# salesforce/LayoutDETR

Measured on AMD Instinct MI355X. Metric: images/sec G+D fwd-bwd, 256x256 bg x9 elems, higher is better.
Workload: dtype f32

## Files before the change

### include/ldetr_hip.h

```cpp
#ifndef LDETR_HIP_H
#define LDETR_HIP_H

#include <stdint.h>

#ifdef __cplusplus
extern "C" {
#endif

const char* ldetr_last_error(void);
int ldetr_abi_version(void);

int ldetr_debug_trace_tiles(int64_t* buffer);

int ldetr_set_split_bf16(int tiles);

int ldetr_engine_launch_counts(int64_t* f32_pipe, int64_t* bf16_split_pipe);

int ldetr_set_workspace(void* ptr, int64_t bytes);

typedef struct ldetr_tensor4 {
    int N, C, H, W;
    int64_t sn, sc, sh, sw;
} ldetr_tensor4;

typedef struct ldetr_epilogue {
    float alpha;
    const float* col_scale;
    const float* col_bias;
    const float* samp_scale;
    int64_t samp_ld;
    const float* residual;
    int64_t ldr;
    int act;
    float act_alpha;
    float act_gain;
    const float* mask_src;
    int64_t ldm;
    int mask_mode;
    float out_scale;
    float p_drop;
    uint64_t seed;
    const uint64_t* seed_ptr;
    int accumulate;
    float* a_rowsum;
} ldetr_epilogue;

int ldetr_bias_act_f32(const float* x, const float* b, const float* xref, const float* yref, const float* dy, float* y,
                       int64_t sizeX, int sizeB, int64_t stepB, int grad, int act, float alpha, float gain, float clamp,
                       void* stream);

int ldetr_upfirdn2d_f32(const float* x, const float* f, float* y, int N, int C, int inH, int inW,
                        const int64_t* x_strides_nchw, int fh, int fw, int64_t f_stride_h, int64_t f_stride_w,
                        int upx, int upy, int downx, int downy, int padx0, int padx1, int pady0, int pady1, int flip,
                        float gain, int outH, int outW, const int64_t* y_strides_nchw,
                        const float* act_bias, int has_act, float act_alpha, float act_gain, void* stream);

int ldetr_gemm_f32(const float* A, int64_t lda, int ta, const float* B, int64_t ldb, int tb, float* C, int64_t ldc,
                   int M, int N, int K, int splitk, const ldetr_epilogue* ep, int pix_per_sample, void* stream);

typedef struct ldetr_gemm_desc {
    const float* A; int64_t lda; int ta;
    const float* B; int64_t ldb; int tb;
    float* C; int64_t ldc;
    int M, N, K, splitk;
    const ldetr_epilogue* ep;
    int pix_per_sample;
} ldetr_gemm_desc;
int ldetr_gemm_pair_f32(const ldetr_gemm_desc* g0, const ldetr_gemm_desc* g1, void* stream);
int ldetr_gemm_pair_is_single_launch(const ldetr_gemm_desc* g0, const ldetr_gemm_desc* g1);

#define LDETR_GEMM_GROUP_MAX 32
int ldetr_gemm_small_group_f32(const ldetr_gemm_desc* g, const float* post_scale, int n, void* stream);

int ldetr_conv2d_fwd_f32(const float* x, const ldetr_tensor4* xt, const float* w, int Cout, int KH, int KW, int stride,
                         int pad, float* y, int64_t ldy, int OH, int OW, const float* in_scale, int64_t in_scale_ld,
                         const ldetr_epilogue* ep, void* stream);
int ldetr_conv2d_bwd_data_f32(const float* dy, const ldetr_tensor4* dyt, const float* w, int Cin, int KH, int KW,
                              int stride, int pad, float* dx, int64_t lddx, int IH, int IW, const float* dy_scale,
                              int64_t dy_scale_ld, const ldetr_epilogue* ep, void* stream);
int ldetr_conv2d_bwd_weight_f32(const float* x, const ldetr_tensor4* xt, const float* dy, const ldetr_tensor4* dyt,
                                float* dw, int KH, int KW, int stride, int pad, int splitk, const float* x_scale,
                                int64_t x_scale_ld, const float* dy_scale, int64_t dy_scale_ld, int accumulate, void* stream);

int ldetr_conv_transpose2d_fwd_f32(const float* x, const ldetr_tensor4* xt, const float* w, int Cout, int KH, int KW,
                                   int stride, int pad, float* y, int64_t ldy, int OH, int OW, const float* in_scale,
                                   int64_t in_scale_ld, const ldetr_epilogue* ep, void* stream);
int ldetr_conv_transpose2d_bwd_data_f32(const float* dy, const ldetr_tensor4* dyt, const float* w, int Cin, int KH,
                                        int KW, int stride, int pad, float* dx, int64_t lddx, int IH, int IW,
                                        const float* dy_scale, int64_t dy_scale_ld, const ldetr_epilogue* ep,
                                        void* stream);
int ldetr_conv_transpose2d_bwd_weight_f32(const float* x, const ldetr_tensor4* xt, const float* dy,
                                          const ldetr_tensor4* dyt, float* dw, int KH, int KW, int stride, int pad,
                                          int splitk, const float* x_scale, int64_t x_scale_ld, const float* dy_scale,
                                          int64_t dy_scale_ld, int accumulate, void* stream);

int ldetr_attention_fwd_f32(const float* q, int64_t ldq, const float* k, int64_t ldk, const float* v, int64_t ldv,
                            const unsigned char* key_padding_mask, float* out, int64_t ldo, float* lse, int B, int H,
                            int Lq, int Lk, int head_dim, float scale, float p_drop, uint64_t seed, const uint64_t* seed_ptr,
                            int causal, void* stream);
int ldetr_attention_bwd_f32(const float* q, int64_t ldq, const float* k, int64_t ldk, const float* v, int64_t ldv,
                            const unsigned char* key_padding_mask, const float* out, int64_t ldo, const float* lse,
                            const float* dout, int64_t lddo, float* dq, int64_t lddq, float* dk, int64_t lddk,
                            float* dv, int64_t lddv, int B, int H, int Lq, int Lk, int head_dim, float scale,
                            float p_drop, uint64_t seed, const uint64_t* seed_ptr, int causal, void* stream);

int ldetr_torgb_bwd_finish_f32(const float* dws, const float* s, const float* w, int B, int C, float* dw, float* ds, void* stream);

int ldetr_loss_combine_fwd_f32(const float* const* x, const float* w, const int* n, const int* fn, const int* red, int K, int ld,
                               float* vals, float* sums, float* total, void* stream);
int ldetr_loss_combine_bwd_f32(const float* const* x, const float* w, const int* n, const int* fn, const int* red, int K, int ld,
                               const float* g, float* grads, void* stream);
int ldetr_masked_mse_fwd_f32(const float* a, const float* b, const uint8_t* valid, int64_t rows, int D, int bdiv, float* out2, void* stream);
int ldetr_masked_mse_bwd_f32(const float* a, const float* b, const uint8_t* valid, int64_t rows, int D, int bdiv, const float* out2,
                             const float* g, float* da, void* stream);

typedef struct ldetr_ln_args {
    const float* x; const float* r; const float* gamma; const float* beta;
    float* y; float* z; float* mean; float* rstd;
    const float* dy; float* dx; float* dr; float* dgamma; float* dbeta;
    int64_t rows; int D; float eps, p_drop; uint64_t seed; const uint64_t* seed_ptr;
    const float* pos; int64_t pos_rows; float* ypos; const float* dy2;
    int r_parts; int64_t r_part_stride; const float* r_bias;
    const float* dy_parts; int dy_nparts; int64_t dy_part_stride;
} ldetr_ln_args;
int ldetr_layernorm_fwd_group_f32(const ldetr_ln_args* a, int n, void* stream);
int ldetr_layernorm_bwd_group_f32(const ldetr_ln_args* a, int n, void* stream);
int ldetr_sum_parts_f32(const float* base, const float* parts, int n_parts, int64_t part_stride, float* out, int64_t n, void* stream);

typedef struct ldetr_ffn_args {
    const float* x; int64_t ldx;
    const float* w1; const float* b1;
    const float* w2;
    float* h;
    float* ypart;
    int M, F;
    float p_drop; uint64_t seed; const uint64_t* seed_ptr;
    const float* dy;
    float* dxpart;
    float* dh;
} ldetr_ffn_args;
int ldetr_ffn_fwd_group_f32(const ldetr_ffn_args* a, int n, void* stream);
int ldetr_ffn_bwd_group_f32(const ldetr_ffn_args* a, int n, void* stream);

typedef struct ldetr_mha_small_args {
    const float* x; int64_t ldx;
    const float* w_in; const float* b_in; const float* w_out;
    const unsigned char* kpm;
    float* qkv; float* o; float* lse; float* ypart;
    int B, L;
    float scale, p_drop; uint64_t seed; const uint64_t* seed_ptr;
    const float* dr;
    float* dqkv; float* dxpart;
} ldetr_mha_small_args;
int ldetr_mha_small_fwd_group_f32(const ldetr_mha_small_args* a, int n, void* stream);
int ldetr_mha_small_bwd_group_f32(const ldetr_mha_small_args* a, int n, void* stream);

typedef struct ldetr_mha_cross_args {
// ... 296 lines not shown
```

### layoutdetr_amd/_lib.py

```python
import ctypes
import os
from ctypes import (POINTER, Structure, c_char_p, c_double, c_float, c_int, c_int64, c_ubyte, c_uint64, c_void_p)

_HERE = os.path.dirname(os.path.abspath(__file__))
ABI_VERSION = 25
LIB_PATH = os.environ.get('LDETR_LIB') or os.path.join(_HERE, 'lib', 'libldetr_hip.so')


class Tensor4(Structure):
    _fields_ = [('N', c_int), ('C', c_int), ('H', c_int), ('W', c_int),
                ('sn', c_int64), ('sc', c_int64), ('sh', c_int64), ('sw', c_int64)]


class GemmDesc(Structure):
    _fields_ = [('A', c_void_p), ('lda', c_int64), ('ta', c_int), ('B', c_void_p), ('ldb', c_int64), ('tb', c_int),
                ('C', c_void_p), ('ldc', c_int64), ('M', c_int), ('N', c_int), ('K', c_int), ('splitk', c_int),
                ('ep', c_void_p), ('pix_per_sample', c_int)]


class P3Epilogue(Structure):
    _fields_ = [('alpha', c_float), ('col_scale', c_void_p), ('col_bias', c_void_p), ('residual_p3', c_void_p),
                ('residual_f32', c_void_p), ('relu_mask_p3', c_void_p), ('relu', c_int)]


class Epilogue(Structure):
    _fields_ = [('alpha', c_float), ('col_scale', c_void_p), ('col_bias', c_void_p), ('samp_scale', c_void_p),
                ('samp_ld', c_int64), ('residual', c_void_p), ('ldr', c_int64), ('act', c_int),
                ('act_alpha', c_float), ('act_gain', c_float), ('mask_src', c_void_p), ('ldm', c_int64),
                ('mask_mode', c_int), ('out_scale', c_float), ('p_drop', c_float), ('seed', c_uint64),
                ('seed_ptr', c_void_p), ('accumulate', c_int), ('a_rowsum', c_void_p)]


class LnArgs(Structure):
    _fields_ = [('x', c_void_p), ('r', c_void_p), ('gamma', c_void_p), ('beta', c_void_p),
                ('y', c_void_p), ('z', c_void_p), ('mean', c_void_p), ('rstd', c_void_p),
                ('dy', c_void_p), ('dx', c_void_p), ('dr', c_void_p), ('dgamma', c_void_p), ('dbeta', c_void_p),
                ('rows', c_int64), ('D', c_int), ('eps', c_float), ('p_drop', c_float), ('seed', c_uint64), ('seed_ptr', c_void_p),
                ('pos', c_void_p), ('pos_rows', c_int64), ('ypos', c_void_p), ('dy2', c_void_p),
                ('r_parts', c_int), ('r_part_stride', c_int64), ('r_bias', c_void_p),
                ('dy_parts', c_void_p), ('dy_nparts', c_int), ('dy_part_stride', c_int64)]


class FfnArgs(Structure):
    _fields_ = [('x', c_void_p), ('ldx', c_int64), ('w1', c_void_p), ('b1', c_void_p), ('w2', c_void_p), ('h', c_void_p), ('ypart', c_void_p),
                ('M', c_int), ('F', c_int), ('p_drop', c_float), ('seed', c_uint64), ('seed_ptr', c_void_p),
                ('dy', c_void_p), ('dxpart', c_void_p), ('dh', c_void_p)]


class MhaSmallArgs(Structure):
    _fields_ = [('x', c_void_p), ('ldx', c_int64), ('w_in', c_void_p), ('b_in', c_void_p), ('w_out', c_void_p), ('kpm', c_void_p),
                ('qkv', c_void_p), ('o', c_void_p), ('lse', c_void_p), ('ypart', c_void_p), ('B', c_int), ('L', c_int),
                ('scale', c_float), ('p_drop', c_float), ('seed', c_uint64), ('seed_ptr', c_void_p),
                ('dr', c_void_p), ('dqkv', c_void_p), ('dxpart', c_void_p)]


class MhaCrossArgs(Structure):
    _fields_ = [('x', c_void_p), ('ldx', c_int64), ('w_q', c_void_p), ('b_q', c_void_p), ('k', c_void_p), ('ldk', c_int64), ('v', c_void_p), ('ldv', c_int64),
                ('w_out', c_void_p), ('kpm', c_void_p), ('q', c_void_p), ('o', c_void_p), ('lse', c_void_p), ('ypart', c_void_p),
                ('B', c_int), ('Lq', c_int), ('Lk', c_int), ('scale', c_float), ('p_drop', c_float), ('seed', c_uint64), ('seed_ptr', c_void_p),
                ('dr', c_void_p), ('dq', c_void_p), ('dk', c_void_p), ('lddk', c_int64), ('dv', c_void_p), ('lddv', c_int64), ('dxpart', c_void_p)]


class WgradDesc(Structure):
    _fields_ = [('A', c_void_p), ('lda', c_int64), ('B', c_void_p), ('ldb', c_int64), ('dW', c_void_p), ('ldw', c_int64), ('db', c_void_p),
                ('M', c_int), ('rows', c_int), ('cols', c_int)]


class DemodDesc(Structure):
    _fields_ = [('weight', c_void_p), ('so', c_int64), ('si', c_int64), ('sh', c_int64), ('sw', c_int64),
                ('styles', c_void_p), ('dcoefs', c_void_p), ('w2', c_void_p), ('grad_dcoefs', c_void_p), ('dweight', c_void_p), ('dstyles', c_void_p),
                ('O', c_int), ('I', c_int), ('KH', c_int), ('KW', c_int)]


class AffineDesc(Structure):
    _fields_ = [('ds', c_void_p), ('A', c_void_p), ('dA', c_void_p), ('db', c_void_p), ('C', c_int), ('scale', c_float), ('post', c_float)]


class LayoutRasterArgs(Structure):
    _fields_ = [('struct_bytes', c_int), ('B', c_int), ('N', c_int), ('S', c_int), ('nrow', c_int), ('n_colors', c_int), ('n_pages', c_int),
                ('bbox', c_void_p), ('valid', c_void_p), ('labels', c_void_p), ('palette', c_void_p), ('page_wh', c_void_p),
                ('pages', c_void_p), ('pages_bytes', c_int64), ('page_table', c_void_p), ('page_index', c_void_p),
                ('coeffs', c_void_p), ('coeffs_len', c_int64), ('cell_coeffs', c_void_p), ('cells_dev', c_void_p), ('out', c_void_p)]


class PatchResizeArgs(Structure):
    _fields_ = [('struct_bytes', c_int), ('n_jobs', c_int), ('src0', c_void_p), ('src0_bytes', c_int64), ('src1', c_void_p), ('src1_bytes', c_int64),
                ('dst', c_void_p), ('dst_bytes', c_int64), ('jobs', c_void_p), ('tables', c_void_p), ('tables_host', c_void_p), ('tables_len', c_int64),
                ('jobs_dev', c_void_p)]


class ImageRasterArgs(Structure):
    _fields_ = [('struct_bytes', c_int), ('B', c_int), ('N', c_int), ('S', c_int), ('nrow', c_int),
                ('bbox', c_void_p), ('valid', c_void_p), ('rects', c_void_p), ('patch_off', c_void_p), ('page_off', c_void_p), ('page_wh', c_void_p),
# ... 37 lines not shown
                            _I, _F, _I, _I, POINTER(c_int64), _P, _I, _F, _F, _P],
    'ldetr_gemm_f32': [_P, _L, _I, _P, _L, _I, _P, _L, _I, _I, _I, _I, _EP, _I, _P],
    'ldetr_conv2d_fwd_f32': [_P, _T4, _P, _I, _I, _I, _I, _I, _P, _L, _I, _I, _P, _L, _EP, _P],
    'ldetr_conv2d_bwd_data_f32': [_P, _T4, _P, _I, _I, _I, _I, _I, _P, _L, _I, _I, _P, _L, _EP, _P],
    'ldetr_conv2d_bwd_weight_f32': [_P, _T4, _P, _T4, _P, _I, _I, _I, _I, _I, _P, _L, _P, _L, _I, _P],
    'ldetr_conv_transpose2d_fwd_f32': [_P, _T4, _P, _I, _I, _I, _I, _I, _P, _L, _I, _I, _P, _L, _EP, _P],
    'ldetr_conv_transpose2d_bwd_data_f32': [_P, _T4, _P, _I, _I, _I, _I, _I, _P, _L, _I, _I, _P, _L, _EP, _P],
    'ldetr_conv_transpose2d_bwd_weight_f32': [_P, _T4, _P, _T4, _P, _I, _I, _I, _I, _I, _P, _L, _P, _L, _I, _P],
    'ldetr_attention_fwd_f32': [_P, _L, _P, _L, _P, _L, _P, _P, _L, _P, _I, _I, _I, _I, _I, _F, _F, c_uint64, _P, _I, _P],
    'ldetr_attention_bwd_f32': [_P, _L, _P, _L, _P, _L, _P, _P, _L, _P, _P, _L, _P, _L, _P, _L, _P, _L,
                                _I, _I, _I, _I, _I, _F, _F, c_uint64, _P, _I, _P],
    'ldetr_colsum_f32': [_P, _P, _I, _L, _I, _P],
    'ldetr_act_bwd_reduce_f32': [_P, _P, _P, _P, _P, _P, _P, _I, _L, _I, _I, _F, _F, _P],
    'ldetr_mul_reduce_f32': [_P, _P, _P, _P, _P, _I, _L, _I, _P],
    'ldetr_torgb_fwd_f32': [_P, _P, _P, _P, _P, _I, _L, _I, _P],
    'ldetr_torgb_bwd_f32': [_P, _P, _P, _P, _P, _P, _P, _I, _L, _I, _P],
    'ldetr_maxpool3x3s2_fwd_f32': [_P, _P, _P, _I, _I, _I, _I, _P],
    'ldetr_maxpool3x3s2_bwd_f32': [_P, _P, _P, _I, _I, _I, _I, _P],
    'ldetr_grad_sanitize_f32': [_P, _L, _F, _F, _F, _F, _P],
    'ldetr_adam_step_f32': [_P, _P, _P, _P, _L, _L, _F, _F, _F, _F, _I, _F, _F, _F, _F, _P],
    'ldetr_adam_ema_step_f32': [_P, _P, _P, _P, _L, _L, _F, _F, _F, _F, _I, _F, _F, _F, _F, _P, _F, _P],
    'ldetr_ema_lerp_f32': [_P, _P, _L, _F, _P],
    'ldetr_lsap_f64': [_P, _I, _I, _I, _P, _P, _P],
    'ldetr_layoutnet_features_f32': [_P, _P, _P, POINTER(c_int), _I, _P, _L, _I, _I, _I, _P, _P],
    'ldetr_layoutnet_forward_f32': [_P, _P, _P, _P, _L, _P, _L, _I, _I, _I, _P, _P, _P, _P, _P],
    'ldetr_feature_stats_f64': [_P, _L, _I, _P, _P, _P],
    'ldetr_box_giou_pairwise_f32': [_P, _P, _I, _I, _I, _I, _P, _P, _P, _P, c_double, _P],
    'ldetr_bmm_strided_f32': [_P, _P, _P, _P, _P, _P, _I, _I, _I, _I, _I, _F, _P],
    'ldetr_softmax_xent_fwd_f32': [_P, _L, _P, _P, _P, _P, _L, _I, _L, _F, _P],
    'ldetr_softmax_xent_bwd_f32': [_P, _L, _P, _P, _P, _P, _P, _L, _L, _I, _L, _F, _P],
    'ldetr_embedding_fwd_f32': [_P, _P, _P, _P, _L, _I, _I, _I, _P],
    'ldetr_embedding_bwd_f32': [_P, _P, _P, _L, _I, _I, _L, _P],
    'ldetr_debug_trace_tiles': [_P],
    'ldetr_set_split_bf16': [c_int],
    'ldetr_engine_launch_counts': [POINTER(c_int64), POINTER(c_int64)],
    'ldetr_layernorm_fwd_group_f32': [_P, _I, _P],
    'ldetr_layernorm_bwd_group_f32': [_P, _I, _P],
    'ldetr_sum_parts_f32': [_P, _P, _I, _L, _P, _L, _P],
    'ldetr_ffn_fwd_group_f32': [_P, _I, _P],
    'ldetr_ffn_bwd_group_f32': [_P, _I, _P],
    'ldetr_mha_small_fwd_group_f32': [_P, _I, _P],
    'ldetr_mha_small_bwd_group_f32': [_P, _I, _P],
    'ldetr_mha_cross_fwd_f32': [_P, _P],
    'ldetr_mha_cross_bwd_f32': [_P, _P],
    'ldetr_wgrad_multi_f32': [_P, _I, _P],
    'ldetr_loss_combine_fwd_f32': [_P, _P, _P, _P, _P, _I, _I, _P, _P, _P, _P],
    'ldetr_loss_combine_bwd_f32': [_P, _P, _P, _P, _P, _I, _I, _P, _P, _P],
    'ldetr_masked_mse_fwd_f32': [_P, _P, _P, _L, _I, _I, _P, _P],
    'ldetr_masked_mse_bwd_f32': [_P, _P, _P, _L, _I, _I, _P, _P, _P, _P],
    'ldetr_torgb_bwd_finish_f32': [_P, _P, _P, _I, _I, _P, _P, _P],
    'ldetr_sg2_handoff_f32': [_P, _P, _P, _P, _P, _P, _P, _P, _P, _P, _P, _P, _P, _P, _I, _L, _I, _F, _F, _P],
    'ldetr_gemm_pair_f32': [_P, _P, _P],
    'ldetr_gemm_pair_is_single_launch': [_P, _P],
    'ldetr_demod_fwd_f32': [_P, _L, _L, _L, _L, _P, _P, _P, _I, _I, _I, _I, _I, _F, _P],
    'ldetr_demod_bwd_f32': [_P, _L, _L, _L, _L, _P, _P, _P, _P, _P, _I, _P, _I, _I, _I, _I, _I, _P],
    'ldetr_demod_group_fwd_f32': [_P, _I, _I, _F, _P],
    'ldetr_demod_group_bwd_f32': [_P, _I, _I, _I, _I, _P],
    'ldetr_sg2_affine_bwd_f32': [_P, _I, _P, _P, _I, _P, _L, _I, _I, _P],
    'ldetr_gemm_small_group_f32': [_P, _P, _I, _P],
    'ldetr_torgb_fwd_add_f32': [_P, _P, _P, _P, _P, _P, _I, _L, _I, _P],
    'ldetr_layout_losses_f32': [_P, _P, _P, _I, _I, _P, _P, _P],
    'ldetr_layout_losses_bwd_f32': [_P, _P, _I, _I, _P, _P],
    'ldetr_layout_finish_f32': [_P, _P, _P, _P, _P, _P, _P, _P, _P, _I, _I, _I, _P],
    'ldetr_resample_coeffs': [_I, _I, _P, _P, _L, _P],
    'ldetr_resample_coeffs_filter': [_I, _I, _I, _P, _P, _L, _P],
    'ldetr_layout_raster_cell_size': [_I, _I, _I, _P, _P],
    'ldetr_layout_raster_u8': [_P, _P],
    'ldetr_patch_resize_u8': [_P, _P],
    'ldetr_image_raster_u8': [_P, _P],
    'ldetr_p3_split_f32': [_P, _L, _P, _L, _I, _P],
    'ldetr_p3_merge_f32': [_P, _P, _L, _L, _I, _P],
    'ldetr_p3_weight_bwd': [_P, _P, _P, _I, _I, _I, _I, _P],
    'ldetr_p3_conv2d_bwd_data': [_P, _I, _I, _I, _I, _P, _I, _I, _I, _I, _I, _I, _I, _P, _P, _P, _P],
    'ldetr_p3_conv2d_fwd': [_P, _I, _I, _I, _I, _P, _I, _I, _I, _I, _I, _P, _P, _P, _P],
    'ldetr_p3_conv2d_bwd_weight': [_P, _I, _I, _I, _I, _P, _I, _I, _I, _I, _I, _P, _P, _P],
    'ldetr_p3_weight_prep': [_P, _I, _I, _P],
    'ldetr_p3_conv2d_fwd_dual': [_P, _P, _I, _I, _I, _I, _P, _P, _I, _I, _I, _I, _I, _P, _P, _P, _P, _P, _P, _P],
    'ldetr_p3_conv2d_bwd_pair': [_P, _I, _I, _I, _I, _P, _P, _I, _I, _I, _I, _I, _I, _I, _P, _P, _P, _P, _P, _P, _P],
    'ldetr_p3_last_launch': [_P],
    'ldetr_engine_last_launch': [_P],
    'ldetr_struct_sizes': [_P],
    'ldetr_resize_normalize_u8': [_P, _L, _I, _I, _I, _I, _P, _P, _I, _P, _P, _I, _P, _P, _P, _F, _F, _F, _F, _F, _F, _P],
    'ldetr_page_filter_u8': [_P, _P, _L, _I, _I, _I, _F, _P],
    'ldetr_png_scan': [_P, _L, _P, _P, _P, _P, _L, _P, _P, _L, _P],
    'ldetr_png_decode_u8': [_P, _P],
    'ldetr_png_encode_bound': [_I, _I, _P, _P],
    'ldetr_png_encode_u8': [_P, _P],
    'ldetr_png_index_bytes': [_I, _I, _P],
    'ldetr_png_scan_packed': [_P, _L, _P, _P, _P, _L, _P, _P, _P, _L, _P],
    'ldetr_png_inflate_u8': [_P, _P],
}

_lib = None


def load():
    global _lib
    if _lib is not None:
        return _lib
    if not os.path.exists(LIB_PATH):
        raise RuntimeError(
            f'{LIB_PATH} not found: build the gfx950 kernels first (python -m layoutdetr_amd.build or '
            f'__graft_entry__.build()).  layoutdetr_amd has no CPU/PyTorch fallback path.')
    import torch
    lib = ctypes.CDLL(LIB_PATH)
    lib.ldetr_last_error.restype = c_char_p
# ... 23 lines not shown
```

### layoutdetr_amd/csrc/attention.hip

```cpp
#include "ldetr_common.hpp"
#include "../../include/ldetr_hip.h"

namespace ldetr {

struct AttnParams {
    const float* q; const float* k; const float* v;
    long ldq, ldk, ldv;
    const unsigned char* kpm;
    float* o; long ldo;
    float* lse;
    const float* dout; long lddo;
    float* dq; long lddq;
    float* dk; long lddk;
    float* dv; long lddv;
    int B, H, Lq, Lk;
    float scale, p_drop;
    unsigned long long seed;
    const unsigned long long* seed_ptr;
    int causal;
};

#define MFMA16(a, b, c) __builtin_amdgcn_mfma_f32_16x16x4f32((a), (b), (c), 0, 0, 0)

__device__ __forceinline__ float ldz(const float* p, bool ok, const float* safe) {
    const float v = *(ok ? p : safe);
    return ok ? v : 0.f;
}

__device__ __forceinline__ float attn_drop(const AttnParams& p, int bh, int q, int key, float inv_keep) {
    return drop_scale(p.seed + (p.seed_ptr ? *p.seed_ptr : 0ull), ((uint64_t)bh * p.Lq + q) * p.Lk + key, p.p_drop, inv_keep);
}

template <int NKT, int DHC>
__global__ __launch_bounds__(64) void attn_fwd_kernel(AttnParams p) {
    constexpr int DH = 32 * DHC;
    const int nqt = (p.Lq + 15) >> 4;
    const int qt = blockIdx.x % nqt;
    const int bh = blockIdx.x / nqt;
    const int b = bh / p.H, h = bh - b * p.H;
    const int lane = threadIdx.x, li = lane & 15, g = lane >> 4;
    const int q0 = qt << 4;
    const int qrow = q0 + li;
    const bool qok = qrow < p.Lq;
    const float* qp = p.q + ((long)b * p.Lq + qrow) * p.ldq + h * DH;
    const float* kb = p.k + (long)b * p.Lk * p.ldk + h * DH;
    const float* vb = p.v + (long)b * p.Lk * p.ldv + h * DH;
    const unsigned char* kpm = p.kpm ? p.kpm + (long)b * p.Lk : nullptr;

    float qf[8 * DHC];
#pragma unroll
    for (int kk = 0; kk < 8 * DHC; kk++) qf[kk] = ldz(qp + 4 * kk + g, qok, p.q) * p.scale;

    f32x4 s[NKT];
    float mx = -INFINITY;
#pragma unroll
    for (int j = 0; j < NKT; j++) {
        f32x4 acc = {0.f, 0.f, 0.f, 0.f};
        const int krow = 16 * j + li;
        const bool kok = krow < p.Lk;
        const float* kp = kb + (long)krow * p.ldk;
#pragma unroll
        for (int kk = 0; kk < 8 * DHC; kk++) acc = MFMA16(ldz(kp + 4 * kk + g, kok, p.q), qf[kk], acc);
#pragma unroll
        for (int r = 0; r < 4; r++) {
            int key = 16 * j + 4 * g + r;
            bool masked = (key >= p.Lk) || (kpm && kpm[key]) || (p.causal && key > qrow);
            acc[r] = masked ? -INFINITY : acc[r];
            mx = fmaxf(mx, acc[r]);
        }
        s[j] = acc;
    }
    mx = fmaxf(mx, __shfl_xor(mx, 16, 64));
    mx = fmaxf(mx, __shfl_xor(mx, 32, 64));
    float sum = 0.f;
#pragma unroll
    for (int j = 0; j < NKT; j++)
#pragma unroll
        for (int r = 0; r < 4; r++) { float e = expf(s[j][r] - mx); s[j][r] = e; sum += e; }
    sum += __shfl_xor(sum, 16, 64);
    sum += __shfl_xor(sum, 32, 64);
    const float inv = 1.f / sum;
    if (p.lse && g == 0 && qok) p.lse[(long)bh * p.Lq + qrow] = mx + logf(sum);
    const float inv_keep = p.p_drop > 0.f ? 1.f / (1.f - p.p_drop) : 1.f;

    f32x4 o[2 * DHC];
#pragma unroll
    for (int c = 0; c < 2 * DHC; c++) o[c] = f32x4{0.f, 0.f, 0.f, 0.f};
#pragma unroll
    for (int j = 0; j < NKT; j++) {
#pragma unroll
        for (int t = 0; t < 4; t++) {
            const int key = 16 * j + 4 * g + t;
            const bool kok = key < p.Lk;
            float pv = s[j][t] * inv;
            if (p.p_drop > 0.f) pv *= attn_drop(p, bh, qrow, key, inv_keep);
            const float* vp = vb + (long)key * p.ldv;
#pragma unroll
            for (int c = 0; c < 2 * DHC; c++) o[c] = MFMA16(ldz(vp + 16 * c + li, kok, p.q), pv, o[c]);
        }
    }
    if (qok) {
        float* op = p.o + ((long)b * p.Lq + qrow) * p.ldo + h * DH + 4 * g;
#pragma unroll
        for (int c = 0; c < 2 * DHC; c++) *reinterpret_cast<float4*>(op + 16 * c) = make_float4(o[c][0], o[c][1], o[c][2], o[c][3]);
    }
}

template <int DHC>
__global__ __launch_bounds__(64) void attn_fwd_long_kernel(AttnParams p) {
    constexpr int DH = 32 * DHC, NKT = 16;
    const int nqt = (p.Lq + 15) >> 4;
    const int qt = blockIdx.x % nqt;
    const int bh = blockIdx.x / nqt;
    const int b = bh / p.H, h = bh - b * p.H;
    const int lane = threadIdx.x, li = lane & 15, g = lane >> 4;
    const int qrow = (qt << 4) + li;
    const bool qok = qrow < p.Lq;
    const float* qp = p.q + ((long)b * p.Lq + qrow) * p.ldq + h * DH;
    const float* kb = p.k + (long)b * p.Lk * p.ldk + h * DH;
    const float* vb = p.v + (long)b * p.Lk * p.ldv + h * DH;
    const unsigned char* kpm = p.kpm ? p.kpm + (long)b * p.Lk : nullptr;
    const float inv_keep = p.p_drop > 0.f ? 1.f / (1.f - p.p_drop) : 1.f;

    float qf[8 * DHC];
#pragma unroll
    for (int kk = 0; kk < 8 * DHC; kk++) qf[kk] = ldz(qp + 4 * kk + g, qok, p.q) * p.scale;

    f32x4 o[2 * DHC];
#pragma unroll
    for (int c = 0; c < 2 * DHC; c++) o[c] = f32x4{0.f, 0.f, 0.f, 0.f};
    float run_max = -INFINITY, run_sum = 0.f;
    const int nkt = (p.Lk + 15) >> 4;
    for (int j0 = 0; j0 < nkt; j0 += NKT) {
        f32x4 s[NKT];
        float mx = run_max;
#pragma unroll
        for (int j = 0; j < NKT; j++) {
            f32x4 acc = {0.f, 0.f, 0.f, 0.f};
            const int krow = 16 * (j0 + j) + li;
            const bool kok = krow < p.Lk;
            const float* kp = kb + (long)krow * p.ldk;
#pragma unroll
            for (int kk = 0; kk < 8 * DHC; kk++) acc = MFMA16(ldz(kp + 4 * kk + g, kok, p.q), qf[kk], acc);
#pragma unroll
            for (int r = 0; r < 4; r++) {
                const int key = 16 * (j0 + j) + 4 * g + r;
                const bool masked = (key >= p.Lk) || (kpm && kpm[key]) || (p.causal && key > qrow);
                acc[r] = masked ? -INFINITY : acc[r];
                mx = fmaxf(mx, acc[r]);
            }
            s[j] = acc;
        }
        mx = fmaxf(mx, __shfl_xor(mx, 16, 64));
        mx = fmaxf(mx, __shfl_xor(mx, 32, 64));
        const float ref = (mx == -INFINITY) ? 0.f : mx;
        const float alpha = expf(run_max - ref);
        float sum = 0.f;
#pragma unroll
        for (int j = 0; j < NKT; j++)
#pragma unroll
            for (int r = 0; r < 4; r++) { const float e = expf(s[j][r] - ref); s[j][r] = e; sum += e; }
        sum += __shfl_xor(sum, 16, 64);
        sum += __shfl_xor(sum, 32, 64);
        run_sum = run_sum * alpha + sum;
        run_max = mx;
#pragma unroll
        for (int c = 0; c < 2 * DHC; c++) { o[c][0] *= alpha; o[c][1] *= alpha; o[c][2] *= alpha; o[c][3] *= alpha; }
#pragma unroll
        for (int j = 0; j < NKT; j++) {
#pragma unroll
            for (int t = 0; t < 4; t++) {
                const int key = 16 * (j0 + j) + 4 * g + t;
                const bool kok = key < p.Lk;
                float pv = s[j][t];
                if (p.p_drop > 0.f) pv *= attn_drop(p, bh, qrow, key, inv_keep);
                const float* vp = vb + (long)key * p.ldv;
#pragma unroll
                for (int c = 0; c < 2 * DHC; c++) o[c] = MFMA16(ldz(vp + 16 * c + li, kok, p.q), pv, o[c]);
            }
        }
    }
    const float inv = 1.f / run_sum;
    if (p.lse && g == 0 && qok) p.lse[(long)bh * p.Lq + qrow] = run_max + logf(run_sum);
    if (qok) {
        float* op = p.o + ((long)b * p.Lq + qrow) * p.ldo + h * DH + 4 * g;
#pragma unroll
        for (int c = 0; c < 2 * DHC; c++)
            *reinterpret_cast<float4*>(op + 16 * c) = make_float4(o[c][0] * inv, o[c][1] * inv, o[c][2] * inv, o[c][3] * inv);
    }
}

template <int NCH, int DHC>
__global__ __launch_bounds__(256) void attn_fwd_wide_kernel(AttnParams p) {
    constexpr int DH = 32 * DHC, DHP = DH + 4, NKT = 4 * NCH;
    extern __shared__ __attribute__((aligned(16))) float kv_tile[];
    const int nq64 = (p.Lq + 63) >> 6;
    const int qb = blockIdx.x % nq64;
    const int bh = blockIdx.x / nq64;
    const int b = bh / p.H, h = bh - b * p.H;
    const int wave = threadIdx.x >> 6, lane = threadIdx.x & 63, li = lane & 15, g = lane >> 4;
    const int qrow = (qb << 6) + (wave << 4) + li;
    const bool qok = qrow < p.Lq;
    const float* qp = p.q + ((long)b * p.Lq + qrow) * p.ldq + h * DH;
    const float* kb = p.k + (long)b * p.Lk * p.ldk + h * DH;
    const float* vb = p.v + (long)b * p.Lk * p.ldv + h * DH;
    const unsigned char* kpm = p.kpm ? p.kpm + (long)b * p.Lk : nullptr;

    auto stage = [&](const float* base, long ld, int key0) {
        constexpr int F4 = DH / 4;
        for (int i = threadIdx.x; i < 64 * F4; i += 256) {
            const int row = i / F4, c4 = i - row * F4;
            float4 v = make_float4(0.f, 0.f, 0.f, 0.f);
            if (key0 + row < p.Lk) v = *reinterpret_cast<const float4*>(base + (long)(key0 + row) * ld + 4 * c4);
            *reinterpret_cast<float4*>(kv_tile + row * DHP + 4 * c4) = v;
        }
    };

    float qf[8 * DHC];
#pragma unroll
    for (int kk = 0; kk < 8 * DHC; kk++) qf[kk] = ldz(qp + 4 * kk + g, qok, p.q) * p.scale;

    f32x4 s[NKT];
    float mx = -INFINITY;
#pragma unroll
    for (int c = 0; c < NCH; c++) {
        if (c > 0) __syncthreads();
        stage(kb, p.ldk, 64 * c);
        __syncthreads();
#pragma unroll
        for (int jj = 0; jj < 4; jj++) {
            const int j = 4 * c + jj;
            f32x4 acc = {0.f, 0.f, 0.f, 0.f};
            const float* kp = kv_tile + (16 * jj + li) * DHP + g;
#pragma unroll
            for (int kk = 0; kk < 8 * DHC; kk++) acc = MFMA16(kp[4 * kk], qf[kk], acc);
#pragma unroll
            for (int r = 0; r < 4; r++) {
                const int key = 16 * j + 4 * g + r;
                const bool masked = (key >= p.Lk) || (kpm && kpm[key]) || (p.causal && key > qrow);
                acc[r] = masked ? -INFINITY : acc[r];
                mx = fmaxf(mx, acc[r]);
            }
            s[j] = acc;
        }
    }
    mx = fmaxf(mx, __shfl_xor(mx, 16, 64));
    mx = fmaxf(mx, __shfl_xor(mx, 32, 64));
    float sum = 0.f;
#pragma unroll
    for (int j = 0; j < NKT; j++)
#pragma unroll
        for (int r = 0; r < 4; r++) { float e = expf(s[j][r] - mx); s[j][r] = e; sum += e; }
    sum += __shfl_xor(sum, 16, 64);
    sum += __shfl_xor(sum, 32, 64);
    const float inv = 1.f / sum;
    if (p.lse && g == 0 && qok) p.lse[(long)bh * p.Lq + qrow] = mx + logf(sum);
    const float inv_keep = p.p_drop > 0.f ? 1.f / (1.f - p.p_drop) : 1.f;

    f32x4 o[2 * DHC];
#pragma unroll
    for (int cc = 0; cc < 2 * DHC; cc++) o[cc] = f32x4{0.f, 0.f, 0.f, 0.f};
#pragma unroll
    for (int c = 0; c < NCH; c++) {
        __syncthreads();
        stage(vb, p.ldv, 64 * c);
        __syncthreads();
#pragma unroll
        for (int jj = 0; jj < 4; jj++) {
            const int j = 4 * c + jj;
#pragma unroll
            for (int t = 0; t < 4; t++) {
                const int key = 16 * j + 4 * g + t;
                float pv = s[j][t] * inv;
                if (p.p_drop > 0.f) pv *= attn_drop(p, bh, qrow, key, inv_keep);
                const float* vp = kv_tile + (16 * jj + 4 * g + t) * DHP + li;
#pragma unroll
                for (int cc = 0; cc < 2 * DHC; cc++) o[cc] = MFMA16(vp[16 * cc], pv, o[cc]);
            }
        }
    }
    if (qok) {
        float* op = p.o + ((long)b * p.Lq + qrow) * p.ldo + h * DH + 4 * g;
#pragma unroll
        for (int cc = 0; cc < 2 * DHC; cc++) *reinterpret_cast<float4*>(op + 16 * cc) = make_float4(o[cc][0], o[cc][1], o[cc][2], o[cc][3]);
    }
}

template <int NKT, int DHC>
__device__ __forceinline__ void attn_bwd_dq(const AttnParams& p, int bh, int qt) {
    constexpr int DH = 32 * DHC;
    const int b = bh / p.H, h = bh - b * p.H;
    const int lane = threadIdx.x, li = lane & 15, g = lane >> 4;
    const int qrow = (qt << 4) + li;
    const bool qok = qrow < p.Lq;
    const float* qp = p.q + ((long)b * p.Lq + qrow) * p.ldq + h * DH;
    const float* dop = p.dout + ((long)b * p.Lq + qrow) * p.lddo + h * DH;
    const float* op = p.o + ((long)b * p.Lq + qrow) * p.ldo + h * DH;
    const float* kb = p.k + (long)b * p.Lk * p.ldk + h * DH;
    const float* vb = p.v + (long)b * p.Lk * p.ldv + h * DH;
    const unsigned char* kpm = p.kpm ? p.kpm + (long)b * p.Lk : nullptr;
    const float inv_keep = p.p_drop > 0.f ? 1.f / (1.f - p.p_drop) : 1.f;

    float qf[8 * DHC], dof[8 * DHC];
    float delta = 0.f;
#pragma unroll
    for (int kk = 0; kk < 8 * DHC; kk++) {
        qf[kk] = ldz(qp + 4 * kk + g, qok, p.q) * p.scale;
        dof[kk] = ldz(dop + 4 * kk + g, qok, p.q);
        delta += dof[kk] * ldz(op + 4 * kk + g, qok, p.q);
    }
    delta += __shfl_xor(delta, 16, 64);
    delta += __shfl_xor(delta, 32, 64);
    const float lse = qok ? p.lse[(long)bh * p.Lq + qrow] : 0.f;

    f32x4 dq[2 * DHC];
#pragma unroll
    for (int c = 0; c < 2 * DHC; c++) dq[c] = f32x4{0.f, 0.f, 0.f, 0.f};
    const int nkt_all = (p.Lk + 15) >> 4;
    for (int j0 = 0; j0 < nkt_all; j0 += NKT)
#pragma unroll
    for (int jj = 0; jj < NKT; jj++) {
        const int j = j0 + jj;
        f32x4 sacc = {0.f, 0.f, 0.f, 0.f}, dpacc = {0.f, 0.f, 0.f, 0.f};
        const int krow = 16 * j + li;
        const bool kok = krow < p.Lk;
        const float* kp = kb + (long)krow * p.ldk;
        const float* vp = vb + (long)krow * p.ldv;
#pragma unroll
        for (int kk = 0; kk < 8 * DHC; kk++) {
            sacc = MFMA16(ldz(kp + 4 * kk + g, kok, p.q), qf[kk], sacc);
            dpacc = MFMA16(ldz(vp + 4 * kk + g, kok, p.q), dof[kk], dpacc);
        }
        f32x4 ds;
#pragma unroll
        for (int r = 0; r < 4; r++) {
            int key = 16 * j + 4 * g + r;
            bool masked = (key >= p.Lk) || (kpm && kpm[key]) || (p.causal && key > qrow);
            float pr = masked ? 0.f : expf(sacc[r] - lse);
// ... 188 lines not shown
            const float* qp = Qs + (16 * jq + li) * DHP + g;
            const float* dop = Ds + (16 * jq + li) * DHP + g;
#pragma unroll
            for (int kk = 0; kk < 8; kk++) {
                sacc = MFMA16(qp[4 * kk] * p.scale, kf[kk], sacc);
                dpacc = MFMA16(dop[4 * kk], vf[kk], dpacc);
            }
            float pd[4], ds[4];
#pragma unroll
            for (int r = 0; r < 4; r++) {
                const int qr = 16 * jq + 4 * g + r;
                const bool qok = qr < p.Lq;
                const float pr = (kmasked || !qok || (p.causal && krow > qr)) ? 0.f : expf(sacc[r] - lse_s[qr]);
                float dm = 1.f;
                if (p.p_drop > 0.f) dm = attn_drop(p, bh, qr, krow, inv_keep);
                pd[r] = pr * dm;
                ds[r] = pr * (dpacc[r] * dm - delta_s[qr]) * p.scale;
            }
#pragma unroll
            for (int t = 0; t < 4; t++) {
                const int qr = 16 * jq + 4 * g + t;
#pragma unroll
                for (int c = 0; c < 2; c++) {
                    dv[c] = MFMA16(Ds[qr * DHP + 16 * c + li], pd[t], dv[c]);
                    dk[c] = MFMA16(Qs[qr * DHP + 16 * c + li], ds[t], dk[c]);
                }
            }
        }
        if (kok) {
            float* dkp = p.dk + ((long)b * p.Lk + krow) * p.lddk + h * DH + 4 * g;
            float* dvp = p.dv + ((long)b * p.Lk + krow) * p.lddv + h * DH + 4 * g;
#pragma unroll
            for (int c = 0; c < 2; c++) {
                *reinterpret_cast<float4*>(dkp + 16 * c) = make_float4(dk[c][0], dk[c][1], dk[c][2], dk[c][3]);
                *reinterpret_cast<float4*>(dvp + 16 * c) = make_float4(dv[c][0], dv[c][1], dv[c][2], dv[c][3]);
            }
        }
    }
}

static int check_attn(const AttnParams& p, const char* what) {
    LDETR_CHECK(p.q && p.k && p.v && p.o, "%s: null pointer", what);
    LDETR_CHECK(p.B > 0 && p.H > 0 && p.Lq > 0 && p.Lk > 0, "%s: empty problem", what);
    LDETR_CHECK(p.Lk <= 16384, "%s: Lk > 16384 is unsupported", what);
    LDETR_CHECK(p.p_drop >= 0.f && p.p_drop < 1.f, "%s: dropout must be in [0,1)", what);
    LDETR_CHECK((p.ldo % 4) == 0 && ((uintptr_t)p.o & 15) == 0, "%s: output must be 16-byte aligned", what);
    return LDETR_OK;
}

}

using namespace ldetr;

extern "C" int ldetr_attention_fwd_f32(const float* q, int64_t ldq, const float* k, int64_t ldk, const float* v, int64_t ldv,
                                       const unsigned char* key_padding_mask, float* out, int64_t ldo, float* lse,
                                       int B, int H, int Lq, int Lk, int head_dim, float scale,
                                       float p_drop, uint64_t seed, const uint64_t* seed_ptr, int causal, void* stream) {
    LDETR_CHECK(head_dim >= 32 && head_dim <= 192 && head_dim % 32 == 0, "attention_fwd: head_dim must be a multiple of 32 up to 192 (got %d)", head_dim);
    AttnParams p; memset(&p, 0, sizeof(p));
    p.q = q; p.k = k; p.v = v; p.ldq = ldq; p.ldk = ldk; p.ldv = ldv; p.kpm = key_padding_mask;
    p.o = out; p.ldo = ldo; p.lse = lse; p.B = B; p.H = H; p.Lq = Lq; p.Lk = Lk;
    p.scale = scale; p.p_drop = p_drop; p.seed = seed; p.seed_ptr = (const unsigned long long*)seed_ptr; p.causal = causal;
    LDETR_CHECK(!causal || Lq == Lk, "attention_fwd: the causal mask is defined for self-attention (Lq == Lk)");
    int rc = check_attn(p, "attention_fwd");
    if (rc) return rc;
    const int nqt = (Lq + 15) / 16, nkt = (Lk + 15) / 16;
    const int grid = B * H * nqt;
    hipStream_t st = (hipStream_t)stream;
#define LDETR_ATTN_FWD(DHC)                                                                     \
    do {                                                                                         \
        if (nkt <= 1) hipLaunchKernelGGL((attn_fwd_kernel<1, DHC>), grid, 64, 0, st, p);         \
        else if (nkt <= 2) hipLaunchKernelGGL((attn_fwd_kernel<2, DHC>), grid, 64, 0, st, p);    \
        else if (nkt <= 4) hipLaunchKernelGGL((attn_fwd_kernel<4, DHC>), grid, 64, 0, st, p);    \
        else if (nkt <= 8) hipLaunchKernelGGL((attn_fwd_kernel<8, DHC>), grid, 64, 0, st, p);    \
        else hipLaunchKernelGGL((attn_fwd_kernel<16, DHC>), grid, 64, 0, st, p);                 \
    } while (0)
    if (nkt > 16) {
        switch (head_dim / 32) {
            case 1: hipLaunchKernelGGL((attn_fwd_long_kernel<1>), grid, 64, 0, st, p); break;
            case 2: hipLaunchKernelGGL((attn_fwd_long_kernel<2>), grid, 64, 0, st, p); break;
            case 3: hipLaunchKernelGGL((attn_fwd_long_kernel<3>), grid, 64, 0, st, p); break;
            case 4: hipLaunchKernelGGL((attn_fwd_long_kernel<4>), grid, 64, 0, st, p); break;
            case 5: hipLaunchKernelGGL((attn_fwd_long_kernel<5>), grid, 64, 0, st, p); break;
            default: hipLaunchKernelGGL((attn_fwd_long_kernel<6>), grid, 64, 0, st, p); break;
        }
        return check_launch("attention_fwd_long");
    }
    if ((head_dim >= 64 || Lq >= 48) && (ldk % 4) == 0 && (ldv % 4) == 0 && ((((uintptr_t)k) | ((uintptr_t)v)) & 15) == 0) {
        const int nch = (Lk + 63) / 64, wgrid = B * H * ((Lq + 63) / 64);
#define LDETR_ATTN_WIDE(NCH, DHC)                                                                                         \
    do {                                                                                                                   \
        constexpr size_t lds = (size_t)64 * (32 * DHC + 4) * sizeof(float);                                                \
        hipLaunchKernelGGL((attn_fwd_wide_kernel<NCH, DHC>), wgrid, 256, lds, st, p);                                      \
    } while (0)
#define LDETR_ATTN_WIDE_D(DHC)                                                                                            \
    do {                                                                                                                   \
        if (nch <= 1) LDETR_ATTN_WIDE(1, DHC); else if (nch <= 2) LDETR_ATTN_WIDE(2, DHC);                                 \
        else if (nch <= 3) LDETR_ATTN_WIDE(3, DHC); else LDETR_ATTN_WIDE(4, DHC);                                          \
    } while (0)
        switch (head_dim / 32) {
            case 1: LDETR_ATTN_WIDE_D(1); break;
            case 2: LDETR_ATTN_WIDE_D(2); break;
            case 3: LDETR_ATTN_WIDE_D(3); break;
            case 4: LDETR_ATTN_WIDE_D(4); break;
            case 5: LDETR_ATTN_WIDE_D(5); break;
            default: LDETR_ATTN_WIDE_D(6); break;
        }
#undef LDETR_ATTN_WIDE_D
#undef LDETR_ATTN_WIDE
        return check_launch("attention_fwd_wide");
    }
    switch (head_dim / 32) {
        case 1: LDETR_ATTN_FWD(1); break;
        case 2: LDETR_ATTN_FWD(2); break;
        case 3: LDETR_ATTN_FWD(3); break;
        case 4: LDETR_ATTN_FWD(4); break;
        case 5: LDETR_ATTN_FWD(5); break;
        default: LDETR_ATTN_FWD(6); break;
    }
#undef LDETR_ATTN_FWD
    return check_launch("attention_fwd");
}

extern "C" int ldetr_attention_bwd_f32(const float* q, int64_t ldq, const float* k, int64_t ldk, const float* v, int64_t ldv,
                                       const unsigned char* key_padding_mask, const float* out, int64_t ldo, const float* lse,
                                       const float* dout, int64_t lddo,
                                       float* dq, int64_t lddq, float* dk, int64_t lddk, float* dv, int64_t lddv,
                                       int B, int H, int Lq, int Lk, int head_dim, float scale,
                                       float p_drop, uint64_t seed, const uint64_t* seed_ptr, int causal, void* stream) {
    LDETR_CHECK(head_dim >= 32 && head_dim <= 192 && head_dim % 32 == 0, "attention_bwd: head_dim must be a multiple of 32 up to 192 (got %d)", head_dim);
    LDETR_CHECK(lse && dout && dq && dk && dv, "attention_bwd: null pointer");
    LDETR_CHECK(!causal || Lq == Lk, "attention_bwd: the causal mask is defined for self-attention (Lq == Lk)");
    AttnParams p; memset(&p, 0, sizeof(p));
    p.q = q; p.k = k; p.v = v; p.ldq = ldq; p.ldk = ldk; p.ldv = ldv; p.kpm = key_padding_mask;
    p.o = const_cast<float*>(out); p.ldo = ldo; p.lse = const_cast<float*>(lse);
    p.dout = dout; p.lddo = lddo; p.dq = dq; p.lddq = lddq; p.dk = dk; p.lddk = lddk; p.dv = dv; p.lddv = lddv;
    p.B = B; p.H = H; p.Lq = Lq; p.Lk = Lk; p.scale = scale; p.p_drop = p_drop; p.seed = seed; p.seed_ptr = (const unsigned long long*)seed_ptr;
    p.causal = causal;
    int rc = check_attn(p, "attention_bwd");
    if (rc) return rc;
    LDETR_CHECK((lddq % 4) == 0 && (lddk % 4) == 0 && (lddv % 4) == 0 &&
                (((uintptr_t)dq | (uintptr_t)dk | (uintptr_t)dv) & 15) == 0, "attention_bwd: gradients must be 16-byte aligned");
    const int nqt = (Lq + 15) / 16, nkt = (Lk + 15) / 16;
    const int grid = B * H * (nqt + nkt);
    hipStream_t st = (hipStream_t)stream;
    if (head_dim == 32 && Lq <= 64 && Lk <= 64 && nkt >= 2 && (ldq % 4) == 0 && (ldk % 4) == 0 && (ldv % 4) == 0 && (lddo % 4) == 0 && (ldo % 4) == 0 &&
        ((((uintptr_t)q) | ((uintptr_t)k) | ((uintptr_t)v) | ((uintptr_t)dout) | ((uintptr_t)out)) & 15) == 0) {
        hipLaunchKernelGGL(attn_bwd_lds_kernel, B * H, 512, 0, st, p);
        return check_launch("attention_bwd_lds");
    }
#define LDETR_ATTN_BWD(DHC)                                                                     \
    do {                                                                                         \
        if (nkt <= 1) hipLaunchKernelGGL((attn_bwd_kernel<1, DHC>), grid, 64, 0, st, p);         \
        else if (nkt <= 2) hipLaunchKernelGGL((attn_bwd_kernel<2, DHC>), grid, 64, 0, st, p);    \
        else if (nkt <= 4) hipLaunchKernelGGL((attn_bwd_kernel<4, DHC>), grid, 64, 0, st, p);    \
        else if (nkt <= 8) hipLaunchKernelGGL((attn_bwd_kernel<8, DHC>), grid, 64, 0, st, p);    \
        else hipLaunchKernelGGL((attn_bwd_kernel<16, DHC>), grid, 64, 0, st, p);                 \
    } while (0)
    switch (head_dim / 32) {
        case 1: LDETR_ATTN_BWD(1); break;
        case 2: LDETR_ATTN_BWD(2); break;
        case 3: LDETR_ATTN_BWD(3); break;
        case 4: LDETR_ATTN_BWD(4); break;
        case 5: LDETR_ATTN_BWD(5); break;
        default: LDETR_ATTN_BWD(6); break;
    }
#undef LDETR_ATTN_BWD
    return check_launch("attention_bwd");
}
```

### layoutdetr_amd/csrc/gemm_conv.hip

```cpp
#include <cstdlib>
#include <type_traits>
#include <atomic>
#include "ldetr_common.hpp"
#include "../../include/ldetr_hip.h"

namespace ldetr {
static thread_local int64_t t_launches_f32 = 0, t_launches_split = 0;
void count_engine_launch(bool bf16_split_pipe) { (bf16_split_pipe ? t_launches_split : t_launches_f32)++; }

enum {
    OP_KC_DENSE = 0,
    OP_KC_CONV = 1,
    OP_KC_CONVT = 2,
    OP_KC_WTAP = 3,
    OP_RC_DENSE = 4,
    OP_RC_PIX = 5,
    OP_RC_WT = 6,
    OP_RC_CONVK = 7,
};

struct Operand {
    const float* p;
    long ld;
    int vec;
// ... 1220 lines not shown
    float alpha, post;
};
struct SmallGroup { SmallGroupProblem q[LDETR_GEMM_GROUP_MAX]; int start[LDETR_GEMM_GROUP_MAX + 1]; int n; GemmEpilogue ep0; };

template <int NW, bool FAST>
__global__ __launch_bounds__(NW * 64) void gemm_small_group_kernel(SmallGroup g) {
    const int blk = (int)blockIdx.x;
    int pi = 0;
    for (int i = 1; i < g.n; i++) pi += (blk >= g.start[i]) ? 1 : 0;
    const SmallGroupProblem& q = g.q[pi];
    GemmParams p = {};
    p.A.KW = p.A.KH = p.A.stride = p.A.C = p.A.Cr = 1; p.B.KW = p.B.KH = p.B.stride = p.B.C = p.B.Cr = 1;
    p.A.p = q.A; p.A.ld = q.lda; p.A.vec = q.avec; p.B.p = q.B; p.B.ld = q.ldb; p.B.vec = q.bvec;
    p.M = q.M; p.N = q.N; p.K = q.K; p.C = q.C; p.ldc = q.ldc;
    p.splitk = 1; p.pstep = 1; p.nsamp = 1;
    p.ep = g.ep0; p.ep.alpha = q.alpha; p.ep.col_bias = q.col_bias;
    const int t = blk - g.start[pi], gx = (q.N + 31) >> 5;
    gemm_small_body<0, 0, NW, FAST, true>(p, t % gx, t / gx, 0, 1, gx, q.post);
}

static inline bool al16(const void* p) { return (((uintptr_t)p) & 15) == 0; }


constexpr long WS_COUNTERS = 262144;
struct Workspace { void* ptr; size_t bytes; size_t counter_cursor; size_t partial_cursor; };
static Workspace g_workspace[64];
static Workspace& workspace_for_current_device() {
    static Workspace none = {nullptr, 0, 0, 0};
    int dev = 0;
    if (hipGetDevice(&dev) != hipSuccess || dev < 0 || dev >= 64) return none;
    return g_workspace[dev];
}

static bool ring_alloc(long tiles, size_t bytes, int** counters, float** partials) {
    Workspace& w = workspace_for_current_device();
    const size_t need = (bytes + 255) & ~(size_t)255;
    const size_t pbytes = w.bytes > WS_COUNTERS * sizeof(int) ? w.bytes - WS_COUNTERS * sizeof(int) : 0;
    if (!w.ptr || need > pbytes || tiles > WS_COUNTERS) return false;
    if (w.counter_cursor + tiles > (size_t)WS_COUNTERS) w.counter_cursor = 0;
    if (w.partial_cursor + need > pbytes) w.partial_cursor = 0;
    *counters = reinterpret_cast<int*>(w.ptr) + w.counter_cursor;
    *partials = reinterpret_cast<float*>(reinterpret_cast<char*>(w.ptr) + WS_COUNTERS * sizeof(int) + w.partial_cursor);
    w.counter_cursor += tiles; w.partial_cursor += need;
    return true;
}

bool splitk_ws_alloc(long tiles, size_t partial_bytes, float** ws, int** counters) { return ring_alloc(tiles, partial_bytes, counters, ws); }

float* scratch_alloc(size_t bytes) {
    int* counters; float* r;
    return ring_alloc(0, bytes, &counters, &r) ? r : nullptr;
}

static int plan_small_split(GemmParams& p, long blocks) {
    int sk = 1;
    if (blocks <= 128 && p.K >= 1024) {
        sk = p.K / 256; if (sk > 8) sk = 8;
        while (sk > 1 && blocks * sk > 640) sk--;
        if (sk > 1 && !ring_alloc(blocks, (size_t)blocks * sk * 1024 * sizeof(float), &p.ws_count, &p.ws)) sk = 1;
    }
    return sk;
}

static bool small_fast_ok(const GemmParams& p, int ta, int tb) {
    static const int on = (int)knob("SMALL_FAST", 1);
    const long a_bytes = (ta ? (long)p.K * p.A.ld : (long)p.M * p.A.ld) * 4, b_bytes = (tb ? (long)p.K * p.B.ld : (long)p.N * p.B.ld) * 4;
    return on && (p.K % 32) == 0 && a_bytes < 0x7fffffffL && b_bytes < 0x7fffffffL && (ta || (p.A.ld % 4) == 0) && (tb || (p.B.ld % 4) == 0) &&
           ((((uintptr_t)p.A.p) | ((uintptr_t)p.B.p)) & 15) == 0;
}

static bool small_wants8(long blocks, int sk, int K) { return blocks * sk <= 256 && (K + sk - 1) / sk >= 512; }

template <int NW, bool FAST, int TA, int TB>
static auto small_kernel() { return gemm_small_kernel<TA, TB, NW, FAST>; }
template <int NW, bool FAST, int TA0, int TB0, int TA1, int TB1>
static auto small_kernel() { return gemm_small_pair_kernel<TA0, TB0, TA1, TB1, NW, FAST>; }

template <int... MODES, typename... Args>
static void launch_small_kernel(bool fast, bool w8, dim3 grid, hipStream_t st, const Args&... args) {
    if (fast) {
        if (w8) hipLaunchKernelGGL((small_kernel<8, true, MODES...>()), grid, 512, 0, st, args...);
        else hipLaunchKernelGGL((small_kernel<4, true, MODES...>()), grid, 256, 0, st, args...);
    } else {
        if (w8) hipLaunchKernelGGL((small_kernel<8, false, MODES...>()), grid, 512, 0, st, args...);
        else hipLaunchKernelGGL((small_kernel<4, false, MODES...>()), grid, 256, 0, st, args...);
    }
    t_launches_f32++;
}

template <int TA, int TB>
static int launch_small(GemmParams& p, hipStream_t st) {
    dim3 grid(cdiv(p.N, 32), cdiv(p.M, 32), 1);
    const long blocks = (long)grid.x * grid.y;
    const int sk = plan_small_split(p, blocks);
    grid.z = sk;
    const bool fast = small_fast_ok(p, TA, TB);
    const bool w8 = small_wants8(blocks, sk, p.K);
    launch_small_kernel<TA, TB>(fast, w8, grid, st, p);
    note_engine_launch(2, 32, 32, 0, w8 ? 8 : 4, fast ? 1 : 0, 0, sk, blocks * sk, TA * 2 + TB);
    return check_launch("gemm_small");
}

template <int TA0>
static int launch_small_pair(GemmParams& p0, GemmParams& p1, hipStream_t st) {
    const int gx0 = cdiv(p0.N, 32), nt0 = gx0 * cdiv(p0.M, 32), gx1 = cdiv(p1.N, 32), nt1 = gx1 * cdiv(p1.M, 32);
    const int sk0 = plan_small_split(p0, nt0), sk1 = plan_small_split(p1, nt1);
    const bool w8 = small_wants8(nt0, sk0, p0.K) && small_wants8(nt1, sk1, p1.K);
    const bool fast = small_fast_ok(p0, TA0, 1) && small_fast_ok(p1, 1, 1);
    const dim3 grid((unsigned)(nt0 * sk0 + nt1 * sk1));
    launch_small_kernel<TA0, 1, 1, 1>(fast, w8, grid, st, p0, p1, gx0, nt0, sk0, gx1, nt1, sk1);
    note_engine_launch(3, 32, 32, 0, w8 ? 8 : 4, fast ? 1 : 0, 0, sk0 * 256 + sk1, (long)grid.x, (TA0 * 2 + 1) * 4 + 3);
    return check_launch("gemm_small_pair");
}
// ... 373 lines not shown
    const bool auto_split = (g.splitk == 0);
    const bool small = auto_split && small_class(M, N, K);
    if (p.ep.a_rowsum) {
        LDETR_CHECK(ta == 1 && g.lda == M, "gemm: a_rowsum needs ta == 1 and a packed A (lda == M)");
        if (!(small && tb)) {
            int rc = ldetr_colsum_f32(g.A, p.ep.a_rowsum, 1, K, M, stream);
            if (rc) return rc;
            p.ep.a_rowsum = nullptr;
        }
    }
    if (small) {
        if (!ta && !tb) return launch_small<0, 0>(p, st);
        if (!ta && tb) return launch_small<0, 1>(p, st);
        if (ta && tb) return launch_small<1, 1>(p, st);
    }
    if (!ta && !tb) return launch_gemm<OP_KC_DENSE, OP_KC_DENSE>(p, M, M, 1, auto_split, false, st);
    if (!ta && tb) return launch_gemm<OP_KC_DENSE, OP_RC_DENSE>(p, M, M, 1, auto_split, false, st);
    if (ta && tb) return launch_gemm<OP_RC_DENSE, OP_RC_DENSE>(p, M, M, 1, auto_split, false, st);
    set_error("gemm: (ta=1, tb=0) is not instantiated");
    return LDETR_ERR_UNSUPPORTED;
}

extern "C" int ldetr_gemm_f32(const float* A, int64_t lda, int ta, const float* B, int64_t ldb, int tb,
                              float* C, int64_t ldc, int M, int N, int K, int splitk,
                              const ldetr_epilogue* ep, int pix_per_sample, void* stream) {
    const ldetr_gemm_desc g = {A, lda, ta, B, ldb, tb, C, ldc, M, N, K, splitk, ep, pix_per_sample};
    return gemm_dense(g, stream);
}

static bool small_class(const ldetr_gemm_desc& g) {
    return g.splitk == 0 && g.M > 0 && g.N > 0 && g.K > 0 && small_class(g.M, g.N, g.K);
}

static bool pair_single_launch(const ldetr_gemm_desc* g0, const ldetr_gemm_desc* g1) {
    static const int pair_on = (int)knob("GEMM_PAIR", 1);
    const bool nn_tn = g0->ta == 0 && g0->tb == 1 && g1->ta == 1 && g1->tb == 1, tn_tn = g0->ta == 1 && g0->tb == 1 && g1->ta == 1 && g1->tb == 1;
    return pair_on && (nn_tn || tn_tn) && g0->A && g0->B && g0->C && g1->A && g1->B && g1->C && small_class(*g0) && small_class(*g1) &&
           (!g1->ep || !g1->ep->a_rowsum || g1->lda == g1->M) && (!(g0->ep && g0->ep->a_rowsum) || (tn_tn && g0->lda == g0->M));
}

extern "C" int ldetr_gemm_pair_is_single_launch(const ldetr_gemm_desc* g0, const ldetr_gemm_desc* g1) {
    return (g0 && g1 && pair_single_launch(g0, g1)) ? 1 : 0;
}

extern "C" int ldetr_gemm_pair_f32(const ldetr_gemm_desc* g0, const ldetr_gemm_desc* g1, void* stream) {
    LDETR_CHECK(g0 && g1, "gemm_pair: null descriptor");
    if (pair_single_launch(g0, g1)) {
        GemmParams p0 = fill_dense(*g0), p1 = fill_dense(*g1);
        return g0->ta == 1 ? launch_small_pair<1>(p0, p1, (hipStream_t)stream) : launch_small_pair<0>(p0, p1, (hipStream_t)stream);
    }
    int rc = gemm_dense(*g0, stream);
    if (rc) return rc;
    return gemm_dense(*g1, stream);
}

static int launch_small_group(const ldetr_gemm_desc* d, const float* post_scale, int n, hipStream_t st) {
    SmallGroup g; memset(&g, 0, sizeof(g));
    g.n = n;
    fill_epilogue(g.ep0, nullptr);
    long total = 0;
    bool fast = false, w8 = false;
    for (int i = 0; i < n; i++) {
        const ldetr_gemm_desc& q = d[i];
        LDETR_CHECK(q.A && q.B && q.C, "gemm_small_group: null pointer (problem %d)", i);
        LDETR_CHECK(q.M > 0 && q.N > 0 && q.K > 0, "gemm_small_group: empty problem %d", i);
        const ldetr_epilogue* e = q.ep;
        const bool plain_ep = !e || (!e->col_scale && !e->samp_scale && !e->residual && e->act == 0 && e->mask_mode == 0 && e->out_scale == 1.f &&
                                     e->p_drop == 0.f && !e->accumulate && !e->a_rowsum);
        if (q.ta || q.tb || q.splitk != 0 || !plain_ep || !small_class(q.M, q.N, q.K)) {
            set_error("gemm_small_group: problem %d is not a plain NN small-tile problem", i);
            return LDETR_ERR_UNSUPPORTED;
        }
        const long blocks = (long)cdiv(q.N, 32) * cdiv(q.M, 32);
        if (blocks <= 128 && q.K >= 1024) {
            set_error("gemm_small_group: problem %d splits its reduction", i);
            return LDETR_ERR_UNSUPPORTED;
        }
        ldetr_gemm_desc one = q; one.pix_per_sample = 0;
        const GemmParams p = fill_dense(one);
        const bool f = small_fast_ok(p, 0, 0), w = small_wants8(blocks, 1, p.K);
        if (i == 0) { fast = f; w8 = w; }
        else if (f != fast || w != w8) {
            set_error("gemm_small_group: problem %d resolves to another instantiation than problem 0", i);
            return LDETR_ERR_UNSUPPORTED;
        }
        SmallGroupProblem& o = g.q[i];
        LDETR_CHECK(q.lda < 0x7fffffffL && q.ldb < 0x7fffffffL && q.ldc < 0x7fffffffL, "gemm_small_group: leading dimension above 2^31 (problem %d)", i);
        o.A = q.A; o.B = q.B; o.C = q.C; o.col_bias = p.ep.col_bias;
        o.lda = (int)q.lda; o.ldb = (int)q.ldb; o.ldc = (int)q.ldc; o.avec = p.A.vec; o.bvec = p.B.vec; o.M = q.M; o.N = q.N; o.K = q.K;
        o.alpha = p.ep.alpha; o.post = post_scale ? post_scale[i] : 1.f;
        g.start[i] = (int)total;
        total += blocks;
    }
    g.start[n] = (int)total;
    const dim3 grid((unsigned)total);
    if (fast) {
        if (w8) hipLaunchKernelGGL((gemm_small_group_kernel<8, true>), grid, 512, 0, st, g);
        else hipLaunchKernelGGL((gemm_small_group_kernel<4, true>), grid, 256, 0, st, g);
    } else {
        if (w8) hipLaunchKernelGGL((gemm_small_group_kernel<8, false>), grid, 512, 0, st, g);
        else hipLaunchKernelGGL((gemm_small_group_kernel<4, false>), grid, 256, 0, st, g);
    }
    t_launches_f32++;
    note_engine_launch(7, 32, 32, 0, w8 ? 8 : 4, fast ? 1 : 0, 0, 1, total, 0);
    return check_launch("gemm_small_group");
}
// ... 204 lines not shown
```

### layoutdetr_amd/hip/attention.py

```python
import math

import torch

from . import core
from .linear import linear


class _AttnFn(torch.autograd.Function):

    @staticmethod
    def forward(ctx, q, k, v, kpm, B, H, Lq, Lk, p_drop, kv_grad_dst=None):
        core.require_gpu(q, k, v, kpm)
        ctx.kv_grad_dst = kv_grad_dst
        dh = q.shape[1] // H
        assert q.stride(1) == 1 and k.stride(1) == 1 and v.stride(1) == 1
        d = H * dh
        out = torch.empty((B * Lq, d), device=q.device, dtype=torch.float32)
        lse = torch.empty((B * H * Lq,), device=q.device, dtype=torch.float32)
        seed = core.next_seed() if p_drop > 0 else 0
        scale = 1.0 / math.sqrt(dh)
        core.check(core.lib().ldetr_attention_fwd_f32(
            core.ptr(q), q.stride(0), core.ptr(k), k.stride(0), core.ptr(v), v.stride(0), core.ptr(kpm),
            core.ptr(out), d, core.ptr(lse), B, H, Lq, Lk, dh, scale, p_drop, seed, core.seed_ptr() if p_drop > 0 else None,
            0, core.stream()), 'attention_fwd')
        ctx.save_for_backward(q, k, v, kpm, out, lse)
        ctx.cfg = (B, H, Lq, Lk, dh, scale, p_drop, seed)
        return out

    @staticmethod
    def backward(ctx, dout):
        q, k, v, kpm, out, lse = ctx.saved_tensors
        B, H, Lq, Lk, dh, scale, p_drop, seed = ctx.cfg
        d = H * dh
        dout = core.f32c(dout)
        dq = torch.empty((B * Lq, d), device=q.device, dtype=torch.float32)
        if ctx.kv_grad_dst is not None:
            dk, dv = ctx.kv_grad_dst()
        else:
            dk = torch.empty((B * Lk, d), device=q.device, dtype=torch.float32)
            dv = torch.empty((B * Lk, d), device=q.device, dtype=torch.float32)
        core.check(core.lib().ldetr_attention_bwd_f32(
            core.ptr(q), q.stride(0), core.ptr(k), k.stride(0), core.ptr(v), v.stride(0), core.ptr(kpm),
            core.ptr(out), d, core.ptr(lse), core.ptr(dout), d, core.ptr(dq), d, core.ptr(dk), dk.stride(0), core.ptr(dv), dv.stride(0),
            B, H, Lq, Lk, dh, scale, p_drop, seed, core.seed_ptr() if p_drop > 0 else None, 0, core.stream()), 'attention_bwd')
        return dq, dk, dv, None, None, None, None, None, None, None


class _AttnPackedFn(torch.autograd.Function):

    @staticmethod
    def forward(ctx, qkv, v_sep, kpm, B, H, L, p_drop, causal=False):
        core.require_gpu(qkv, v_sep, kpm)
        assert qkv.stride(1) == 1
        d = qkv.shape[1] // (3 if v_sep is None else 2)
        dh = d // H
        q, k = qkv[:, :d], qkv[:, d:2 * d]
        v = qkv[:, 2 * d:] if v_sep is None else v_sep
        assert v.stride(1) == 1
        out = torch.empty((B * L, d), device=qkv.device, dtype=torch.float32)
        lse = torch.empty((B * H * L,), device=qkv.device, dtype=torch.float32)
        seed = core.next_seed() if p_drop > 0 else 0
        scale = 1.0 / math.sqrt(dh)
        core.check(core.lib().ldetr_attention_fwd_f32(
            core.ptr(q), q.stride(0), core.ptr(k), k.stride(0), core.ptr(v), v.stride(0), core.ptr(kpm),
            core.ptr(out), d, core.ptr(lse), B, H, L, L, dh, scale, p_drop, seed, core.seed_ptr() if p_drop > 0 else None,
            1 if causal else 0, core.stream()), 'attention_fwd')
        ctx.save_for_backward(qkv, v_sep, kpm, out, lse)
        ctx.cfg = (B, H, L, dh, scale, p_drop, seed, 1 if causal else 0)
        return out

    @staticmethod
    def backward(ctx, dout):
        qkv, v_sep, kpm, out, lse = ctx.saved_tensors
        B, H, L, dh, scale, p_drop, seed, causal = ctx.cfg
        d = H * dh
        q, k = qkv[:, :d], qkv[:, d:2 * d]
        v = qkv[:, 2 * d:] if v_sep is None else v_sep
        dout = core.f32c(dout)
        dqkv = torch.empty_like(qkv)
        dq, dk = dqkv[:, :d], dqkv[:, d:2 * d]
        dv = dqkv[:, 2 * d:] if v_sep is None else torch.empty((B * L, d), device=qkv.device, dtype=torch.float32)
        core.check(core.lib().ldetr_attention_bwd_f32(
            core.ptr(q), q.stride(0), core.ptr(k), k.stride(0), core.ptr(v), v.stride(0), core.ptr(kpm),
            core.ptr(out), d, core.ptr(lse), core.ptr(dout), d, core.ptr(dq), dq.stride(0), core.ptr(dk), dk.stride(0),
            core.ptr(dv), dv.stride(0), B, H, L, L, dh, scale, p_drop, seed, core.seed_ptr() if p_drop > 0 else None,
            causal, core.stream()), 'attention_bwd')
        return dqkv, (None if v_sep is None else dv), None, None, None, None, None, None


def kpm_u8(key_padding_mask):
    m = key_padding_mask
    if m is None:
        return None
    if m.dtype == torch.bool:
        return (m if m.is_contiguous() else m.contiguous()).view(torch.uint8)
    return m.to(torch.uint8).contiguous()


def attention(q, k, v, key_padding_mask, B, H, Lq, Lk, p_drop=0.0, kv_grad_dst=None):
    return _AttnFn.apply(q, k, v, kpm_u8(key_padding_mask), B, H, Lq, Lk, p_drop, kv_grad_dst)


class _GroupedKVFn(torch.autograd.Function):

    @staticmethod
    def forward(ctx, mem_pos, mem, holder, *params):
        core.require_gpu(mem_pos, mem)
        ctx.set_materialize_grads(False)
        Ws, bs = params[0::2], params[1::2]
        n, d = len(Ws), mem.shape[1]
        M = mem.shape[0]
        mp, mm = core.f32c(mem_pos), core.f32c(mem)
        with torch.no_grad():
            Wk = torch.cat([w.detach()[d:2 * d] for w in Ws] + [w.detach()[2 * d:] for w in Ws])
            bk = torch.cat([b.detach()[d:2 * d] for b in bs] + [b.detach()[2 * d:] for b in bs])
        nd = n * d
        KV = torch.empty((M, 2 * nd), device=mem.device, dtype=torch.float32)
        core.gemm(mp, Wk[:nd], 0, 0, M, nd, d, out=KV[:, :nd], ep=core.epilogue(col_bias=bk[:nd]))
        core.gemm(mm, Wk[nd:], 0, 0, M, nd, d, out=KV[:, nd:], ep=core.epilogue(col_bias=bk[nd:]))
# ... 122 lines not shown
```

### layoutdetr_amd/hip/blocks.py

```python
import math

from .. import _lib
from . import core

D_MODEL, N_HEAD = 256, 8
SCALE = 1.0 / math.sqrt(D_MODEL // N_HEAD)

_ENTRIES = {'layernorm_fwd': ('ldetr_layernorm_fwd_group_f32', True), 'layernorm_bwd': ('ldetr_layernorm_bwd_group_f32', True),
            'ffn_fwd': ('ldetr_ffn_fwd_group_f32', True), 'ffn_bwd': ('ldetr_ffn_bwd_group_f32', True),
            'mha_small_fwd': ('ldetr_mha_small_fwd_group_f32', True), 'mha_small_bwd': ('ldetr_mha_small_bwd_group_f32', True),
            'mha_cross_fwd': ('ldetr_mha_cross_fwd_f32', False), 'mha_cross_bwd': ('ldetr_mha_cross_bwd_f32', False)}


def launch(what, args, flops=0.0, nbytes=0.0):
    entry, grouped = _ENTRIES[what]
    fn = getattr(core.lib(), entry)
    n = len(args)
    arr = (type(args[0]) * n)(*args)
    if grouped:
        call = lambda: core.check(fn(arr, n, core.stream()), what)
    else:
        assert n == 1
        call = lambda: core.check(fn(arr, core.stream()), what)
    if flops > 0:
        core.engine_call('ldetr_token_stack', flops, call, nbytes=nbytes)
    else:
        call()


def draw_seed(p_drop):
    return core.next_seed() if p_drop > 0 else 0


def _set_dropout(a, p_drop, seed):
    a.p_drop, a.seed, a.seed_ptr = p_drop, seed, (core.iter_seed().data_ptr() if p_drop > 0 else None)


def _p(t):
    return t.data_ptr() if t is not None else None


def ln_fwd(x, r, gamma, beta, eps, p_drop, seed, y, z, mean, rstd, r_parts=0, r_bias=None, pos=None, ypos=None):
    a = _lib.LnArgs()
    M, D = x.shape
    a.x, a.r, a.gamma, a.beta, a.y, a.z, a.mean, a.rstd = x.data_ptr(), _p(r), gamma.data_ptr(), beta.data_ptr(), y.data_ptr(), _p(z), mean.data_ptr(), rstd.data_ptr()
    a.rows, a.D, a.eps = M, D, eps
    if r is not None:
        _set_dropout(a, p_drop, seed)
    a.r_parts, a.r_part_stride = r_parts, M * D
    a.r_bias = _p(r_bias) if r_parts > 0 else None
    if pos is not None:
        a.pos, a.pos_rows, a.ypos = pos.data_ptr(), pos.shape[0], ypos.data_ptr()
    return a


def ln_bwd(dy, z, mean, rstd, gamma, dx, dr, dgamma, dbeta, p_drop, seed, dy2=None, parts=None, n_parts=0):
    a = _lib.LnArgs()
    M, D = z.shape
    a.dy, a.z, a.mean, a.rstd, a.gamma, a.dx = dy.data_ptr(), z.data_ptr(), mean.data_ptr(), rstd.data_ptr(), gamma.data_ptr(), dx.data_ptr()
    a.dy2, a.dr, a.dgamma, a.dbeta = _p(dy2), _p(dr), _p(dgamma), _p(dbeta)
    a.dy_parts = parts.data_ptr() if n_parts else None
    a.dy_nparts, a.dy_part_stride = n_parts, M * D
    a.rows, a.D = M, D
    _set_dropout(a, p_drop, seed)
    return a


def ffn_fwd(x, w1, b1, w2, h, ypart, p_drop, seed):
    a = _lib.FfnArgs()
    a.x, a.ldx, a.w1, a.b1, a.w2, a.h, a.ypart = x.data_ptr(), x.stride(0), w1.data_ptr(), b1.data_ptr(), w2.data_ptr(), h.data_ptr(), ypart.data_ptr()
    a.M, a.F = h.shape
    _set_dropout(a, p_drop, seed)
    return a


def ffn_bwd(dy, x, h, w1, w2, dxpart, dh, p_drop):
    a = _lib.FfnArgs()
    a.dy, a.x, a.ldx, a.h, a.w1, a.w2, a.dxpart, a.dh = dy.data_ptr(), x.data_ptr(), x.stride(0), h.data_ptr(), w1.data_ptr(), w2.data_ptr(), dxpart.data_ptr(), _p(dh)
    a.M, a.F = h.shape
    a.p_drop = p_drop
    return a


def mha_small_fwd(x, w_in, b_in, w_out, kpm, qkv, o, lse, ypart, B, L, p_drop, seed):
    a = _lib.MhaSmallArgs()
    a.x, a.ldx, a.w_in, a.b_in, a.w_out, a.kpm = x.data_ptr(), x.stride(0), w_in.data_ptr(), b_in.data_ptr(), w_out.data_ptr(), _p(kpm)
    a.qkv, a.o, a.lse, a.ypart, a.B, a.L, a.scale = qkv.data_ptr(), o.data_ptr(), lse.data_ptr(), ypart.data_ptr(), B, L, SCALE
    _set_dropout(a, p_drop, seed)
    return a


def mha_small_bwd(dr, w_in, w_out, kpm, qkv, o, lse, dqkv, dxpart, B, L, p_drop, seed):
    a = _lib.MhaSmallArgs()
    a.w_in, a.w_out, a.kpm, a.qkv, a.o, a.lse = w_in.data_ptr(), w_out.data_ptr(), _p(kpm), qkv.data_ptr(), o.data_ptr(), lse.data_ptr()
    a.dr, a.dqkv, a.dxpart, a.B, a.L, a.scale = dr.data_ptr(), _p(dqkv), dxpart.data_ptr(), B, L, SCALE
    _set_dropout(a, p_drop, seed)
    return a


def mha_cross_fwd(x, w_q, b_q, k, v, w_out, kpm, q, o, lse, ypart, B, Lq, Lk, p_drop, seed):
    a = _lib.MhaCrossArgs()
    a.x, a.ldx, a.w_q, a.b_q, a.w_out, a.kpm = x.data_ptr(), x.stride(0), w_q.data_ptr(), b_q.data_ptr(), w_out.data_ptr(), _p(kpm)
    a.k, a.ldk, a.v, a.ldv = k.data_ptr(), k.stride(0), v.data_ptr(), v.stride(0)
    a.q, a.o, a.lse, a.ypart, a.B, a.Lq, a.Lk, a.scale = q.data_ptr(), o.data_ptr(), lse.data_ptr(), ypart.data_ptr(), B, Lq, Lk, SCALE
    _set_dropout(a, p_drop, seed)
    return a


def mha_cross_bwd(dr, w_q, k, v, w_out, kpm, q, o, lse, dq, dk, dv, dxpart, B, Lq, Lk, p_drop, seed):
    a = _lib.MhaCrossArgs()
    a.w_q, a.w_out, a.kpm, a.q, a.o, a.lse = w_q.data_ptr(), w_out.data_ptr(), _p(kpm), q.data_ptr(), o.data_ptr(), lse.data_ptr()
    a.k, a.ldk, a.v, a.ldv = k.data_ptr(), k.stride(0), v.data_ptr(), v.stride(0)
    a.dr, a.dq, a.dk, a.lddk, a.dv, a.lddv, a.dxpart = dr.data_ptr(), dq.data_ptr(), dk.data_ptr(), dk.stride(0), dv.data_ptr(), dv.stride(0), dxpart.data_ptr()
    a.B, a.Lq, a.Lk, a.scale = B, Lq, Lk, SCALE
    _set_dropout(a, p_drop, seed)
    return a
```

### layoutdetr_amd/hip/core.py

```python
import ctypes
import os

import torch

from .. import _lib
from .._lib import Epilogue, Tensor4

ACT_NONE, ACT_RELU, ACT_LRELU = 0, 1, 2

_seed_counter = [0x5EED]

WEIGHT_GRADIENTS_DISABLED = [False]


class _EngineProfile(object):

    def __init__(self):
        self.enabled = False
        self.records = []

    def reset(self):
        self.records = []

    def summary(self):
# ... 33 lines not shown
    return default


def engine_call(tag, flops, thunk, operands=(), nbytes=None):
    if not PROF.enabled:
        return thunk()
    s = torch.cuda.Event(enable_timing=True)
    e = torch.cuda.Event(enable_timing=True)
    c0 = engine_launch_counts()
    s.record()
    r = thunk()
    e.record()
    c1 = engine_launch_counts()
    if nbytes is None:
        nbytes = 4.0 * sum(t.numel() for t in operands if t is not None)
    PROF.records.append((tag, float(flops), s, e, nbytes, (c1[0] - c0[0], c1[1] - c0[1]), launched_kernel(tag)))
    return r


_P3_KINDS = {1: 'p3_nt_kernel', 2: 'p3_c3_kernel', 3: 'p3_tn_kernel', 4: 'p3_bwd_pair_nt_kernel', 5: 'p3_bwd_pair_c3_kernel'}
_ENGINE_KINDS = {1: 'gemm_f32_kernel', 2: 'gemm_small_kernel', 3: 'gemm_small_pair_kernel', 4: 'conv3x3_c32_kernel', 5: 'wgrad_c32_3x3_kernel', 6: 'stem_conv7x7_kernel', 7: 'gemm_small_group_kernel'}


def launched_kernel(tag):
    info = (ctypes.c_int32 * 10)()
    if tag.startswith('ldetr_p3'):
        check(lib().ldetr_p3_last_launch(info), 'p3_last_launch')
        kind, bm, bn, nw, sk = info[0], info[1], info[2], info[3], info[4]
        name = _P3_KINDS.get(kind, 'p3_?')
        if kind in (2, 5):
            return name
        return f'{name}<{bm},{bn},{nw}w>' + (f' splitK={sk}' if sk > 1 else '')
    if tag == 'ldetr_token_stack':
        return 'token-stack kernels (mha_small / mha_cross / ffn / wgrad_multi)'
    check(lib().ldetr_engine_last_launch(info), 'engine_last_launch')
    kind, bm, bn, bk, nw, fast, split, sk = [info[i] for i in range(8)]
    name = _ENGINE_KINDS.get(kind, 'engine_?')
    if kind == 1:
        return f'{name}<{bm},{bn},{bk},{nw}w' + (',FAST' if fast else '') + (',SPLIT' if split else '') + '>' + (f' splitK={sk}' if sk > 1 else '')
    if kind in (2, 3, 7):
        return f'{name}<{nw}w' + (',FAST' if fast else '') + '>'
    if kind == 4:
        return 'conv3x3_c32_split_kernel' if split else name
    return name


def engine_launch_counts():
    a, b = ctypes.c_int64(0), ctypes.c_int64(0)
    lib().ldetr_engine_launch_counts(ctypes.byref(a), ctypes.byref(b))
    return a.value, b.value



_workspace = {}
WORKSPACE_BYTES = int(os.environ.get('LDETR_WORKSPACE_MIB', '256')) << 20


def disable_splitk_workspace():
    l = _lib.load()
    dev = torch.cuda.current_device()
    _workspace[dev] = None
    check(l.ldetr_set_workspace(None, 0), 'set_workspace')


def enable_splitk_workspace():
    _workspace.pop(torch.cuda.current_device(), None)
    lib()


def lib():
    l = _lib.load()
    if torch.cuda.is_available():
        dev = torch.cuda.current_device()
        if dev not in _workspace:
            ws = torch.zeros(WORKSPACE_BYTES // 4, dtype=torch.float32, device=torch.device('cuda', dev))
            _workspace[dev] = ws
            check_rc = l.ldetr_set_workspace(ctypes.c_void_p(ws.data_ptr()), ws.numel() * 4)
            if check_rc != 0:
                raise RuntimeError('ldetr_set_workspace failed: ' + l.ldetr_last_error().decode())
    return l


def check(rc, what=''):
    _lib.check(rc, what)


def require_gpu(*tensors):
    for t in tensors:
        if t is not None and t.device.type != 'cuda':
            raise RuntimeError('layoutdetr_amd ops require tensors in GPU memory (no CPU fallback); got device '
                               f'{t.device}')


def stream():
    return ctypes.c_void_p(torch.cuda.current_stream().cuda_stream)


def ptr(t):
    if t is None:
        return None
    return ctypes.c_void_p(t.data_ptr())


def f32c(t):
    if t is None:
        return None
    if t.dtype != torch.float32:
        t = t.float()
    return t.contiguous()


def next_seed():
    _seed_counter[0] += 1
    base = int(torch.initial_seed()) & 0xFFFFFFFF
    return ((base << 32) ^ (_seed_counter[0] * 0x9E3779B1)) & 0xFFFFFFFFFFFFFFFF


_iter_seed = {}


def iter_seed(device=None):
    device = torch.device('cuda', torch.cuda.current_device()) if device is None else torch.device(device)
    key = (device.type, device.index)
    if key not in _iter_seed:
        _iter_seed[key] = torch.zeros(1, dtype=torch.int64, device=device)
    return _iter_seed[key]


def reseed(device=None):
    iter_seed(device).random_()


def seed_ptr():
    return ctypes.c_void_p(iter_seed().data_ptr())


def tensor4_nhwc(x):
    N, H, W, C = x.shape
    sn, sh, sw, sc = x.stride()
    return Tensor4(N, C, H, W, sn, sc, sh, sw)


def tensor4_nchw(x):
    N, C, H, W = x.shape
    sn, sc, sh, sw = x.stride()
    return Tensor4(N, C, H, W, sn, sc, sh, sw)


def epilogue(alpha=1.0, col_scale=None, col_bias=None, samp_scale=None, residual=None, act=ACT_NONE, act_alpha=0.0,
             act_gain=1.0, mask_src=None, mask_mode=0, out_scale=1.0, p_drop=0.0, seed=0, accumulate=False, a_rowsum=None):
    ep = Epilogue()
    ep.alpha = alpha
    ep.col_scale = col_scale.data_ptr() if col_scale is not None else None
    ep.col_bias = col_bias.data_ptr() if col_bias is not None else None
    if samp_scale is not None:
        ep.samp_scale = samp_scale.data_ptr()
        ep.samp_ld = samp_scale.stride(0)
    if residual is not None:
        ep.residual = residual.data_ptr()
        ep.ldr = residual.shape[-1]
    ep.act = act
    ep.act_alpha = act_alpha
    ep.act_gain = act_gain
    if mask_src is not None:
        ep.mask_src = mask_src.data_ptr()
        ep.ldm = mask_src.shape[-1]
    ep.mask_mode = mask_mode
    ep.out_scale = out_scale
    ep.p_drop = p_drop
    ep.seed = seed
    ep.seed_ptr = iter_seed().data_ptr() if p_drop > 0 else None
    ep.accumulate = 1 if accumulate else 0
    ep.a_rowsum = a_rowsum.data_ptr() if a_rowsum is not None else None
    return ep


def gemm(A, B, ta, tb, M, N, K, out=None, ep=None, splitk=0, pix_per_sample=0, lda=None, ldb=None):
    require_gpu(A, B)
    if out is None:
        out = torch.empty((M, N), device=A.device, dtype=torch.float32)
    lda = A.stride(0) if lda is None else lda
    ldb = B.stride(0) if ldb is None else ldb
    engine_call('gemm', 2.0 * M * N * K, lambda: check(lib().ldetr_gemm_f32(
        ptr(A), lda, int(ta), ptr(B), ldb, int(tb), ptr(out), out.stride(0), M, N, K, splitk,
        ctypes.byref(ep) if ep is not None else None, pix_per_sample, stream()), 'gemm'), nbytes=4.0 * (M * K + N * K + M * N))
    return out


def _pair_descs(g0, g1):
    descs = []
    flops = 0.0
    for g in (g0, g1):
        require_gpu(g['A'], g['B'], g['out'])
        d = _lib.GemmDesc()
        d.A = g['A'].data_ptr(); d.lda = g['A'].stride(0); d.ta = int(g['ta'])
        d.B = g['B'].data_ptr(); d.ldb = g['B'].stride(0); d.tb = int(g['tb'])
        d.C = g['out'].data_ptr(); d.ldc = g['out'].stride(0)
        d.M, d.N, d.K, d.splitk = int(g['M']), int(g['N']), int(g['K']), 0
        d.ep = ctypes.addressof(g['ep']) if g.get('ep') is not None else None
        d.pix_per_sample = 0
        descs.append(d)
        flops += 2.0 * d.M * d.N * d.K
    return descs, flops


def gemm_pair_is_single_launch(g0, g1):
    descs, _ = _pair_descs(g0, g1)
    return lib().ldetr_gemm_pair_is_single_launch(ctypes.byref(descs[0]), ctypes.byref(descs[1])) == 1


def gemm_pair(g0, g1):
    descs, flops = _pair_descs(g0, g1)
    engine_call('gemm', flops, lambda: check(lib().ldetr_gemm_pair_f32(ctypes.byref(descs[0]), ctypes.byref(descs[1]), stream()), 'gemm_pair'),
                nbytes=4.0 * sum(d.M * d.K + d.N * d.K + d.M * d.N for d in descs))


GEMM_GROUP_MAX = 32


def gemm_group(problems, post=None):
    n = len(problems)
    if n < 1 or n > GEMM_GROUP_MAX:
        return False
    descs = (_lib.GemmDesc * n)()
    flops = nbytes = 0.0
    for d, g in zip(descs, problems):
        require_gpu(g['A'], g['B'], g['out'])
        d.A = g['A'].data_ptr(); d.lda = g['A'].stride(0); d.ta = 0
        d.B = g['B'].data_ptr(); d.ldb = g['B'].stride(0); d.tb = 0
        d.C = g['out'].data_ptr(); d.ldc = g['out'].stride(0)
        d.M, d.N, d.K, d.splitk = int(g['M']), int(g['N']), int(g['K']), 0
        d.ep = ctypes.addressof(g['ep']) if g.get('ep') is not None else None
        d.pix_per_sample = 0
        flops += 2.0 * d.M * d.N * d.K
        nbytes += 4.0 * (d.M * d.K + d.N * d.K + d.M * d.N)
# ... 95 lines not shown
```

### layoutdetr_amd/hip/linear.py

```python
import ctypes
import os

import torch

from . import core
from .core import ACT_LRELU, ACT_NONE, ACT_RELU


def act_backward(dy2, y2, act, act_alpha, act_gain, want_dbias, bias=None, demod=None, want_ddemod=False, B=1, dbias_out=None):
    R, C = dy2.shape
    if C % 4 != 0:
        if act == ACT_NONE:
            dv = dy2 * act_gain if act_gain != 1.0 else dy2
        else:
            neg = 0.0 if act == ACT_RELU else act_alpha
            dv = dy2 * torch.where(y2 > 0, act_gain, act_gain * neg)
        if want_dbias and dbias_out is not None:
            dbias_out += dv.sum(0)
            return dv, None, None
        return dv, (dv.sum(0) if want_dbias else None), None
    dv = torch.empty_like(dy2)
    if want_dbias and dbias_out is not None:
        dbias = dbias_out
    else:
        dbias = torch.zeros(C, device=dy2.device, dtype=torch.float32) if want_dbias else None
    ddemod = core.zeros((B, C), dy2.device) if want_ddemod else None
    core.check(core.lib().ldetr_act_bwd_reduce_f32(
        core.ptr(dy2), core.ptr(y2), core.ptr(dv), core.ptr(bias), core.ptr(demod), core.ptr(dbias), core.ptr(ddemod),
        B, R // B, C, act, act_alpha, act_gain, core.stream()), 'act_bwd_reduce')
    return dv, (None if dbias_out is not None else dbias), ddemod


class _LinearFn(torch.autograd.Function):
    @staticmethod
    def forward(ctx, x, weight, bias, act, act_alpha, act_gain, p_drop, wscale, rows, add_input, passthru):
        core.require_gpu(x, weight, bias)
        ctx.set_materialize_grads(False)
        r0, r1 = rows if rows is not None else (0, weight.shape[0])
        N, K = r1 - r0, weight.shape[1]
        x2 = x.reshape(-1, K)
        if not (x2.dtype == torch.float32 and x2.stride(1) == 1 and x2.stride(0) >= K and x2.stride(0) % 4 == 0 and x2.data_ptr() % 16 == 0):
            x2 = core.f32c(x2)
        if add_input is not None:
            if add_input.requires_grad:
                raise RuntimeError('linear: add_input is a constant (the sine position embedding); a learned embedding must be added by the caller')
            x2 = x2 + add_input.reshape(-1, K)
        w = core.f32c(weight.detach()[r0:r1])
        b = core.f32c(bias.detach()[r0:r1]) if bias is not None else None
        M = x2.shape[0]
        seed = core.next_seed() if p_drop > 0 else 0
        ep = core.epilogue(alpha=wscale, col_bias=b, act=act, act_alpha=act_alpha, act_gain=act_gain, p_drop=p_drop,
                           seed=seed)
        y = core.gemm(x2, w, 0, 0, M, N, K, ep=ep)
        ctx.save_for_backward(x2, w, y if act != ACT_NONE else None)
        ctx.cfg = (act, act_alpha, act_gain, p_drop, wscale, bias is not None, x.shape)
        ctx.params = (weight, bias, r0, r1)
        if p_drop > 0 and act != ACT_RELU:
            raise RuntimeError('linear: fused dropout is only defined after relu (FFN hidden layer)')
        if passthru:
            return y.reshape(*x.shape[:-1], N), x
        return y.reshape(*x.shape[:-1], N)

    @staticmethod
    def backward(ctx, dy, dx_pass=None):
        x2, w, y = ctx.saved_tensors
        act, act_alpha, act_gain, p_drop, wscale, has_bias, xshape = ctx.cfg
        N, K = w.shape
        M = x2.shape[0]
        if dy is None:
            return (dx_pass,) + (None,) * 10
        dy2 = core.f32c(dy.reshape(-1, N))
        need_x, need_w, need_b = ctx.needs_input_grad[0], ctx.needs_input_grad[1], has_bias and ctx.needs_input_grad[2]
        wparam, bparam, r0, r1 = ctx.params
        gw = core.flat_grad(wparam) if need_w else None
        gb = core.flat_grad(bparam) if need_b else None
        if gw is not None:
            gw = gw[r0:r1]
        if gb is not None:
            gb = gb[r0:r1] if (N % 4 == 0 and r0 % 4 == 0) else None
        pairable = need_x and need_w and gw is not None and gw.is_contiguous()
        dx = dw = db = None
        if act != ACT_NONE:
            gain = act_gain / (1.0 - p_drop) if p_drop > 0 else act_gain
            dpre, db, _ = act_backward(dy2, y, act, act_alpha, gain, need_b, dbias_out=gb)
        else:
            dpre = dy2
            db = None
            fold_db = need_b and gb is not None and need_w and gw is not None and gw.is_contiguous() and dpre.is_contiguous()
            if need_b and not fold_db:
                if gb is not None:
                    core.check(core.lib().ldetr_colsum_f32(core.ptr(dpre), core.ptr(gb), 1, M, N, core.stream()), 'colsum')
                else:
                    db = core.colsum(dpre).reshape(-1)
        if need_x and need_w and pairable:
            res = core.f32c(dx_pass.reshape(-1, K)) if dx_pass is not None else None
            dx2 = torch.empty((M, K), device=dpre.device, dtype=torch.float32)
            rsum = gb if (act == ACT_NONE and fold_db) else None
            core.gemm_pair(dict(A=dpre, B=w, ta=0, tb=1, M=M, N=K, K=N, out=dx2, ep=core.epilogue(alpha=wscale, residual=res)),
# ... 24 lines not shown
```

### layoutdetr_amd/training/detr_transformer.py

```python
import copy
from typing import Optional

import torch
from torch import Tensor, nn

from ..hip import composite, core
from ..hip.attention import kpm_u8 as _mask_u8
from ..hip.attention import grouped_kv, mha_cross_kv, mha_forward
from ..hip import ffn as hffn
from ..hip import stacks as hstacks
from ..hip.layernorm import add_layernorm
from ..hip.linear import linear


class _MHAParams(nn.MultiheadAttention):

    def forward(self, *a, **k):
        raise RuntimeError('use layoutdetr_amd.hip.attention.mha_forward')


def _mha(m: nn.MultiheadAttention, q2, k2, v2, B, Lq, Lk, kpm, training, same_qk=False, same_qkv=False, qk_pos=None, qk_in=None, kv_alias=False):
    p = m.dropout if training else 0.0
    return mha_forward(q2, k2, v2, m.in_proj_weight, m.in_proj_bias, m.out_proj.weight, m.out_proj.bias, m.num_heads,
                       B, Lq, Lk, key_padding_mask=kpm, p_drop=p, same_qk=same_qk, same_qkv=same_qkv, qk_pos=qk_pos, passthru=True,
                       qk_in=qk_in, kv_alias=kv_alias)


_GROUP_KV = True


def _ffn(layer, x2):
    p = layer.dropout.p if layer.training else 0.0
    if hffn.large_usable(x2, layer.linear1, layer.linear2):
        return hffn.ffn_large(x2, layer.linear1, layer.linear2, p)
    h, x2 = linear(x2, layer.linear1.weight, layer.linear1.bias, act=core.ACT_RELU, p_drop=p, passthru=True)
    return linear(h, layer.linear2.weight, layer.linear2.bias), x2


def _add_ln(norm: nn.LayerNorm, x2, r2, drop: nn.Dropout, training, pos=None):
    return add_layernorm(x2, r2, norm.weight, norm.bias, norm.eps, drop.p if training else 0.0, pos=pos)


def _add_ln_ffn_add_ln(layer, norm_a: nn.LayerNorm, x2, r2, drop_a: nn.Dropout, norm_b: nn.LayerNorm, drop_b: nn.Dropout, pos=None):
    t = layer.training
    if hffn.usable(x2, layer.linear1, layer.linear2):
        return hffn.add_ln_ffn_add_ln(x2, r2, norm_a, drop_a.p if t else 0.0, layer.linear1, layer.linear2, norm_b, layer.dropout.p if t else 0.0,
                                      drop_b.p if t else 0.0, pos=pos)
    x2 = _add_ln(norm_a, x2, r2, drop_a, t)
    f, x2 = _ffn(layer, x2)
    return _add_ln(norm_b, x2, f, drop_b, t, pos=pos)


class TransformerEncoderLayer(nn.Module):
    def __init__(self, d_model, nhead, dim_feedforward=2048, dropout=0.1, activation='relu', normalize_before=False):
        super().__init__()
        if activation != 'relu' or normalize_before:
            raise NotImplementedError('only the post-norm relu configuration used by LayoutDETR is implemented')
        self.self_attn = _MHAParams(d_model, nhead, dropout=dropout)
        self.linear1 = nn.Linear(d_model, dim_feedforward)
# ... 10 lines not shown
            a, x2 = _mha(self.self_attn, x2, x2, x2, B, L, L, kpm, self.training, same_qkv=True)
            return _add_ln_ffn_add_ln(self, self.norm1, x2, a, self.dropout1, self.norm2, self.dropout2)
        a, x2 = _mha(self.self_attn, x2, x2, x2, B, L, L, kpm, self.training, same_qk=True, qk_pos=pos2, qk_in=xpos2)
        return _add_ln_ffn_add_ln(self, self.norm1, x2, a, self.dropout1, self.norm2, self.dropout2, pos=pos2 if emit_pos else None)


class TransformerDecoderLayer(nn.Module):
    def __init__(self, d_model, nhead, dim_feedforward=2048, dropout=0.1, activation='relu', normalize_before=False):
        super().__init__()
        if activation != 'relu' or normalize_before:
            raise NotImplementedError('only the post-norm relu configuration used by LayoutDETR is implemented')
        self.self_attn = _MHAParams(d_model, nhead, dropout=dropout)
        self.multihead_attn = _MHAParams(d_model, nhead, dropout=dropout)
        self.linear1 = nn.Linear(d_model, dim_feedforward)
        self.dropout = nn.Dropout(dropout)
        self.linear2 = nn.Linear(dim_feedforward, d_model)
        self.norm1 = nn.LayerNorm(d_model)
        self.norm2 = nn.LayerNorm(d_model)
        self.norm3 = nn.LayerNorm(d_model)
        self.dropout1 = nn.Dropout(dropout)
        self.dropout2 = nn.Dropout(dropout)
        self.dropout3 = nn.Dropout(dropout)
        self.normalize_before = normalize_before

    def forward2d(self, t2, mem2, mem_pos2, B, Lq, S, tgt_kpm, mem_kpm, kv=None):
        a, t2 = _mha(self.self_attn, t2, t2, t2, B, Lq, Lq, tgt_kpm, self.training, same_qkv=True)
        t2 = _add_ln(self.norm1, t2, a, self.dropout1, self.training)
        if kv is not None:
            m = self.multihead_attn
            a, t2 = mha_cross_kv(t2, kv[0], kv[1], kv[2], m.in_proj_weight, m.in_proj_bias, m.out_proj.weight, m.out_proj.bias, m.num_heads, B, Lq, S,
                                 key_padding_mask=mem_kpm, p_drop=m.dropout if self.training else 0.0)
        else:
            a, t2, mem_pos2, mem2 = _mha(self.multihead_attn, t2, mem_pos2, mem2, B, Lq, S, mem_kpm, self.training, kv_alias=True)
        return _add_ln_ffn_add_ln(self, self.norm2, t2, a, self.dropout2, self.norm3, self.dropout3), mem2, mem_pos2


def _get_clones(module, N):
    return nn.ModuleList([copy.deepcopy(module) for _ in range(N)])


class TransformerEncoder(nn.Module):
    def __init__(self, encoder_layer, num_layers, norm=None):
        super().__init__()
        self.layers = _get_clones(encoder_layer, num_layers)
        self.num_layers = num_layers
        self.norm = norm

    def as_prog(self, x2, B, L, kpm):
        if self.norm is not None or not hstacks.ENABLED:
            return None
        prog = hstacks.Prog('enc', self.layers, x2, B, L, _mask_u8(kpm), self.training)
        return prog if hstacks.usable(prog) else None

    def forward2d(self, x2, B, L, kpm, pos2, want_pos=False):
        kpm = _mask_u8(kpm)
        if pos2 is None and not want_pos:
            prog = self.as_prog(x2, B, L, kpm)
            if prog is not None:
                return hstacks.run([prog])[0]
        xpos2 = None
        n = len(self.layers)
        for i, layer in enumerate(self.layers):
            emit = pos2 is not None and (i + 1 < n or (want_pos and self.norm is None))
            if pos2 is not None and xpos2 is None:
                xpos2 = x2 + pos2
            r = layer.forward2d(x2, B, L, kpm, pos2, xpos2=xpos2, emit_pos=emit)
            x2, xpos2 = r if emit else (r, None)
        if self.norm is not None:
            r = add_layernorm(x2, None, self.norm.weight, self.norm.bias, self.norm.eps, pos=pos2 if want_pos else None)
            x2, xpos2 = r if (want_pos and pos2 is not None) else (r, None)
        if want_pos:
            return x2, (xpos2 if xpos2 is not None else x2 + pos2)
        return x2


class TransformerDecoder(nn.Module):
    def __init__(self, decoder_layer, num_layers, norm=None, return_intermediate=False):
        super().__init__()
        if return_intermediate:
            raise NotImplementedError('return_intermediate_dec=True is not used by LayoutDETR')
        self.layers = _get_clones(decoder_layer, num_layers)
        self.num_layers = num_layers
        self.norm = norm
        self.return_intermediate = return_intermediate

    def forward2d(self, t2, mem2, pos2, B, Lq, S, tgt_kpm, mem_kpm, mem_pos2=None, partner=None):
        if mem_pos2 is None:
            mem_pos2 = mem2 + pos2
        if composite.active():
            out = composite.decoder_forward2d(self, t2, mem2, mem_pos2, B, Lq, S, tgt_kpm, mem_kpm)
            return out if partner is None else (out, hstacks.run([partner])[0])
        tgt_kpm, mem_kpm = _mask_u8(tgt_kpm), _mask_u8(mem_kpm)
        kvs = grouped_kv(mem_pos2, mem2, [l.multihead_attn for l in self.layers]) if (_GROUP_KV and len(self.layers) > 1) else None
        if kvs is not None and hstacks.ENABLED:
            prog = hstacks.Prog('dec', self.layers, t2, B, Lq, tgt_kpm, self.training, final_norm=self.norm, kvs=kvs, S=S, mem_kpm=mem_kpm)
            if hstacks.usable(prog):
                outs = hstacks.run([prog] + ([partner] if partner is not None else []))
                return outs[0] if partner is None else (outs[0], outs[1])
        for i, layer in enumerate(self.layers):
            t2, mem2, mem_pos2 = layer.forward2d(t2, mem2, mem_pos2, B, Lq, S, tgt_kpm, mem_kpm, kv=None if kvs is None else kvs[i])
        if self.norm is not None:
            t2 = add_layernorm(t2, None, self.norm.weight, self.norm.bias, self.norm.eps)
        return t2 if partner is None else (t2, hstacks.run([partner])[0])


def _rows_from_nchw(x):
    B, C, h, w = x.shape
    return x.permute(0, 2, 3, 1).reshape(B * h * w, C), h * w


class Transformer(nn.Module):
    _with_token = False

    def __init__(self, d_model=512, nhead=8, num_encoder_layers=6, num_decoder_layers=6, dim_feedforward=2048,
                 dropout=0.1, activation='relu', normalize_before=False, return_intermediate_dec=False):
        super().__init__()
        if self._with_token:
            self.token = nn.Parameter(torch.randn(1, 1, d_model))
            self.register_buffer('token_mask', torch.zeros(1, 1, dtype=torch.bool))
        encoder_layer = TransformerEncoderLayer(d_model, nhead, dim_feedforward, dropout, activation, normalize_before)
        encoder_norm = nn.LayerNorm(d_model) if normalize_before else None
        self.encoder = TransformerEncoder(encoder_layer, num_encoder_layers, encoder_norm)
        decoder_layer = TransformerDecoderLayer(d_model, nhead, dim_feedforward, dropout, activation, normalize_before)
        decoder_norm = nn.LayerNorm(d_model)
        self.decoder = TransformerDecoder(decoder_layer, num_decoder_layers, decoder_norm,
                                          return_intermediate=return_intermediate_dec)
        self._reset_parameters()
        self.d_model = d_model
        self.nhead = nhead
        if d_model % nhead != 0 or (d_model // nhead) % 32 != 0 or d_model // nhead > 192:
            raise NotImplementedError('the fused attention kernels take head widths that are multiples of 32 up to 192 '
                                      f'(d_model {d_model} / {nhead} heads = {d_model / nhead:g})')

    def _reset_parameters(self):
        for p in self.parameters():
            if p.dim() > 1:
                nn.init.xavier_uniform_(p)

    def forward(self, src, mask, pos_embed, tgt, tgt_key_padding_mask, decoder_mask=None, partner=None):
        if decoder_mask is not None:
            raise NotImplementedError('decoder_mask (tgt_mask) is never passed on the LayoutDETR path')
        bs, c, h, w = src.shape
        x2, S = _rows_from_nchw(src)
        pos2, _ = _rows_from_nchw(pos_embed)
        pos2 = pos2.contiguous()
        mem_kpm = mask.flatten(1)
        mem2, mem_pos2 = self.encoder.forward2d(x2, bs, S, mem_kpm, pos2, want_pos=True)
        if self._with_token:
            tgt = torch.cat([self.token.expand(-1, bs, -1), tgt], dim=0)
            tgt_key_padding_mask = torch.cat([self.token_mask.expand(bs, -1), tgt_key_padding_mask], dim=1)
        Lq = tgt.shape[0]
        t2 = tgt.permute(1, 0, 2).reshape(bs * Lq, c)
        hs2 = self.decoder.forward2d(t2, mem2, pos2, bs, Lq, S, tgt_key_padding_mask, mem_kpm, mem_pos2=mem_pos2, partner=partner)
        if partner is not None:
            hs2, other = hs2
        hs = hs2.reshape(bs, Lq, c)
        memory = mem2.reshape(bs, h, w, c).permute(0, 3, 1, 2)
        return (hs, memory) if partner is None else (hs, memory, other)


class TransformerWithToken(Transformer):
    _with_token = True


def build_transformer(args):
    return Transformer(d_model=args.hidden_dim, dropout=args.dropout, nhead=args.nheads,
                       dim_feedforward=args.dim_feedforward, num_encoder_layers=args.enc_layers,
                       num_decoder_layers=args.dec_layers, normalize_before=args.pre_norm, return_intermediate_dec=True)
```

### layoutdetr_amd/training/loss.py

```python

import torch
import torch.nn.functional as F

from ..detr_util.misc import NestedTensor
from ..hip import composite, core

from ..hip import losses as hl
from ..metrics.metric_layoutnet import compute_alignment, compute_overlap, generalized_iou_loss, layout_losses_per_sample
from .detr_backbone import ResNet50Body, dual_trunk_forward, trunk_body


def _masked_mse(a, b, valid):
    if a.is_cuda and a.dtype == torch.float32 and not b.requires_grad:
        return hl.masked_mse(a, b, valid.contiguous().view(torch.uint8))
    vf = valid.to(a.dtype)
    return ((a - b).square().sum(-1) * vf).sum() / (vf.sum().clamp_min(1.0) * a.shape[-1])


def _masked_ce(logits, target, valid):
    from .med import softmax_cross_entropy
    return softmax_cross_entropy(logits.flatten(0, 1), target.flatten().masked_fill(~valid.flatten(), -100), raw=True)


def _masked_giou(a, b, valid):
    unit = a.new_full((4,), 0.5)
    unit[2:] = 1.0
    v3 = valid.unsqueeze(-1)
    a2 = torch.where(v3, a, unit).flatten(0, 1)
    b2 = torch.where(v3, b, unit).flatten(0, 1)
    l1, t1, r1, b1 = a2[:, 0] - a2[:, 2] / 2, a2[:, 1] - a2[:, 3] / 2, a2[:, 0] + a2[:, 2] / 2, a2[:, 1] + a2[:, 3] / 2
    l2, t2, r2, bb2 = b2[:, 0] - b2[:, 2] / 2, b2[:, 1] - b2[:, 3] / 2, b2[:, 0] + b2[:, 2] / 2, b2[:, 1] + b2[:, 3] / 2
    a_1, a_2 = (r1 - l1) * (b1 - t1), (r2 - l2) * (bb2 - t2)
    lm, rm, tm, bm = torch.maximum(l1, l2), torch.minimum(r1, r2), torch.maximum(t1, t2), torch.minimum(b1, bb2)
    ai = torch.where((lm < rm) & (tm < bm), (rm - lm) * (bm - tm), torch.zeros_like(a_1))
    au = a_1 + a_2 - ai
    ah = (torch.maximum(r1, r2) - torch.minimum(l1, l2)) * (torch.maximum(b1, bb2) - torch.minimum(t1, t2))
    per = 1.0 - (ai / au - (ah - au) / ah)
    vf = valid.to(a.dtype).flatten()
    return (per * vf).sum() / vf.sum().clamp_min(1.0)


def _detached(trunk_out):
    feats, pos = trunk_out
    return [NestedTensor(f.tensors.detach(), f.mask, getattr(f, 'uniform', False)) for f in feats], [p.detach() for p in pos]


class Loss:
    def accumulate_gradients(self, phase, bbox_real, bbox_class, bbox_text, bbox_patch, padding_mask, background, real_c, gen_z, gen_c, gain, cur_nimg,
                             trunks=None):
        raise NotImplementedError()


class StyleGAN2Loss(Loss):
    def __init__(self, device, G, D, augment_pipe=None, r1_gamma=0.0, style_mixing_prob=0, pl_weight=0.0, pl_batch_shrink=2,
                 pl_decay=0.01, pl_no_weight_grad=False, blur_init_sigma=0, blur_fade_kimg=0,
                 Dreal_bbox_cls_weight=50.0, Dreal_bbox_rec_weight=500.0, Dreal_text_rec_weight=0.1, Dreal_text_len_rec_weight=2.0,
                 Dreal_im_rec_weight=0.5, Ggen_bbox_rec_weight=100.0, Ggen_bbox_gIoU_weight=4.0, Ggen_overlapping_weight=7.0,
                 Ggen_alignment_weight=17.0, Ggen_z_rec_weight=5.0, Ggen_bbox_cls_weight=50.0, Ggen_text_rec_weight=1.0,
                 Ggen_text_len_rec_weight=1.0, report_fn=None, share_D_trunk=True):
        super().__init__()
        self.device = device
        self.G = G
        self.D = D
        self.augment_pipe = augment_pipe
        self.r1_gamma = r1_gamma
        self.style_mixing_prob = style_mixing_prob
        self.pl_weight = pl_weight
        self.pl_batch_shrink = pl_batch_shrink
        self.pl_decay = pl_decay
        self.pl_no_weight_grad = pl_no_weight_grad
        self.pl_mean = torch.zeros([], device=device)
        self.pl_noise_fn = None
        self.w = dict(Dreal_bbox_cls=Dreal_bbox_cls_weight, Dreal_bbox_rec=Dreal_bbox_rec_weight, Dreal_text_rec=Dreal_text_rec_weight,
                      Dreal_text_len_rec=Dreal_text_len_rec_weight, Dreal_im_rec=Dreal_im_rec_weight, Ggen_bbox_rec=Ggen_bbox_rec_weight,
                      Ggen_bbox_gIoU=Ggen_bbox_gIoU_weight, Ggen_overlapping=Ggen_overlapping_weight, Ggen_alignment=Ggen_alignment_weight,
                      Ggen_z_rec=Ggen_z_rec_weight, Ggen_bbox_cls=Ggen_bbox_cls_weight, Ggen_text_rec=Ggen_text_rec_weight,
                      Ggen_text_len_rec=Ggen_text_len_rec_weight)
        self.share_D_trunk = share_D_trunk
        self.pair_D_passes = bool(share_D_trunk) and hasattr(D, 'forward_pair')
        self._reporting = report_fn is not None
        self.report = report_fn if report_fn is not None else (lambda name, value: None)
        self.last = {}

    def precompute_D_trunk(self, background, stages=None):
        if self.share_D_trunk != 'iteration' or not hasattr(self.D, 'trunk'):
            return None
        body = self.D.backbone[0].body
        trunk_params = [p for m in (self.G, self.D) if hasattr(m, 'backbone') for p in m.backbone.parameters()]
        was = [p.requires_grad for p in trunk_params]
        for p in trunk_params:
            p.requires_grad_(True)
        try:
            if stages is not None:
                body.stages = stages
            with torch.enable_grad():
                g_out, d_out = self.grouped_trunks(background)
                return g_out, (d_out if d_out is not None else self.D.trunk(background))
        finally:
            if stages is not None:
                body.stages = None
            for p, w in zip(trunk_params, was):
                p.requires_grad_(w)

    def grouped_trunks(self, background):
        g_body, d_body = trunk_body(self.G), trunk_body(self.D)
        if (not isinstance(background, torch.Tensor) or not isinstance(g_body, ResNet50Body) or type(d_body) is not type(g_body)
                or g_body.stages is not None or d_body.stages is not None):
            return None, None
        outs = dual_trunk_forward(g_body, d_body, background, background)
        if outs is None:
            return None, None
        return self.G.trunk(background, body_out=outs[0]), self.D.trunk(background, body_out=outs[1])

    def run_G(self, z, bbox_class, bbox_real, bbox_text, bbox_patch, padding_mask, background, c, reconst=False, update_emas=False, trunk_out=None):
        kw = {} if trunk_out is None else dict(trunk_out=trunk_out)
        if not reconst:
            return self.G(z, bbox_class, bbox_real, bbox_text, bbox_patch, padding_mask, background, c, **kw)
        return self.G(z, bbox_class, bbox_real, bbox_text, bbox_patch, padding_mask, background, c, reconst, **kw)

    def run_D(self, bbox, bbox_class, bbox_text, bbox_patch, padding_mask, background, c, reconst=False, blur_sigma=0, update_emas=False,
              trunk_out=None):
        kw = {} if trunk_out is None else dict(trunk_out=trunk_out)
        if not reconst:
            return self.D(bbox, bbox_class, bbox_text, bbox_patch, padding_mask, background, c, **kw)
        return self.D(bbox, bbox_class, bbox_text, bbox_patch, padding_mask, background, c, reconst, **kw)

    def g_main_loss(self, bbox_real, bbox_class, bbox_text, bbox_patch, padding_mask, background, gen_z, gen_c, gain=1.0, trunks=None):
        w = self.w
        valid = ~padding_mask
        static = bool(getattr(self.G, 'static_shapes', False))
        g_trunk, d_trunk = self.grouped_trunks(background) if trunks is None else (trunks[0], _detached(trunks[1]))
        bbox_fake, loss_z, cls_logits, loss_lm, loss_text_len = self.run_G(gen_z, bbox_class, bbox_real, bbox_text, bbox_patch, padding_mask, background, gen_c,
                                                                           reconst=True, trunk_out=g_trunk)
        gen_logits, gen_logits_uncond = self.run_D(bbox_fake, bbox_class, bbox_text, bbox_patch, padding_mask, background, gen_c, trunk_out=d_trunk)
        T = hl.Term
        lay = None
        if static and bbox_fake.is_cuda and bbox_fake.shape[1] <= 64:
            lay = layout_losses_per_sample(bbox_fake, bbox_real, valid)
        elif static:
            l_rec, l_giou = _masked_mse(bbox_fake, bbox_real, valid), _masked_giou(bbox_fake, bbox_real, valid)
            l_ovl, l_aln = compute_overlap(bbox_fake, valid), compute_alignment(bbox_fake, valid)
        else:
            l_rec, l_giou = F.mse_loss(bbox_fake[valid], bbox_real[valid]), generalized_iou_loss(bbox_fake[valid], bbox_real[valid])
            l_ovl, l_aln = compute_overlap(bbox_fake, valid), compute_alignment(bbox_fake, valid)
        self.report('Loss/scores/fake', gen_logits)
        if self._reporting:
            self.report('Loss/signs/fake', gen_logits.sign())
        terms = [T('loss_Ggen', gen_logits, 1.0, hl.SOFTPLUS_NEG), T('loss_Ggen_uncond', gen_logits_uncond, 1.0, hl.SOFTPLUS_NEG)]
        if lay is not None:
            terms.append(T(['loss_Ggen_bbox_rec', 'loss_Ggen_bbox_gIoU', 'loss_Ggen_overlapping', 'loss_Ggen_alignment'], lay,
                           [w['Ggen_bbox_rec'], w['Ggen_bbox_gIoU'], w['Ggen_overlapping'], w['Ggen_alignment']], hl.IDENT, [True, True, False, False]))
        else:
            terms += [T('loss_Ggen_bbox_rec', l_rec, w['Ggen_bbox_rec']), T('loss_Ggen_bbox_gIoU', l_giou, w['Ggen_bbox_gIoU']),
                      T('loss_Ggen_overlapping', l_ovl, w['Ggen_overlapping']), T('loss_Ggen_alignment', l_aln, w['Ggen_alignment'])]
        terms.append(T('loss_Ggen_z_rec', loss_z, w['Ggen_z_rec']))
        if static:
            terms.append(T('loss_Ggen_bbox_cls', _masked_ce(cls_logits, bbox_class, valid), w['Ggen_bbox_cls'], hl.RATIO))
        else:
            terms.append(T('loss_Ggen_bbox_cls', F.cross_entropy(cls_logits, bbox_class[valid]), w['Ggen_bbox_cls']))
        terms += [T('loss_Ggen_text_rec', loss_lm, w['Ggen_text_rec']), T('loss_Ggen_text_len_rec', loss_text_len, w['Ggen_text_len_rec'])]
        total, rep = hl.combine(terms, gain)
        for k, v in rep.items():
            self.report('Loss/G/' + k, v)
        self.last = dict(bbox_fake=bbox_fake.detach(), **{k: v.detach() for k, v in rep.items()})
        return total

    def _generate_for_D(self, bbox_real, bbox_class, bbox_text, bbox_patch, padding_mask, background, gen_z, gen_c, trunk_out=None):
        g_trunk = None
        if trunk_out is None:
            g_trunk, trunk_out = self.grouped_trunks(background)
        bbox_fake = self.run_G(gen_z, bbox_class, bbox_real, bbox_text, bbox_patch, padding_mask, background, gen_c, update_emas=True, trunk_out=g_trunk)
        return bbox_fake, trunk_out

    def d_gen_terms(self, bbox_real, bbox_class, bbox_text, bbox_patch, padding_mask, background, gen_z, gen_c, trunk_out=None, gen_out=None):
        if gen_out is None:
            bbox_fake, trunk_out = self._generate_for_D(bbox_real, bbox_class, bbox_text, bbox_patch, padding_mask, background, gen_z, gen_c, trunk_out)
            gen_out = self.run_D(bbox_fake, bbox_class, bbox_text, bbox_patch, padding_mask, background, gen_c, update_emas=True, trunk_out=trunk_out)
        gen_logits, gen_logits_uncond = gen_out
        self.report('Loss/scores/fake', gen_logits)
        if self._reporting:
            self.report('Loss/signs/fake', gen_logits.sign())
        return [hl.Term('loss_Dgen', gen_logits, 1.0, hl.SOFTPLUS), hl.Term('loss_Dgen_uncond', gen_logits_uncond, 1.0, hl.SOFTPLUS)]

    def d_real_terms(self, bbox_real, bbox_class, bbox_text, bbox_patch, padding_mask, background, real_c, trunk_out=None, real_out=None):
        w = self.w
        valid = ~padding_mask
        static = bool(getattr(self.D, 'static_shapes', False))
        bbox_real_tmp = bbox_real.detach()
        if real_out is None:
            real_out = self.run_D(bbox_real_tmp, bbox_class, bbox_text, bbox_patch, padding_mask, background, real_c, reconst=True, trunk_out=trunk_out)
        (real_logits, real_logits_uncond, bbox_rec, cls_logits, loss_lm, loss_text_len, bg_rec, bbox_rec_uncond, cls_logits_uncond) = real_out
        T = hl.Term

        def ce(logits):
            if static:
                return dict(x=_masked_ce(logits, bbox_class, valid), fn=hl.RATIO)
            return dict(x=F.cross_entropy(logits, bbox_class[valid]))
        mse = (lambda a: _masked_mse(a, bbox_real_tmp, valid)) if static else (lambda a: F.mse_loss(a, bbox_real_tmp[valid]))
        self.report('Loss/scores/real', real_logits)
        if self._reporting:
            self.report('Loss/signs/real', real_logits.sign())
        return [T('loss_Dreal', real_logits, 1.0, hl.SOFTPLUS_NEG), T('loss_Dreal_uncond', real_logits_uncond, 1.0, hl.SOFTPLUS_NEG),
                T('loss_Dreal_bbox_rec', mse(bbox_rec), w['Dreal_bbox_rec']), T('loss_Dreal_bbox_cls', weight=w['Dreal_bbox_cls'], **ce(cls_logits)),
                T('loss_Dreal_text_rec', loss_lm, w['Dreal_text_rec']), T('loss_Dreal_text_len_rec', loss_text_len, w['Dreal_text_len_rec']),
                T('loss_Dreal_bg_rec', F.mse_loss(bg_rec, background), w['Dreal_im_rec']),
                T('loss_Dreal_bbox_rec_uncond', mse(bbox_rec_uncond), w['Dreal_bbox_rec']),
                T('loss_Dreal_bbox_cls_uncond', weight=w['Dreal_bbox_cls'], **ce(cls_logits_uncond))]

    def _finish(self, terms, prefix, gain=1.0):
        total, rep = hl.combine(terms, gain)
        for k, v in rep.items():
            self.report(prefix + k, v)
        return total

    def d_gen_loss(self, *args, gain=1.0, **kwargs):
        return self._finish(self.d_gen_terms(*args, **kwargs), 'Loss/D/', gain)

    def d_real_loss(self, *args, gain=1.0, **kwargs):
        return self._finish(self.d_real_terms(*args, **kwargs), 'Loss/D/', gain)

    def accumulate_gradients(self, phase, bbox_real, bbox_class, bbox_text, bbox_patch, padding_mask, background, real_c, gen_z, gen_c, gain, cur_nimg,
                             trunks=None):
        assert phase in ['Gmain', 'Greg', 'Gboth', 'Dmain', 'Dreg', 'Dboth']
        if self.pl_weight == 0:
# ... 3 lines not shown
        if isinstance(background, torch.Tensor) and background.is_cuda:
            core.zero_arena_begin(background.device)
        try:
            self._run_phase(phase, bbox_real, bbox_class, bbox_text, bbox_patch, padding_mask, background, real_c, gen_z, gen_c, gain, trunks)
        finally:
            core.zero_arena_end()

    def g_pl_loss(self, bbox_real, bbox_class, bbox_text, bbox_patch, padding_mask, background, gen_z, gen_c, gain=1.0):
        bs = gen_z.shape[0] // self.pl_batch_shrink
        z = gen_z[:bs].detach().requires_grad_(True)
        with composite.higher_order():
            bbox_fake = self.run_G(z, bbox_class[:bs], bbox_real[:bs], bbox_text[:bs], bbox_patch[:bs], padding_mask[:bs], background[:bs], gen_c[:bs])
        noise = self.pl_noise_fn(bbox_fake) if self.pl_noise_fn is not None else torch.randn_like(bbox_fake)
        pl_noise = noise / float(bbox_fake.shape[2])
        pl_grads = torch.autograd.grad(outputs=[(bbox_fake * pl_noise).sum()], inputs=[z], create_graph=True, only_inputs=True)[0]
        pl_lengths = pl_grads.square().sum([1, 2]).sqrt()
        pl_mean = self.pl_mean.lerp(pl_lengths.mean(), self.pl_decay)
        self.pl_mean.copy_(pl_mean.detach())
        pl_penalty = (pl_lengths - pl_mean).square()
        self.report('Loss/pl_penalty', pl_penalty)
        loss_Gpl = pl_penalty * self.pl_weight
        self.report('Loss/G/reg', loss_Gpl)
        self.last = dict(pl_penalty=pl_penalty.detach(), pl_lengths=pl_lengths.detach(), pl_grads=pl_grads.detach())
        return loss_Gpl.mean().mul(gain)

    def d_r1_loss(self, bbox_real, bbox_class, bbox_text, bbox_patch, padding_mask, background, real_c, gain=1.0):
        bbox_real_tmp = bbox_real.detach().requires_grad_(True)
        with composite.higher_order():
            real_logits, _ = self.run_D(bbox_real_tmp, bbox_class, bbox_text, bbox_patch, padding_mask, background, real_c)
        self.report('Loss/scores/real', real_logits)
        if self._reporting:
            self.report('Loss/signs/real', real_logits.sign())
        r1_grads = torch.autograd.grad(outputs=[real_logits.sum()], inputs=[bbox_real_tmp], create_graph=True, only_inputs=True)[0]
        r1_penalty = r1_grads.square().sum([1, 2])
        loss_Dr1 = r1_penalty * (self.r1_gamma / 2)
        self.report('Loss/r1_penalty', r1_penalty)
        self.report('Loss/D/reg', loss_Dr1)
        self.last = dict(r1_penalty=r1_penalty.detach(), r1_grads=r1_grads.detach(), real_logits=real_logits.detach())
        return loss_Dr1.mean().mul(gain)

    def _run_phase(self, phase, bbox_real, bbox_class, bbox_text, bbox_patch, padding_mask, background, real_c, gen_z, gen_c, gain, trunks):
        if phase in ('Greg', 'Gboth'):
            if phase == 'Gboth':
                self._run_phase('Gmain', bbox_real, bbox_class, bbox_text, bbox_patch, padding_mask, background, real_c, gen_z, gen_c, gain, trunks)
            self.g_pl_loss(bbox_real, bbox_class, bbox_text, bbox_patch, padding_mask, background, gen_z, gen_c, gain=gain).backward()
        if phase in ('Dreg', 'Dboth'):
            if phase == 'Dboth':
                self._run_phase('Dmain', bbox_real, bbox_class, bbox_text, bbox_patch, padding_mask, background, real_c, gen_z, gen_c, gain, trunks)
            self.d_r1_loss(bbox_real, bbox_class, bbox_text, bbox_patch, padding_mask, background, real_c, gain=gain).backward()
        if phase == 'Gmain':
            self.g_main_loss(bbox_real, bbox_class, bbox_text, bbox_patch, padding_mask, background, gen_z, gen_c, gain=gain, trunks=trunks).backward()
        if phase == 'Dmain':
            if self.share_D_trunk and hasattr(self.D, 'trunk'):
                bbox_fake, trunk = self._generate_for_D(bbox_real, bbox_class, bbox_text, bbox_patch, padding_mask, background, gen_z, gen_c,
                                                        None if trunks is None else trunks[1])
                if self.pair_D_passes:
                    gen_out, real_out = self.D.forward_pair(bbox_fake, bbox_real.detach(), bbox_class, bbox_text, bbox_patch, padding_mask, background, real_c,
                                                            trunk_out=trunk)
                else:
                    trunk = trunk if trunk is not None else self.D.trunk(background)
                    gen_out = self.run_D(bbox_fake, bbox_class, bbox_text, bbox_patch, padding_mask, background, gen_c, update_emas=True, trunk_out=trunk)
                    real_out = None
                t_gen = self.d_gen_terms(bbox_real, bbox_class, bbox_text, bbox_patch, padding_mask, background, gen_z, gen_c, gen_out=gen_out)
                t_real = self.d_real_terms(bbox_real, bbox_class, bbox_text, bbox_patch, padding_mask, background, real_c, trunk_out=trunk, real_out=real_out)
                self._finish(t_gen + t_real, 'Loss/D/', gain).backward()
            else:
                self.d_gen_loss(bbox_real, bbox_class, bbox_text, bbox_patch, padding_mask, background, gen_z, gen_c, gain=gain).backward()
                self.d_real_loss(bbox_real, bbox_class, bbox_text, bbox_patch, padding_mask, background, real_c, gain=gain).backward()
```

### layoutdetr_amd/training/networks_detr.py

```python
import numpy as np
import torch
import torch.nn as nn
import torch.nn.functional as F

from ..detr_util.misc import NestedTensor, nested_tensor_from_tensor_list
from ..hip import composite
from ..hip import conv as hconv
from ..hip import core
from ..hip.linear import linear
from .detr_backbone import Backbone, Joiner
from .detr_position_encoding import PositionEmbeddingSine
from .detr_transformer import Transformer, TransformerEncoder, TransformerEncoderLayer, TransformerWithToken
from .networks_stylegan2 import Decoder
from .util import TransformerWithToken_layoutganpp, encode_seq_first, encode_seq_first_pair


def merge_lists(lists):
    ret = []
    for l in lists:
        ret += l
    return ret


def split_list(list_a, chunk_size):
    return [list_a[i:i + chunk_size] for i in range(0, len(list_a), chunk_size)]


def normalize_2nd_moment(x, eps=1e-8):
    return x * (x.square().mean(dim=1, keepdim=True) + eps).rsqrt()


REFERENCE_DEFAULTS = False


def _resolve_text_mode(text_mode, tokenizer):
    if text_mode is not None:
        return text_mode
    if not REFERENCE_DEFAULTS:
        return 'features'
    if tokenizer is None:
        raise RuntimeError("Generator / Discriminator built through the reference's module names (layoutdetr_amd.dropin) take strings as bbox_text "
                           "and therefore need the BERT vocabulary: set LDETR_BERT_VOCAB=<path to bert-base-uncased vocab.txt> (or pass "
                           "tokenizer_vocab=...), or pass text_mode='features' and feed TextFeatures")
    return 'encoder+lm'


def build_backbone():
    backbone = Backbone(name='resnet50', train_backbone=True, return_interm_layers=None, dilation=False)
    position_embedding = PositionEmbeddingSine(num_pos_feats=128, normalize=True)
    model = Joiner(backbone, position_embedding)
    model.num_channels = backbone.num_channels
    return model


class TextFeatures(object):

    def __init__(self, text_feat, text_len, input_ids=None, attention_mask=None):
        self.text_feat = text_feat
        self.text_len = text_len
        self.input_ids = input_ids
        self.attention_mask = attention_mask

    def __len__(self):
        return self.text_feat.shape[0]

# ... 163 lines not shown

def _masked_ce_static(logits, target, valid):
    from .med import softmax_cross_entropy
    return softmax_cross_entropy(logits.flatten(0, 1), target.flatten().masked_fill(~valid.flatten(), -100))


def _zero_like_loss(ref):
    return ref.new_full((), 0.0)


class Generator(nn.Module):
    def __init__(self, z_dim, num_bbox_labels, img_channels, img_height, img_width, c_dim,
                 f_dim=256, num_heads=4, num_layers=8, hidden_dim=256,
                 med_config='configs/med_config.json', bert_f_dim=768, bert_num_encoder_layers=12, bert_num_decoder_layers=12,
                 bert_num_heads=12, background_size=1024, im_f_dim=512, max_text_length=256, text_mode=None, tokenizer_vocab=None):
        super().__init__()
        self.z_dim = z_dim
        self.tokenizer = _build_tokenizer(tokenizer_vocab)
        self.num_bbox_labels = num_bbox_labels
        self.c_dim = c_dim
        self.max_text_length = max_text_length
        self.text_mode = text_mode = _resolve_text_mode(text_mode, self.tokenizer)
        self.static_shapes = False
        _check_background_size(background_size)

        self.backbone = build_backbone()
        self.input_proj = Conv1x1(self.backbone.num_channels, hidden_dim, kernel_size=1)
        self.fc_z = Linear(z_dim * 9, bert_f_dim)
        self.emb_label = Embedding(num_bbox_labels, bert_f_dim)
        self.text_encoder = _build_text_encoder(text_mode, med_config, bert_num_encoder_layers, bert_num_heads)
        self.text_decoder = _build_text_decoder(text_mode, med_config, bert_num_decoder_layers, bert_num_heads, im_f_dim)
        self.enc_text_len = Embedding(max_text_length, bert_f_dim)
        self.fc_in = MLP(input_dim=4 * bert_f_dim, hidden_dim=bert_f_dim, output_dim=hidden_dim, num_layers=3)
        self.transformer = Transformer(d_model=hidden_dim, dropout=0.1, nhead=8, dim_feedforward=2048, num_encoder_layers=6,
                                       num_decoder_layers=6, normalize_before=False, return_intermediate_dec=False)
        self.bbox_embed = MLP(input_dim=hidden_dim, hidden_dim=hidden_dim, output_dim=4, num_layers=3)
        self.fc_z_rec = Linear(hidden_dim, z_dim * 9)
        self.fc_out_cls = Linear(hidden_dim, num_bbox_labels)
        self.fc_text_len_rec = Linear(hidden_dim, max_text_length)

    def trunk(self, background, body_out=None):
        if isinstance(background, (list, torch.Tensor)):
            background = nested_tensor_from_tensor_list(background)
        return self.backbone(background, body_out)

    def encode_condition(self, background, bbox_class, bbox_text, padding_mask):
        from . import shared_decode
        return shared_decode.encode_condition(self, background, bbox_class, bbox_text, padding_mask)

    def decode_candidates(self, cond, z):
        from . import shared_decode
        return shared_decode.decode_candidates(self, cond, z)

    def forward(self, z, bbox_class, bbox_real, bbox_text, bbox_patch, padding_mask, background, c, reconst=False, trunk_out=None):
        bg_feat, pos = self.trunk(background) if trunk_out is None else trunk_out
        bg_feat, mask = bg_feat[-1].decompose()
        assert mask is not None

        B, N = bbox_patch.shape[0], bbox_patch.shape[1]
        bbox_text = _coerce_text(self, bbox_text, bbox_class.device)
        z0 = normalize_2nd_moment(z.view(B, -1))
        zf = self.fc_z(z0).unsqueeze(1).expand(-1, N, -1)
        l = self.emb_label(bbox_class)
        text_feat, text_len = _text_inputs(self, bbox_text, B, N, bbox_class.device)
        text_len_feat = self.enc_text_len(text_len)
        x = torch.cat([zf, l, text_feat, text_len_feat], dim=-1)
        x = self.fc_in(x, final_relu=True).permute(1, 0, 2)

        x = self.transformer(src=self.input_proj(bg_feat), mask=mask, pos_embed=pos[-1], tgt=x, tgt_key_padding_mask=padding_mask)[0]
        bbox_fake = self.bbox_embed(x).sigmoid()
        if not reconst:
            return bbox_fake

        valid = ~padding_mask
        if self.static_shapes:
            z_rec = self.fc_z_rec(x)
            if z_rec.is_cuda and not z0.requires_grad:
                from ..hip.losses import masked_mse
                loss_z = masked_mse(z_rec, z0, valid.contiguous().view(torch.uint8), bdiv=N)
            else:
                vf = valid.to(torch.float32)
                cnt = vf.sum().clamp_min(1.0)
                loss_z = ((z_rec - z0.unsqueeze(1)).square().sum(-1) * vf).sum() / (cnt * z_rec.shape[-1])
            logit_cls = self.fc_out_cls(x)
            loss_text_len = _masked_ce_static(self.fc_text_len_rec(x), text_len, valid)
            loss_lm = _lm_loss(self, bbox_text, padding_mask, B, N, True)
            return bbox_fake, loss_z, logit_cls, (loss_lm if loss_lm is not None else _zero_like_loss(loss_z)), loss_text_len
        xv = x[valid]
        z_rec = self.fc_z_rec(xv)
        loss_z = F.mse_loss(z_rec, z0.unsqueeze(1).expand(-1, N, -1)[valid])
        logit_cls = self.fc_out_cls(xv)
        loss_lm = _lm_loss(self, bbox_text, padding_mask, B, N, False)
        loss_lm = loss_lm if loss_lm is not None else _zero_like_loss(loss_z)
        text_len_rec = self.fc_text_len_rec(xv)
        loss_text_len = F.cross_entropy(text_len_rec, text_len[valid])
        return bbox_fake, loss_z, logit_cls, loss_lm, loss_text_len


class Discriminator(nn.Module):
    def __init__(self, num_bbox_labels, img_channels, img_height, img_width, c_dim,
                 f_dim=256, num_heads=4, num_layers=8, max_bbox=50, hidden_dim=256,
                 med_config='configs/med_config.json', bert_f_dim=768, bert_num_encoder_layers=12, bert_num_decoder_layers=12,
                 bert_num_heads=12, background_size=1024, im_f_dim=512, max_text_length=256, text_mode=None, tokenizer_vocab=None):
        super().__init__()
        self.tokenizer = _build_tokenizer(tokenizer_vocab)
        self.num_bbox_labels = num_bbox_labels
        self.c_dim = c_dim
        self.max_text_length = max_text_length
        self.text_mode = text_mode = _resolve_text_mode(text_mode, self.tokenizer)
        self.static_shapes = False
        _check_background_size(background_size)

        self.backbone = build_backbone()
        self.input_proj = Conv1x1(self.backbone.num_channels, hidden_dim, kernel_size=1)
        self.fc_bbox = Linear(4, bert_f_dim)
        self.emb_label = Embedding(num_bbox_labels, bert_f_dim)
        self.text_encoder = _build_text_encoder(text_mode, med_config, bert_num_encoder_layers, bert_num_heads)
        self.text_decoder = _build_text_decoder(text_mode, med_config, bert_num_decoder_layers, bert_num_heads, im_f_dim)
        self.enc_text_len = Embedding(max_text_length, bert_f_dim)
        self.enc_fc_in = MLP(input_dim=4 * bert_f_dim, hidden_dim=bert_f_dim, output_dim=hidden_dim, num_layers=3)
        self.enc_transformer = TransformerWithToken(d_model=hidden_dim, dropout=0.1, nhead=8, dim_feedforward=2048,
                                                    num_encoder_layers=6, num_decoder_layers=6, normalize_before=False,
                                                    return_intermediate_dec=False)
        self.fc_out_disc = Linear(hidden_dim, 1)

        self.pos_token = nn.Parameter(torch.rand(max_bbox, 1, hidden_dim))
        self.dec_fc_in = Linear(hidden_dim + hidden_dim, hidden_dim)
        self.dec_transformer = TransformerEncoder(TransformerEncoderLayer(d_model=hidden_dim, nhead=8, dim_feedforward=2048), num_layers=6)
        self.bbox_embed = Linear(hidden_dim, 4)
        self.fc_out_cls = Linear(hidden_dim, num_bbox_labels)
        self.fc_text_len_rec = Linear(hidden_dim, max_text_length)
        self.bg_decoder = Decoder(z_dim=hidden_dim, w_dim=im_f_dim, channel_max=im_f_dim, channel_base=8192, img_channels=img_channels,
                                  img_resolution=background_size, use_noise=False, num_fp16_res=0, conv_clamp=None,
                                  fused_modconv_default=False)

        self.fc_bbox_uncond = Linear(4, bert_f_dim)
        self.emb_label_uncond = Embedding(num_bbox_labels, bert_f_dim)
        self.enc_fc_in_uncond = MLP(input_dim=2 * bert_f_dim, hidden_dim=bert_f_dim, output_dim=hidden_dim, num_layers=3)
        self.enc_transformer_uncond = TransformerWithToken_layoutganpp(d_model=hidden_dim, dim_feedforward=2048, nhead=8, num_layers=6)
        self.fc_out_disc_uncond = Linear(hidden_dim, 1)
        self.pos_token_uncond = nn.Parameter(torch.rand(max_bbox, 1, hidden_dim))
        self.dec_fc_in_uncond = Linear(hidden_dim + hidden_dim, hidden_dim)
        self.dec_transformer_uncond = TransformerEncoder(TransformerEncoderLayer(d_model=hidden_dim, nhead=8, dim_feedforward=2048), num_layers=6)
        self.bbox_embed_uncond = Linear(hidden_dim, 4)
        self.fc_out_cls_uncond = Linear(hidden_dim, num_bbox_labels)

    def trunk(self, background, body_out=None):
        if isinstance(background, (list, torch.Tensor)):
            background = nested_tensor_from_tensor_list(background)
        return self.backbone(background, body_out)

    def _logits(self, bbox, l, text_feat, text_len_feat, l_uncond, padding_mask, src, mask, pos):
        b = self.fc_bbox(bbox)
        x = torch.cat([b, l, text_feat, text_len_feat], dim=-1)
        x = self.enc_fc_in(x, final_relu=True).permute(1, 0, 2)
        x_uncond = torch.cat([self.fc_bbox_uncond(bbox), l_uncond], dim=-1)
        x_uncond = self.enc_fc_in_uncond(x_uncond, final_relu=True).permute(1, 0, 2)
        partner = None if composite.active() else self.enc_transformer_uncond.as_prog(x_uncond, padding_mask)
        if partner is not None:
            x, _, y_uncond = self.enc_transformer(src=src, mask=mask, pos_embed=pos, tgt=x, tgt_key_padding_mask=padding_mask, partner=partner[0])
            x_uncond = partner[1](y_uncond)
        else:
            x = self.enc_transformer(src=src, mask=mask, pos_embed=pos, tgt=x, tgt_key_padding_mask=padding_mask)[0]
            x_uncond = self.enc_transformer_uncond(x_uncond, src_key_padding_mask=padding_mask)
        x0 = x.transpose(0, 1)[0]
        logit_disc = self.fc_out_disc(x0).squeeze(-1)
        x0_uncond = x_uncond[0]
        return x0, logit_disc, x0_uncond, self.fc_out_disc_uncond(x0_uncond).squeeze(-1)

    def _reconstruct(self, x0, x0_uncond, bbox_text, text_len, padding_mask, B, N):
        valid = ~padding_mask
        x = x0.unsqueeze(0).expand(N, -1, -1)
        t = self.pos_token[:N].expand(-1, B, -1)
        x = self.dec_fc_in(torch.cat([x, t], dim=-1), relu=True)
        x_uncond = x0_uncond.unsqueeze(0).expand(N, -1, -1)
        t_uncond = self.pos_token_uncond[:N].expand(-1, B, -1)
        x_uncond = self.dec_fc_in_uncond(torch.cat([x_uncond, t_uncond], dim=-1), relu=True)
        x, x_uncond = encode_seq_first_pair(self.dec_transformer, x, self.dec_transformer_uncond, x_uncond, padding_mask)
        static = self.static_shapes
        x = x.permute(1, 0, 2) if static else x.permute(1, 0, 2)[valid]
        bbox_pred = self.bbox_embed(x).sigmoid()
        logit_cls = self.fc_out_cls(x)
        text_len_rec = self.fc_text_len_rec(x)
        if static:
            loss_text_len = _masked_ce_static(text_len_rec, text_len, valid)
        else:
            loss_text_len = F.cross_entropy(text_len_rec, text_len[valid])
        loss_lm = _lm_loss(self, bbox_text, padding_mask, B, N, static)
        loss_lm = loss_lm if loss_lm is not None else _zero_like_loss(loss_text_len)
        bg_rec = self.bg_decoder(x0)

        x_uncond = x_uncond.permute(1, 0, 2) if static else x_uncond.permute(1, 0, 2)[valid]
        bbox_pred_uncond = self.bbox_embed_uncond(x_uncond).sigmoid()
        logit_cls_uncond = self.fc_out_cls_uncond(x_uncond)
        return bbox_pred, logit_cls, loss_lm, loss_text_len, bg_rec, bbox_pred_uncond, logit_cls_uncond

    def forward(self, bbox, bbox_class, bbox_text, bbox_patch, padding_mask, background, c, reconst=False, trunk_out=None):
        bg_feat, pos = self.trunk(background) if trunk_out is None else trunk_out
        bg_feat, mask = bg_feat[-1].decompose()
        assert mask is not None

        B, N = bbox_patch.shape[0], bbox_patch.shape[1]
        bbox_text = _coerce_text(self, bbox_text, bbox_class.device)
        l = self.emb_label(bbox_class)
        text_feat, text_len = _text_inputs(self, bbox_text, B, N, bbox_class.device)
        text_len_feat = self.enc_text_len(text_len)
        x0, logit_disc, x0_uncond, logit_disc_uncond = self._logits(bbox, l, text_feat, text_len_feat, self.emb_label_uncond(bbox_class), padding_mask,
                                                                    self.input_proj(bg_feat), mask, pos[-1])
        if not reconst:
            return logit_disc, logit_disc_uncond
        return (logit_disc, logit_disc_uncond) + self._reconstruct(x0, x0_uncond, bbox_text, text_len, padding_mask, B, N)

    def forward_pair(self, bbox_fake, bbox_real, bbox_class, bbox_text, bbox_patch, padding_mask, background, c, trunk_out=None):
        bg_feat, pos = self.trunk(background) if trunk_out is None else trunk_out
        bg_feat, mask = bg_feat[-1].decompose()
        B, N = bbox_patch.shape[0], bbox_patch.shape[1]
        bbox_text = _coerce_text(self, bbox_text, bbox_class.device)
        l = self.emb_label(bbox_class)
        text_feat, text_len = _text_inputs(self, bbox_text, B, N, bbox_class.device)
        text_len_feat = self.enc_text_len(text_len)
        l_uncond = self.emb_label_uncond(bbox_class)
        two = lambda t: torch.cat([t, t], dim=0)
        x0, logit, x0_uncond, logit_uncond = self._logits(torch.cat([bbox_fake, bbox_real], dim=0), two(l), two(text_feat), two(text_len_feat), two(l_uncond),
                                                            two(padding_mask), two(self.input_proj(bg_feat)), two(mask), two(pos[-1]))
        rec = self._reconstruct(x0[B:], x0_uncond[B:], bbox_text, text_len, padding_mask, B, N)
        return (logit[:B], logit_uncond[:B]), (logit[B:], logit_uncond[B:]) + rec
```

### layoutdetr_amd/training/training_loop.py

```python
import copy

import numpy as np
import torch

from ..hip import core
from .detr_backbone import BackwardStages, trunk_body
from .networks_detr import split_list


def _phys_view(flat_slice, like):
    if like.is_contiguous():
        return flat_slice.view(like.shape)
    if like.ndim == 4 and like.is_contiguous(memory_format=torch.channels_last):
        O, I, KH, KW = like.shape
        return flat_slice.view(O, KH, KW, I).permute(0, 3, 1, 2)
    raise RuntimeError('FlatModule: parameter is neither contiguous nor channels_last')


def _trunk_bodies(module):
    from .detr_backbone import ResNet50Body
    return [m for m in module.modules() if isinstance(m, ResNet50Body)]


def refresh_weight_planes(module):
# ... 430 lines not shown
        try:
            return torch.load(resume_pkl, map_location='cpu')
        except Exception:
            raise RuntimeError(f'resume_pkl={resume_pkl!r}: neither a snapshot of this package (save_snapshot) nor a torch file of state dicts; '
                               f'pickles of the reference\'s own classes need the reference tree + its legacy loader ({e})')


def load_resume(resume_pkl, G, D, G_ema):
    data = read_snapshot(resume_pkl)
    for name, module in (('G', G), ('D', D), ('G_ema', G_ema)):
        if name in data and data[name] is not None:
            copy_params_and_buffers(data[name], module, require_all=False)


MIN_STAGE_MS = 1.5


def backward_stage_count(per_gpu_batch, stage_ms=None):
    import os
    forced = os.environ.get('LDETR_BACKWARD_STAGES')
    if forced in ('2', '3'):
        return int(forced)
    if stage_ms is not None and len(stage_ms) == 3:
        return 3 if min(stage_ms) >= MIN_STAGE_MS else 2
    return 2 if per_gpu_batch <= 4 else 3


def measure_backward_stages(loss, phase, dp, accumulate):
    segs = phase.fm.stage_segments(3)
    body = trunk_body(phase.module)
    if segs is None or body is None or not hasattr(body, 'stages') or not torch.cuda.is_available():
        return None
    ev = [torch.cuda.Event(enable_timing=True) for _ in range(4)]
    ev[0].record()
    staged_backward(loss, phase, dp, accumulate, between=lambda i: ev[i].record(), exchange=lambda ranges: None, n_stages=3)
    torch.cuda.synchronize()
    return [ev[i].elapsed_time(ev[i + 1]) for i in range(3)]


def staged_backward(loss, phase, dp, run_stage1, between=None, exchange=None, stages=None, n_stages=3):
    if stages is not None:
        n_stages = stages.n_stages
    segs = phase.fm.stage_segments(n_stages)
    body = trunk_body(phase.module)
    if segs is None or body is None or not hasattr(body, 'stages'):
        run_stage1()
        return False
    st = stages if stages is not None else BackwardStages(n_stages)
    if stages is None:
        body.stages = st
    if exchange is None:
        exchange = lambda ranges: [dp.exchange_async(phase.fm.gflat, lo, hi) for lo, hi in ranges]
    try:
        run_stage1()
        if between is not None:
            between(1)
        exchange(segs[0])
        for i in range(2, n_stages + 1):
            st.run(i)
            if between is not None:
                between(i)
            exchange(segs[i - 1])
    finally:
        body.stages = None
    return True


def _shares_iteration(loss, phases):
    return getattr(loss, 'share_D_trunk', None) == 'iteration' and any(p.name == 'Dmain' for p in phases)


def trunk_pre_pass(loss, phases, batch, batch_gpu, overlap, n_stages):
    if not _shares_iteration(loss, phases):
        return None, None
    b = batch['bbox_real'].shape[0]
    d_stages = None
    d_phase = next(p for p in phases if p.name == 'Dmain')
    if overlap and b <= batch_gpu and d_phase.fm.stage_segments() is not None and hasattr(trunk_body(d_phase.module), 'stages'):
        d_stages = BackwardStages(n_stages)
    pre = [loss.precompute_D_trunk(batch['background'][s:s + batch_gpu], stages=d_stages) for s in range(0, b, batch_gpu)]
    return [None if t is None else list(t) for t in pre], d_stages


def accumulate_micro_batches(loss, phase, batch, batch_gpu, gen_z, gen_c, gain, cur_nimg, pre=None):
    for i, s in enumerate(range(0, batch['bbox_real'].shape[0], batch_gpu)):
        sl = slice(s, s + batch_gpu)
        trunks = None if pre is None or pre[i] is None else tuple(pre[i])
        if trunks is not None and phase.name in ('Gmain', 'Gboth'):
            pre[i][0] = None
        if trunks is not None and phase.name == 'Dmain':
            pre[i] = None
        loss.accumulate_gradients(phase=phase.name, bbox_real=batch['bbox_real'][sl], bbox_class=batch['bbox_class'][sl],
                                  bbox_text=batch['bbox_text'][sl], bbox_patch=batch['bbox_patch'][sl],
                                  padding_mask=batch['padding_mask'][sl], background=batch['background'][sl],
                                  real_c=batch['real_c'][sl], gen_z=gen_z[sl], gen_c=gen_c[sl], gain=gain, cur_nimg=cur_nimg, trunks=trunks)


def training_iteration(loss, phases, dp, batch, batch_gpu, gen_z_per_phase, ema=None, batch_size=None, ema_kimg=None, cur_nimg=0, overlap=None,
                       gen_c_per_phase=None, ema_rampup=0.05, batch_idx=0):
    b = batch['bbox_real'].shape[0]
    core.reseed(batch['bbox_real'].device)
    if overlap is None:
        overlap = dp.world > 1
    pre, d_stages = trunk_pre_pass(loss, phases, batch, batch_gpu, overlap, backward_stage_count(b))
    lerp_done = False
    due = [batch_idx % getattr(p, 'interval', 1) == 0 for p in phases]
    last_of_fm = {id(p.fm): pi for pi, p in enumerate(phases) if due[pi]}
    for pi, (phase, gen_z) in enumerate(zip(phases, gen_z_per_phase)):
        if not due[pi]:
            continue
        regulariser = getattr(phase, 'main', phase) is not phase
        phase.fm.zero_grad()
        phase.module.requires_grad_(True)
        phase.module.text_encoder.requires_grad_(False)
        gen_c = batch['gen_c'] if gen_c_per_phase is None else gen_c_per_phase[pi]

# ... 297 lines not shown
```

Measured before the change: 522.2.

## Co-launch G and D encoder work as paired attention and GEMM kernels

Adds paired forward kernels for attention and small NT GEMMs. Each takes two independent problems and runs them in one grid, with the block index choosing which problem a block handles. The G generator and D discriminator transformer encoders over the same background are wired through an EncoderPartner/rider path so their layers can be issued together. The aim is to cut launch count and fill the GPU better on small per-layer problems. In exchange it adds a lot of plumbing through the training loop and a backward_staged flag, and it only supports 32-wide heads and problems that resolve to the same kernel instantiation.

New measurement: 528.6, median of 6. +1.2%, better.

```diff
diff --git a/include/ldetr_hip.h b/include/ldetr_hip.h
--- a/include/ldetr_hip.h
+++ b/include/ldetr_hip.h
@@ -69,6 +69,8 @@
 int ldetr_gemm_pair_f32(const ldetr_gemm_desc* g0, const ldetr_gemm_desc* g1, void* stream);
 int ldetr_gemm_pair_is_single_launch(const ldetr_gemm_desc* g0, const ldetr_gemm_desc* g1);
 
+int ldetr_gemm_pair_fwd_f32(const ldetr_gemm_desc* g0, const ldetr_gemm_desc* g1, void* stream);
+
 #define LDETR_GEMM_GROUP_MAX 32
 int ldetr_gemm_small_group_f32(const ldetr_gemm_desc* g, const float* post_scale, int n, void* stream);
 
@@ -103,6 +105,17 @@
                             const float* dout, int64_t lddo, float* dq, int64_t lddq, float* dk, int64_t lddk,
                             float* dv, int64_t lddv, int B, int H, int Lq, int Lk, int head_dim, float scale,
                             float p_drop, uint64_t seed, const uint64_t* seed_ptr, int causal, void* stream);
+
+typedef struct ldetr_attn_args {
+    const float* q; int64_t ldq; const float* k; int64_t ldk; const float* v; int64_t ldv;
+    const unsigned char* key_padding_mask;
+    float* out; int64_t ldo; float* lse;
+    int B, H, Lq, Lk, head_dim;
+    float scale, p_drop;
+    uint64_t seed; const uint64_t* seed_ptr;
+    int causal;
+} ldetr_attn_args;
+int ldetr_attention_fwd_group_f32(const ldetr_attn_args* a, int n, void* stream);
 
 int ldetr_torgb_bwd_finish_f32(const float* dws, const float* s, const float* w, int B, int C, float* dw, float* ds, void* stream);
 
diff --git a/layoutdetr_amd/_lib.py b/layoutdetr_amd/_lib.py
--- a/layoutdetr_amd/_lib.py
+++ b/layoutdetr_amd/_lib.py
@@ -39,6 +39,12 @@
                 ('pos', c_void_p), ('pos_rows', c_int64), ('ypos', c_void_p), ('dy2', c_void_p),
                 ('r_parts', c_int), ('r_part_stride', c_int64), ('r_bias', c_void_p),
                 ('dy_parts', c_void_p), ('dy_nparts', c_int), ('dy_part_stride', c_int64)]
+
+
+class AttnArgs(Structure):
+    _fields_ = [('q', c_void_p), ('ldq', c_int64), ('k', c_void_p), ('ldk', c_int64), ('v', c_void_p), ('ldv', c_int64), ('key_padding_mask', c_void_p),
+                ('out', c_void_p), ('ldo', c_int64), ('lse', c_void_p), ('B', c_int), ('H', c_int), ('Lq', c_int), ('Lk', c_int), ('head_dim', c_int),
+                ('scale', c_float), ('p_drop', c_float), ('seed', c_uint64), ('seed_ptr', c_void_p), ('causal', c_int)]
 
 
 class FfnArgs(Structure):
@@ -182,6 +188,8 @@
     'ldetr_sg2_handoff_f32': [_P, _P, _P, _P, _P, _P, _P, _P, _P, _P, _P, _P, _P, _P, _I, _L, _I, _F, _F, _P],
     'ldetr_gemm_pair_f32': [_P, _P, _P],
     'ldetr_gemm_pair_is_single_launch': [_P, _P],
+    'ldetr_gemm_pair_fwd_f32': [_P, _P, _P],
+    'ldetr_attention_fwd_group_f32': [_P, _I, _P],
     'ldetr_demod_fwd_f32': [_P, _L, _L, _L, _L, _P, _P, _P, _I, _I, _I, _I, _I, _F, _P],
     'ldetr_demod_bwd_f32': [_P, _L, _L, _L, _L, _P, _P, _P, _P, _P, _I, _P, _I, _I, _I, _I, _I, _P],
     'ldetr_demod_group_fwd_f32': [_P, _I, _I, _F, _P],
diff --git a/layoutdetr_amd/csrc/attention.hip b/layoutdetr_amd/csrc/attention.hip
--- a/layoutdetr_amd/csrc/attention.hip
+++ b/layoutdetr_amd/csrc/attention.hip
@@ -32,11 +32,11 @@
 }
 
 template <int NKT, int DHC>
-__global__ __launch_bounds__(64) void attn_fwd_kernel(AttnParams p) {
+__device__ __forceinline__ void attn_fwd_body(const AttnParams& p, const int blk) {
     constexpr int DH = 32 * DHC;
     const int nqt = (p.Lq + 15) >> 4;
-    const int qt = blockIdx.x % nqt;
-    const int bh = blockIdx.x / nqt;
+    const int qt = blk % nqt;
+    const int bh = blk / nqt;
     const int b = bh / p.H, h = bh - b * p.H;
     const int lane = threadIdx.x, li = lane & 15, g = lane >> 4;
     const int q0 = qt << 4;
@@ -104,6 +104,18 @@
 #pragma unroll
         for (int c = 0; c < 2 * DHC; c++) *reinterpret_cast<float4*>(op + 16 * c) = make_float4(o[c][0], o[c][1], o[c][2], o[c][3]);
     }
+}
+
+template <int NKT, int DHC>
+__global__ __launch_bounds__(64) void attn_fwd_kernel(AttnParams p) {
+    attn_fwd_body<NKT, DHC>(p, (int)blockIdx.x);
+}
+
+template <int NKT, int DHC>
+__global__ __launch_bounds__(64) void attn_fwd_pair_kernel(AttnParams pa, AttnParams pb, int nb0) {
+    const int blk = (int)blockIdx.x;
+    if (blk < nb0) attn_fwd_body<NKT, DHC>(pa, blk);
+    else attn_fwd_body<NKT, DHC>(pb, blk - nb0);
 }
 
 template <int DHC>
@@ -191,12 +203,12 @@
 }
 
 template <int NCH, int DHC>
-__global__ __launch_bounds__(256) void attn_fwd_wide_kernel(AttnParams p) {
+__device__ __forceinline__ void attn_fwd_wide_body(const AttnParams& p, const int blk) {
     constexpr int DH = 32 * DHC, DHP = DH + 4, NKT = 4 * NCH;
     extern __shared__ __attribute__((aligned(16))) float kv_tile[];
     const int nq64 = (p.Lq + 63) >> 6;
-    const int qb = blockIdx.x % nq64;
-    const int bh = blockIdx.x / nq64;
+    const int qb = blk % nq64;
+    const int bh = blk / nq64;
     const int b = bh / p.H, h = bh - b * p.H;
     const int wave = threadIdx.x >> 6, lane = threadIdx.x & 63, li = lane & 15, g = lane >> 4;
     const int qrow = (qb << 6) + (wave << 4) + li;
@@ -284,6 +296,18 @@
 #pragma unroll
         for (int cc = 0; cc < 2 * DHC; cc++) *reinterpret_cast<float4*>(op + 16 * cc) = make_float4(o[cc][0], o[cc][1], o[cc][2], o[cc][3]);
     }
+}
+
+template <int NCH, int DHC>
+__global__ __launch_bounds__(256) void attn_fwd_wide_kernel(AttnParams p) {
+    attn_fwd_wide_body<NCH, DHC>(p, (int)blockIdx.x);
+}
+
+template <int NCH, int DHC>
+__global__ __launch_bounds__(256) void attn_fwd_wide_pair_kernel(AttnParams pa, AttnParams pb, int nb0) {
+    const int blk = (int)blockIdx.x;
+    if (blk < nb0) attn_fwd_wide_body<NCH, DHC>(pa, blk);
+    else attn_fwd_wide_body<NCH, DHC>(pb, blk - nb0);
 }
 
 template <int NKT, int DHC>
@@ -578,6 +602,19 @@
 
 using namespace ldetr;
 
+static int attn_fwd_route(const AttnParams& p, int head_dim, int* tmpl) {
+    const int nkt = (p.Lk + 15) / 16;
+    *tmpl = 0;
+    if (nkt > 16) return 0;
+    if ((head_dim >= 64 || p.Lq >= 48) && (p.ldk % 4) == 0 && (p.ldv % 4) == 0 && ((((uintptr_t)p.k) | ((uintptr_t)p.v)) & 15) == 0) {
+        const int nch = (p.Lk + 63) / 64;
+        *tmpl = nch <= 1 ? 1 : nch <= 2 ? 2 : nch <= 3 ? 3 : 4;
+        return 2;
+    }
+    *tmpl = nkt <= 1 ? 1 : nkt <= 2 ? 2 : nkt <= 4 ? 4 : nkt <= 8 ? 8 : 16;
+    return 1;
+}
+
 extern "C" int ldetr_attention_fwd_f32(const float* q, int64_t ldq, const float* k, int64_t ldk, const float* v, int64_t ldv,
                                        const unsigned char* key_padding_mask, float* out, int64_t ldo, float* lse,
                                        int B, int H, int Lq, int Lk, int head_dim, float scale,
@@ -590,18 +627,20 @@
     LDETR_CHECK(!causal || Lq == Lk, "attention_fwd: the causal mask is defined for self-attention (Lq == Lk)");
     int rc = check_attn(p, "attention_fwd");
     if (rc) return rc;
-    const int nqt = (Lq + 15) / 16, nkt = (Lk + 15) / 16;
+    const int nqt = (Lq + 15) / 16;
     const int grid = B * H * nqt;
     hipStream_t st = (hipStream_t)stream;
+    int tmpl = 0;
+    const int route = attn_fwd_route(p, head_dim, &tmpl);
 #define LDETR_ATTN_FWD(DHC)                                                                     \
     do {                                                                                         \
-        if (nkt <= 1) hipLaunchKernelGGL((attn_fwd_kernel<1, DHC>), grid, 64, 0, st, p);         \
-        else if (nkt <= 2) hipLaunchKernelGGL((attn_fwd_kernel<2, DHC>), grid, 64, 0, st, p);    \
-        else if (nkt <= 4) hipLaunchKernelGGL((attn_fwd_kernel<4, DHC>), grid, 64, 0, st, p);    \
-        else if (nkt <= 8) hipLaunchKernelGGL((attn_fwd_kernel<8, DHC>), grid, 64, 0, st, p);    \
+        if (tmpl == 1) hipLaunchKernelGGL((attn_fwd_kernel<1, DHC>), grid, 64, 0, st, p);        \
+        else if (tmpl == 2) hipLaunchKernelGGL((attn_fwd_kernel<2, DHC>), grid, 64, 0, st, p);   \
+        else if (tmpl == 4) hipLaunchKernelGGL((attn_fwd_kernel<4, DHC>), grid, 64, 0, st, p);   \
+        else if (tmpl == 8) hipLaunchKernelGGL((attn_fwd_kernel<8, DHC>), grid, 64, 0, st, p);   \
         else hipLaunchKernelGGL((attn_fwd_kernel<16, DHC>), grid, 64, 0, st, p);                 \
     } while (0)
-    if (nkt > 16) {
+    if (route == 0) {
         switch (head_dim / 32) {
             case 1: hipLaunchKernelGGL((attn_fwd_long_kernel<1>), grid, 64, 0, st, p); break;
             case 2: hipLaunchKernelGGL((attn_fwd_long_kernel<2>), grid, 64, 0, st, p); break;
@@ -612,8 +651,8 @@
         }
         return check_launch("attention_fwd_long");
     }
-    if ((head_dim >= 64 || Lq >= 48) && (ldk % 4) == 0 && (ldv % 4) == 0 && ((((uintptr_t)k) | ((uintptr_t)v)) & 15) == 0) {
-        const int nch = (Lk + 63) / 64, wgrid = B * H * ((Lq + 63) / 64);
+    if (route == 2) {
+        const int nch = tmpl, wgrid = B * H * ((Lq + 63) / 64);
 #define LDETR_ATTN_WIDE(NCH, DHC)                                                                                         \
     do {                                                                                                                   \
         constexpr size_t lds = (size_t)64 * (32 * DHC + 4) * sizeof(float);                                                \
@@ -646,6 +685,55 @@
     }
 #undef LDETR_ATTN_FWD
     return check_launch("attention_fwd");
+}
+
+extern "C" int ldetr_attention_fwd_group_f32(const ldetr_attn_args* a, int n, void* stream) {
+    LDETR_CHECK(a && (n == 1 || n == 2), "attention_fwd_group: 1 or 2 problems");
+    if (n == 1)
+        return ldetr_attention_fwd_f32(a->q, a->ldq, a->k, a->ldk, a->v, a->ldv, a->key_padding_mask, a->out, a->ldo, a->lse, a->B, a->H, a->Lq, a->Lk,
+                                       a->head_dim, a->scale, a->p_drop, a->seed, a->seed_ptr, a->causal, stream);
+    AttnParams p[2];
+    int route[2], tmpl[2] = {0, 0};
+    for (int i = 0; i < 2; i++) {
+        const ldetr_attn_args& s = a[i];
+        if (s.head_dim != 32) {
+            set_error("attention_fwd_group: 32-wide heads only (problem %d has %d)", i, s.head_dim);
+            return LDETR_ERR_UNSUPPORTED;
+        }
+        AttnParams& q = p[i]; memset(&q, 0, sizeof(q));
+        q.q = s.q; q.k = s.k; q.v = s.v; q.ldq = s.ldq; q.ldk = s.ldk; q.ldv = s.ldv; q.kpm = s.key_padding_mask;
+        q.o = s.out; q.ldo = s.ldo; q.lse = s.lse; q.B = s.B; q.H = s.H; q.Lq = s.Lq; q.Lk = s.Lk;
+        q.scale = s.scale; q.p_drop = s.p_drop; q.seed = s.seed; q.seed_ptr = (const unsigned long long*)s.seed_ptr; q.causal = s.causal;
+        LDETR_CHECK(!s.causal || s.Lq == s.Lk, "attention_fwd_group: the causal mask is defined for self-attention (Lq == Lk)");
+        int rc = check_attn(q, "attention_fwd_group");
+        if (rc) return rc;
+        route[i] = attn_fwd_route(q, s.head_dim, &tmpl[i]);
+    }
+    if (route[0] == 0 || route[0] != route[1] || tmpl[0] != tmpl[1]) {
+        set_error("attention_fwd_group: the problems resolve to different kernels");
+        return LDETR_ERR_UNSUPPORTED;
+    }
+    hipStream_t st = (hipStream_t)stream;
+    if (route[0] == 2) {
+        const int nb0 = p[0].B * p[0].H * ((p[0].Lq + 63) / 64), nb1 = p[1].B * p[1].H * ((p[1].Lq + 63) / 64);
+        constexpr size_t lds = (size_t)64 * (32 + 4) * sizeof(float);
+        switch (tmpl[0]) {
+            case 1: hipLaunchKernelGGL((attn_fwd_wide_pair_kernel<1, 1>), nb0 + nb1, 256, lds, st, p[0], p[1], nb0); break;
+            case 2: hipLaunchKernelGGL((attn_fwd_wide_pair_kernel<2, 1>), nb0 + nb1, 256, lds, st, p[0], p[1], nb0); break;
+            case 3: hipLaunchKernelGGL((attn_fwd_wide_pair_kernel<3, 1>), nb0 + nb1, 256, lds, st, p[0], p[1], nb0); break;
+            default: hipLaunchKernelGGL((attn_fwd_wide_pair_kernel<4, 1>), nb0 + nb1, 256, lds, st, p[0], p[1], nb0); break;
+        }
+        return check_launch("attention_fwd_wide_pair");
+    }
+    const int nb0 = p[0].B * p[0].H * ((p[0].Lq + 15) / 16), nb1 = p[1].B * p[1].H * ((p[1].Lq + 15) / 16);
+    switch (tmpl[0]) {
+        case 1: hipLaunchKernelGGL((attn_fwd_pair_kernel<1, 1>), nb0 + nb1, 64, 0, st, p[0], p[1], nb0); break;
+        case 2: hipLaunchKernelGGL((attn_fwd_pair_kernel<2, 1>), nb0 + nb1, 64, 0, st, p[0], p[1], nb0); break;
+        case 4: hipLaunchKernelGGL((attn_fwd_pair_kernel<4, 1>), nb0 + nb1, 64, 0, st, p[0], p[1], nb0); break;
+        case 8: hipLaunchKernelGGL((attn_fwd_pair_kernel<8, 1>), nb0 + nb1, 64, 0, st, p[0], p[1], nb0); break;
+        default: hipLaunchKernelGGL((attn_fwd_pair_kernel<16, 1>), nb0 + nb1, 64, 0, st, p[0], p[1], nb0); break;
+    }
+    return check_launch("attention_fwd_pair");
 }
 
 extern "C" int ldetr_attention_bwd_f32(const float* q, int64_t ldq, const float* k, int64_t ldk, const float* v, int64_t ldv,
diff --git a/layoutdetr_amd/csrc/gemm_conv.hip b/layoutdetr_amd/csrc/gemm_conv.hip
--- a/layoutdetr_amd/csrc/gemm_conv.hip
+++ b/layoutdetr_amd/csrc/gemm_conv.hip
@@ -1296,13 +1296,18 @@
     return ring_alloc(0, bytes, &counters, &r) ? r : nullptr;
 }
 
+static int small_split_factor(int K, long blocks) {
+    int sk = 1;
+    if (blocks <= 128 && K >= 1024) {
+        sk = K / 256; if (sk > 8) sk = 8;
+        while (sk > 1 && blocks * sk > 640) sk--;
+    }
+    return sk;
+}
+
 static int plan_small_split(GemmParams& p, long blocks) {
-    int sk = 1;
-    if (blocks <= 128 && p.K >= 1024) {
-        sk = p.K / 256; if (sk > 8) sk = 8;
-        while (sk > 1 && blocks * sk > 640) sk--;
-        if (sk > 1 && !ring_alloc(blocks, (size_t)blocks * sk * 1024 * sizeof(float), &p.ws_count, &p.ws)) sk = 1;
-    }
+    int sk = small_split_factor(p.K, blocks);
+    if (sk > 1 && !ring_alloc(blocks, (size_t)blocks * sk * 1024 * sizeof(float), &p.ws_count, &p.ws)) sk = 1;
     return sk;
 }
 
@@ -1782,6 +1787,40 @@
     int rc = gemm_dense(*g0, stream);
     if (rc) return rc;
     return gemm_dense(*g1, stream);
+}
+
+extern "C" int ldetr_gemm_pair_fwd_f32(const ldetr_gemm_desc* g0, const ldetr_gemm_desc* g1, void* stream) {
+    LDETR_CHECK(g0 && g1, "gemm_pair_fwd: null descriptor");
+    const ldetr_gemm_desc* gs[2] = {g0, g1};
+    for (int i = 0; i < 2; i++) {
+        const ldetr_gemm_desc& q = *gs[i];
+        LDETR_CHECK(q.A && q.B && q.C, "gemm_pair_fwd: null pointer (problem %d)", i);
+        if (q.ta || q.tb || !small_class(q) || (q.ep && (q.ep->a_rowsum || q.ep->samp_scale))) {
+            set_error("gemm_pair_fwd: problem %d is not an NT small-tile problem", i);
+            return LDETR_ERR_UNSUPPORTED;
+        }
+    }
+    GemmParams p0 = fill_dense(*g0), p1 = fill_dense(*g1);
+    const int gx0 = cdiv(p0.N, 32), nt0 = gx0 * cdiv(p0.M, 32), gx1 = cdiv(p1.N, 32), nt1 = gx1 * cdiv(p1.M, 32);
+    const bool fast = small_fast_ok(p0, 0, 0);
+    if (fast != small_fast_ok(p1, 0, 0)) {
+        set_error("gemm_pair_fwd: the problems resolve to different instantiations (FAST)");
+        return LDETR_ERR_UNSUPPORTED;
+    }
+    if (small_wants8(nt0, small_split_factor(p0.K, nt0), p0.K) != small_wants8(nt1, small_split_factor(p1.K, nt1), p1.K)) {
+        set_error("gemm_pair_fwd: the problems resolve to different instantiations (waves)");
+        return LDETR_ERR_UNSUPPORTED;
+    }
+    const int sk0 = plan_small_split(p0, nt0), sk1 = plan_small_split(p1, nt1);
+    const bool w8 = small_wants8(nt0, sk0, p0.K);
+    if (w8 != small_wants8(nt1, sk1, p1.K)) {
+        set_error("gemm_pair_fwd: the problems resolve to different instantiations (waves, one split without workspace)");
+        return LDETR_ERR_UNSUPPORTED;
+    }
+    const dim3 grid((unsigned)(nt0 * sk0 + nt1 * sk1));
+    launch_small_kernel<0, 0, 0, 0>(fast, w8, grid, (hipStream_t)stream, p0, p1, gx0, nt0, sk0, gx1, nt1, sk1);
+    note_engine_launch(3, 32, 32, 0, w8 ? 8 : 4, fast ? 1 : 0, 0, sk0 * 256 + sk1, (long)grid.x, 0);
+    return check_launch("gemm_small_pair_fwd");
 }
 
 static int launch_small_group(const ldetr_gemm_desc* d, const float* post_scale, int n, hipStream_t st) {
diff --git a/layoutdetr_amd/hip/attention.py b/layoutdetr_amd/hip/attention.py
--- a/layoutdetr_amd/hip/attention.py
+++ b/layoutdetr_amd/hip/attention.py
@@ -2,7 +2,7 @@
 
 import torch
 
-from . import core
+from . import core, rider
 from .linear import linear
 
 
@@ -61,10 +61,13 @@
         lse = torch.empty((B * H * L,), device=qkv.device, dtype=torch.float32)
         seed = core.next_seed() if p_drop > 0 else 0
         scale = 1.0 / math.sqrt(dh)
-        core.check(core.lib().ldetr_attention_fwd_f32(
-            core.ptr(q), q.stride(0), core.ptr(k), k.stride(0), core.ptr(v), v.stride(0), core.ptr(kpm),
-            core.ptr(out), d, core.ptr(lse), B, H, L, L, dh, scale, p_drop, seed, core.seed_ptr() if p_drop > 0 else None,
-            1 if causal else 0, core.stream()), 'attention_fwd')
+        if rider.MODE is not None:
+            rider.attention(q, k, v, kpm, out, lse, B, H, L, dh, scale, p_drop, seed, 1 if causal else 0)
+        else:
+            core.check(core.lib().ldetr_attention_fwd_f32(
+                core.ptr(q), q.stride(0), core.ptr(k), k.stride(0), core.ptr(v), v.stride(0), core.ptr(kpm),
+                core.ptr(out), d, core.ptr(lse), B, H, L, L, dh, scale, p_drop, seed, core.seed_ptr() if p_drop > 0 else None,
+                1 if causal else 0, core.stream()), 'attention_fwd')
         ctx.save_for_backward(qkv, v_sep, kpm, out, lse)
         ctx.cfg = (B, H, L, dh, scale, p_drop, seed, 1 if causal else 0)
         return out
diff --git a/layoutdetr_amd/hip/blocks.py b/layoutdetr_amd/hip/blocks.py
--- a/layoutdetr_amd/hip/blocks.py
+++ b/layoutdetr_amd/hip/blocks.py
@@ -1,7 +1,7 @@
 import math
 
 from .. import _lib
-from . import core
+from . import core, rider
 
 D_MODEL, N_HEAD = 256, 8
 SCALE = 1.0 / math.sqrt(D_MODEL // N_HEAD)
@@ -14,6 +14,8 @@
 
 def launch(what, args, flops=0.0, nbytes=0.0):
     entry, grouped = _ENTRIES[what]
+    if rider.takes_block(what, args):
+        return rider.block(what, args[0])
     fn = getattr(core.lib(), entry)
     n = len(args)
     arr = (type(args[0]) * n)(*args)
@@ -51,6 +53,9 @@
     a.r_bias = _p(r_bias) if r_parts > 0 else None
     if pos is not None:
         a.pos, a.pos_rows, a.ypos = pos.data_ptr(), pos.shape[0], ypos.data_ptr()
+    if rider.MODE == 'record':
+        a._keep = (x, r, gamma, beta, y, z, mean, rstd, r_bias, pos, ypos)
+        a._outs = (y, z, mean, rstd, ypos)
     return a
 
 
@@ -71,6 +76,9 @@
     a.x, a.ldx, a.w1, a.b1, a.w2, a.h, a.ypart = x.data_ptr(), x.stride(0), w1.data_ptr(), b1.data_ptr(), w2.data_ptr(), h.data_ptr(), ypart.data_ptr()
     a.M, a.F = h.shape
     _set_dropout(a, p_drop, seed)
+    if rider.MODE == 'record':
+        a._keep = (x, w1, b1, w2, h, ypart)
+        a._outs = (h, ypart)
     return a
 
 
diff --git a/layoutdetr_amd/hip/core.py b/layoutdetr_amd/hip/core.py
--- a/layoutdetr_amd/hip/core.py
+++ b/layoutdetr_amd/hip/core.py
@@ -109,6 +109,7 @@
 
 
 
+_rider = None
 _workspace = {}
 WORKSPACE_BYTES = int(os.environ.get('LDETR_WORKSPACE_MIB', '256')) << 20
 
@@ -150,6 +151,8 @@
 
 
 def stream():
+    if _rider is not None and _rider.MODE == 'record':
+        raise RuntimeError('a launch that hip.rider does not queue was issued while an encoder stack was being recorded')
     return ctypes.c_void_p(torch.cuda.current_stream().cuda_stream)
 
 
@@ -162,15 +165,55 @@
 def f32c(t):
     if t is None:
         return None
+    if _rider is not None and _rider.MODE == 'record' and (t.dtype != torch.float32 or not t.is_contiguous()):
+        _rider.check_ready(t, 'f32c (copy)')
     if t.dtype != torch.float32:
         t = t.float()
     return t.contiguous()
 
 
+def _seed_at(position):
+    base = int(torch.initial_seed()) & 0xFFFFFFFF
+    return ((base << 32) ^ (position * 0x9E3779B1)) & 0xFFFFFFFFFFFFFFFF
+
+
 def next_seed():
+    if _seed_lease[0] is not None:
+        return _seed_lease[0].draw()
     _seed_counter[0] += 1
-    base = int(torch.initial_seed()) & 0xFFFFFFFF
-    return ((base << 32) ^ (_seed_counter[0] * 0x9E3779B1)) & 0xFFFFFFFFFFFFFFFF
+    return _seed_at(_seed_counter[0])
+
+
+class SeedLease(object):
+
+    def __init__(self, start):
+        self.start, self.drawn = start, 0
+
+    def draw(self):
+        self.drawn += 1
+        return _seed_at(self.start + self.drawn)
+
+    def __enter__(self):
+        assert _seed_lease[0] is None
+        _seed_lease[0] = self
+        return self
+
+    def __exit__(self, *exc):
+        _seed_lease[0] = None
+        return False
+
+    def redeem(self):
+        if _seed_counter[0] != self.start:
+            return False
+        _seed_counter[0] += self.drawn
+        return True
+
+
+_seed_lease = [None]
+
+
+def seed_position():
+    return _seed_counter[0]
 
 
 _iter_seed = {}
@@ -229,6 +272,8 @@
     ep.seed_ptr = iter_seed().data_ptr() if p_drop > 0 else None
     ep.accumulate = 1 if accumulate else 0
     ep.a_rowsum = a_rowsum.data_ptr() if a_rowsum is not None else None
+    if _rider is not None and _rider.MODE == 'record':
+        ep._keep = (col_scale, col_bias, samp_scale, residual, mask_src, a_rowsum)
     return ep
 
 
@@ -238,6 +283,9 @@
         out = torch.empty((M, N), device=A.device, dtype=torch.float32)
     lda = A.stride(0) if lda is None else lda
     ldb = B.stride(0) if ldb is None else ldb
+    if _rider is not None and _rider.MODE is not None and not ta and not tb and splitk == 0 and pix_per_sample == 0:
+        _rider.gemm(A, B, M, N, K, out, ep, lda, ldb)
+        return out
     engine_call('gemm', 2.0 * M * N * K, lambda: check(lib().ldetr_gemm_f32(
         ptr(A), lda, int(ta), ptr(B), ldb, int(tb), ptr(out), out.stride(0), M, N, K, splitk,
         ctypes.byref(ep) if ep is not None else None, pix_per_sample, stream()), 'gemm'), nbytes=4.0 * (M * K + N * K + M * N))
diff --git a/layoutdetr_amd/hip/linear.py b/layoutdetr_amd/hip/linear.py
--- a/layoutdetr_amd/hip/linear.py
+++ b/layoutdetr_amd/hip/linear.py
@@ -44,6 +44,8 @@
         if add_input is not None:
             if add_input.requires_grad:
                 raise RuntimeError('linear: add_input is a constant (the sine position embedding); a learned embedding must be added by the caller')
+            if core._rider is not None:
+                core._rider.check_ready(x2, 'linear(add_input=)')
             x2 = x2 + add_input.reshape(-1, K)
         w = core.f32c(weight.detach()[r0:r1])
         b = core.f32c(bias.detach()[r0:r1]) if bias is not None else None
diff --git a/layoutdetr_amd/hip/rider.py b/layoutdetr_amd/hip/rider.py
--- /dev/null
+++ b/layoutdetr_amd/hip/rider.py
@@ -0,0 +1,145 @@
+import ctypes
+import sys
+
+from .. import _lib
+from . import core
+
+ENABLED = bool(core.knob('ENC_RIDER', 1))
+MODE = None
+STATS = dict(paired=0, split=0, alone=0)
+_queue = []
+_unwritten = set()
+_BLOCK_KINDS = ('layernorm_fwd', 'ffn_fwd')
+
+
+class _Pending(object):
+    __slots__ = ('kind', 'args', 'keep')
+
+    def __init__(self, kind, args, keep, outs=()):
+        self.kind, self.args, self.keep = kind, args, keep
+        if MODE == 'record':
+            _unwritten.update(t.untyped_storage().data_ptr() for t in outs if t is not None)
+
+
+def check_ready(t, what):
+    if MODE == 'record' and t is not None and t.untyped_storage().data_ptr() in _unwritten:
+        raise RuntimeError(f'{what}: reads the result of a launch that hip.rider has queued and not sent yet')
+
+
+def _take(kind):
+    if _queue and _queue[0].kind == kind:
+        return _queue.pop(0)
+    return None
+
+
+def _send_alone(p):
+    l = core.lib()
+    if p.kind == 'gemm':
+        d, ep = p.args, p.keep[3]
+        core.check(l.ldetr_gemm_f32(ctypes.c_void_p(d.A), d.lda, 0, ctypes.c_void_p(d.B), d.ldb, 0, ctypes.c_void_p(d.C), d.ldc, d.M, d.N, d.K, 0,
+                                    ctypes.byref(ep) if ep is not None else None, 0, core.stream()), 'gemm')
+    elif p.kind == 'attention':
+        core.check(l.ldetr_attention_fwd_group_f32(ctypes.byref(p.args), 1, core.stream()), 'attention_fwd')
+    else:
+        entry = getattr(l, 'ldetr_' + p.kind + '_group_f32')
+        core.check(entry(ctypes.byref(p.args), 1, core.stream()), p.kind)
+
+
+def _send(me):
+    if MODE == 'record':
+        _queue.append(me)
+        return
+    mate = _take(me.kind)
+    if mate is None:
+        STATS['alone'] += 1
+        _send_alone(me)
+        return
+    l = core.lib()
+    if me.kind == 'gemm':
+        rc = l.ldetr_gemm_pair_fwd_f32(ctypes.byref(mate.args), ctypes.byref(me.args), core.stream())
+    elif me.kind == 'attention':
+        arr = (_lib.AttnArgs * 2)(mate.args, me.args)
+        rc = l.ldetr_attention_fwd_group_f32(arr, 2, core.stream())
+    else:
+        arr = (type(me.args) * 2)(mate.args, me.args)
+        rc = getattr(l, 'ldetr_' + me.kind + '_group_f32')(arr, 2, core.stream())
+    if rc == 3:
+        STATS['split'] += 1
+        _send_alone(mate)
+        _send_alone(me)
+        return
+    core.check(rc, me.kind + ' (pair)')
+    STATS['paired'] += 1
+
+
+def gemm(A, B, M, N, K, out, ep, lda, ldb):
+    d = _lib.GemmDesc()
+    d.A, d.lda, d.ta, d.B, d.ldb, d.tb = A.data_ptr(), lda, 0, B.data_ptr(), ldb, 0
+    d.C, d.ldc, d.M, d.N, d.K, d.splitk = out.data_ptr(), out.stride(0), int(M), int(N), int(K), 0
+    d.ep = ctypes.addressof(ep) if ep is not None else None
+    d.pix_per_sample = 0
+    _send(_Pending('gemm', d, (A, B, out, ep, getattr(ep, '_keep', None)), outs=(out,)))
+
+
+def attention(q, k, v, kpm, out, lse, B, H, L, dh, scale, p_drop, seed, causal):
+    a = _lib.AttnArgs()
+    a.q, a.ldq, a.k, a.ldk, a.v, a.ldv = q.data_ptr(), q.stride(0), k.data_ptr(), k.stride(0), v.data_ptr(), v.stride(0)
+    a.key_padding_mask = kpm.data_ptr() if kpm is not None else None
+    a.out, a.ldo, a.lse = out.data_ptr(), out.stride(0), lse.data_ptr()
+    a.B, a.H, a.Lq, a.Lk, a.head_dim, a.scale, a.p_drop, a.seed = B, H, L, L, dh, scale, p_drop, seed
+    a.seed_ptr = core.iter_seed().data_ptr() if p_drop > 0 else None
+    a.causal = causal
+    _send(_Pending('attention', a, (q, k, v, kpm, out, lse), outs=(out, lse)))
+
+
+def takes_block(what, args):
+    return MODE is not None and what in _BLOCK_KINDS and len(args) == 1
+
+
+def block(what, a):
+    _send(_Pending(what, a, getattr(a, '_keep', None), outs=getattr(a, '_outs', ())))
+
+
+def flush():
+    while _queue:
+        STATS['alone'] += 1
+        _send_alone(_queue.pop(0))
+
+
+class mode(object):
+
+    def __init__(self, m):
+        self.m = m
+
+    def __enter__(self):
+        global MODE
+        assert MODE is None, 'rider modes do not nest'
+        MODE = self.m
+
+    def __exit__(self, et, ev, tb):
+        global MODE
+        MODE = None
+        if et is not None:
+            del _queue[:]
+        elif self.m == 'pair':
+            flush()
+        if et is not None or self.m == 'pair':
+            _unwritten.clear()
+        return False
+
+
+def eligible(enc_a, enc_b, rows_a, rows_b, staged=False, higher_order=False, profiled=False):
+    if not ENABLED or staged or higher_order or profiled:
+        return False
+    la, lb = list(enc_a.layers), list(enc_b.layers)
+    if len(la) != len(lb) or not la or enc_a.norm is not None or enc_b.norm is not None:
+        return False
+    from . import ffn as hffn
+    for x, y in zip(la, lb):
+        if (x.self_attn.embed_dim != y.self_attn.embed_dim or x.self_attn.num_heads != y.self_attn.num_heads
+                or x.linear1.weight.shape != y.linear1.weight.shape or x.self_attn.embed_dim // x.self_attn.num_heads != 32):
+            return False
+    return (rows_a <= hffn.MAX_ROWS) == (rows_b <= hffn.MAX_ROWS)
+
+
+core._rider = sys.modules[__name__]
diff --git a/layoutdetr_amd/training/detr_transformer.py b/layoutdetr_amd/training/detr_transformer.py
--- a/layoutdetr_amd/training/detr_transformer.py
+++ b/layoutdetr_amd/training/detr_transformer.py
@@ -1,3 +1,4 @@
+import contextlib
 import copy
 from typing import Optional
 
@@ -5,6 +6,7 @@
 from torch import Tensor, nn
 
 from ..hip import composite, core
+from ..hip import rider as hrider
 from ..hip.attention import kpm_u8 as _mask_u8
 from ..hip.attention import grouped_kv, mha_cross_kv, mha_forward
 from ..hip import ffn as hffn
@@ -121,6 +123,18 @@
         prog = hstacks.Prog('enc', self.layers, x2, B, L, _mask_u8(kpm), self.training)
         return prog if hstacks.usable(prog) else None
 
+    def forward(self, x2, B, L, kpm, pos2, want_pos=False, rider=None, lease=None, rider_lease=None):
+        if rider is None:
+            with (lease if lease is not None else contextlib.nullcontext()):
+                return self.forward2d(x2, B, L, kpm, pos2, want_pos=want_pos)
+        enc, rx2, rB, rL, rkpm, rpos2 = rider
+        assert pos2 is not None and rpos2 is not None, 'the lock-step path is the position-embedded encoders\''
+        with torch.no_grad(), (rider_lease if rider_lease is not None else contextlib.nullcontext()), hrider.mode('record'):
+            other = enc.forward2d(rx2, rB, rL, rkpm, rpos2, want_pos=want_pos)
+        with (lease if lease is not None else contextlib.nullcontext()), hrider.mode('pair'):
+            mine = self.forward2d(x2, B, L, kpm, pos2, want_pos=want_pos)
+        return mine, other
+
     def forward2d(self, x2, B, L, kpm, pos2, want_pos=False):
         kpm = _mask_u8(kpm)
         if pos2 is None and not want_pos:
@@ -132,6 +146,7 @@
         for i, layer in enumerate(self.layers):
             emit = pos2 is not None and (i + 1 < n or (want_pos and self.norm is None))
             if pos2 is not None and xpos2 is None:
+                hrider.check_ready(x2, 'encoder layer input + pos')
                 xpos2 = x2 + pos2
             r = layer.forward2d(x2, B, L, kpm, pos2, xpos2=xpos2, emit_pos=emit)
             x2, xpos2 = r if emit else (r, None)
@@ -178,6 +193,26 @@
     return x.permute(0, 2, 3, 1).reshape(B * h * w, C), h * w
 
 
+class EncoderPartner(object):
+
+    def __init__(self, encoder, src, mask, pos_embed, plan, key):
+        self.encoder, self.src, self.mask, self.pos_embed, self.plan, self.key = encoder, src, mask, pos_embed, plan, key
+        self.memory = self.lease = self.probe_start = None
+
+    def collect(self):
+        if self.memory is not None:
+            mem, lease = self.memory, self.lease
+            self.memory = self.lease = None
+            if lease.redeem():
+                return mem
+            self.plan.pop(self.key, None)
+            return None
+        if self.probe_start is not None:
+            self.plan[self.key] = core.seed_position() - self.probe_start
+            self.probe_start = None
+        return None
+
+
 class Transformer(nn.Module):
     _with_token = False
 
@@ -206,7 +241,31 @@
             if p.dim() > 1:
                 nn.init.xavier_uniform_(p)
 
-    def forward(self, src, mask, pos_embed, tgt, tgt_key_padding_mask, decoder_mask=None, partner=None):
+    def _encode(self, x2, bs, S, mem_kpm, pos2, enc_partner, enc_memory):
+        if enc_memory is not None:
+            got = enc_memory.collect()
+            if got is not None:
+                return got
+        if enc_partner is None:
+            return self.encoder.forward2d(x2, bs, S, mem_kpm, pos2, want_pos=True)
+        p = enc_partner
+        start = core.seed_position()
+        px2, pS = _rows_from_nchw(p.src)
+        ppos2 = _rows_from_nchw(p.pos_embed)[0].contiguous()
+        pkpm, pbs = p.mask.flatten(1), p.src.shape[0]
+        gap = p.plan.get(p.key)
+        if gap is None or not hrider.eligible(self.encoder, p.encoder, x2.shape[0], px2.shape[0], profiled=core.PROF.enabled):
+            p.probe_start = start
+            return self.encoder.forward2d(x2, bs, S, mem_kpm, pos2, want_pos=True)
+        lease = core.SeedLease(start + gap)
+        if torch.is_grad_enabled() and (px2.requires_grad or any(q.requires_grad for q in p.encoder.parameters())):
+            other, mine = p.encoder(px2, pbs, pS, pkpm, ppos2, want_pos=True, rider=(self.encoder, x2, bs, S, mem_kpm, pos2), lease=lease)
+        else:
+            mine, other = self.encoder(x2, bs, S, mem_kpm, pos2, want_pos=True, rider=(p.encoder, px2, pbs, pS, pkpm, ppos2), rider_lease=lease)
+        p.memory, p.lease = other, lease
+        return mine
+
+    def forward(self, src, mask, pos_embed, tgt, tgt_key_padding_mask, decoder_mask=None, partner=None, enc_partner=None, enc_memory=None):
         if decoder_mask is not None:
             raise NotImplementedError('decoder_mask (tgt_mask) is never passed on the LayoutDETR path')
         bs, c, h, w = src.shape
@@ -214,7 +273,7 @@
         pos2, _ = _rows_from_nchw(pos_embed)
         pos2 = pos2.contiguous()
         mem_kpm = mask.flatten(1)
-        mem2, mem_pos2 = self.encoder.forward2d(x2, bs, S, mem_kpm, pos2, want_pos=True)
+        mem2, mem_pos2 = self._encode(x2, bs, S, mem_kpm, pos2, enc_partner, enc_memory)
         if self._with_token:
             tgt = torch.cat([self.token.expand(-1, bs, -1), tgt], dim=0)
             tgt_key_padding_mask = torch.cat([self.token_mask.expand(bs, -1), tgt_key_padding_mask], dim=1)
diff --git a/layoutdetr_amd/training/loss.py b/layoutdetr_amd/training/loss.py
--- a/layoutdetr_amd/training/loss.py
+++ b/layoutdetr_amd/training/loss.py
@@ -7,7 +7,9 @@
 
 from ..hip import losses as hl
 from ..metrics.metric_layoutnet import compute_alignment, compute_overlap, generalized_iou_loss, layout_losses_per_sample
+from ..hip import rider as hrider
 from .detr_backbone import ResNet50Body, dual_trunk_forward, trunk_body
+from .detr_transformer import Transformer
 
 
 def _masked_mse(a, b, valid):
@@ -43,6 +45,18 @@
 def _detached(trunk_out):
     feats, pos = trunk_out
     return [NestedTensor(f.tensors.detach(), f.mask, getattr(f, 'uniform', False)) for f in feats], [p.detach() for p in pos]
+
+
+def _staged(module):
+    body = trunk_body(module)
+    return getattr(body, 'stages', None) is not None
+
+
+def encoder_partner_applies(G, D, background, staged=False, higher_order=False):
+    gt, dt = getattr(G, 'transformer', None), getattr(D, 'enc_transformer', None)
+    if not (hasattr(D, 'encoder_partner') and isinstance(gt, Transformer) and isinstance(dt, Transformer) and isinstance(background, torch.Tensor)):
+        return False
+    return hrider.eligible(gt.encoder, dt.encoder, 1, 1, staged=staged, higher_order=higher_order)
 
 
 class Loss:
@@ -78,6 +92,8 @@
                       Ggen_text_len_rec=Ggen_text_len_rec_weight)
         self.share_D_trunk = share_D_trunk
         self.pair_D_passes = bool(share_D_trunk) and hasattr(D, 'forward_pair')
+        self.backward_staged = False
+        self._enc_plan = {}
         self._reporting = report_fn is not None
         self.report = report_fn if report_fn is not None else (lambda name, value: None)
         self.last = {}
@@ -112,15 +128,20 @@
             return None, None
         return self.G.trunk(background, body_out=outs[0]), self.D.trunk(background, body_out=outs[1])
 
-    def run_G(self, z, bbox_class, bbox_real, bbox_text, bbox_patch, padding_mask, background, c, reconst=False, update_emas=False, trunk_out=None):
+    def run_G(self, z, bbox_class, bbox_real, bbox_text, bbox_patch, padding_mask, background, c, reconst=False, update_emas=False, trunk_out=None,
+              enc_partner=None):
         kw = {} if trunk_out is None else dict(trunk_out=trunk_out)
+        if enc_partner is not None:
+            kw['enc_partner'] = enc_partner
         if not reconst:
             return self.G(z, bbox_class, bbox_real, bbox_text, bbox_patch, padding_mask, background, c, **kw)
         return self.G(z, bbox_class, bbox_real, bbox_text, bbox_patch, padding_mask, background, c, reconst, **kw)
 
     def run_D(self, bbox, bbox_class, bbox_text, bbox_patch, padding_mask, background, c, reconst=False, blur_sigma=0, update_emas=False,
-              trunk_out=None):
+              trunk_out=None, enc_memory=None):
         kw = {} if trunk_out is None else dict(trunk_out=trunk_out)
+        if enc_memory is not None:
+            kw['enc_memory'] = enc_memory
         if not reconst:
             return self.D(bbox, bbox_class, bbox_text, bbox_patch, padding_mask, background, c, **kw)
         return self.D(bbox, bbox_class, bbox_text, bbox_patch, padding_mask, background, c, reconst, **kw)
@@ -130,9 +151,11 @@
         valid = ~padding_mask
         static = bool(getattr(self.G, 'static_shapes', False))
         g_trunk, d_trunk = self.grouped_trunks(background) if trunks is None else (trunks[0], _detached(trunks[1]))
+        partner = self.encoder_partner('Gmain', d_trunk, background)
         bbox_fake, loss_z, cls_logits, loss_lm, loss_text_len = self.run_G(gen_z, bbox_class, bbox_real, bbox_text, bbox_patch, padding_mask, background, gen_c,
-                                                                           reconst=True, trunk_out=g_trunk)
-        gen_logits, gen_logits_uncond = self.run_D(bbox_fake, bbox_class, bbox_text, bbox_patch, padding_mask, background, gen_c, trunk_out=d_trunk)
+                                                                           reconst=True, trunk_out=g_trunk, enc_partner=partner)
+        gen_logits, gen_logits_uncond = self.run_D(bbox_fake, bbox_class, bbox_text, bbox_patch, padding_mask, background, gen_c, trunk_out=d_trunk,
+                                                   enc_memory=partner)
         T = hl.Term
         lay = None
         if static and bbox_fake.is_cuda and bbox_fake.shape[1] <= 64:
@@ -165,11 +188,18 @@
         self.last = dict(bbox_fake=bbox_fake.detach(), **{k: v.detach() for k, v in rep.items()})
         return total
 
-    def _generate_for_D(self, bbox_real, bbox_class, bbox_text, bbox_patch, padding_mask, background, gen_z, gen_c, trunk_out=None):
+    def encoder_partner(self, phase, d_trunk, background, pair=False):
+        staged = self.backward_staged or _staged(self.G) or _staged(self.D)
+        if d_trunk is None or not encoder_partner_applies(self.G, self.D, background, staged=staged, higher_order=composite.active()):
+            return None
+        return self.D.encoder_partner(d_trunk, self._enc_plan, (phase, tuple(background.shape), self.G.training, self.D.training), pair=pair)
+
+    def _generate_for_D(self, bbox_real, bbox_class, bbox_text, bbox_patch, padding_mask, background, gen_z, gen_c, trunk_out=None, enc_partner=None):
         g_trunk = None
         if trunk_out is None:
             g_trunk, trunk_out = self.grouped_trunks(background)
-        bbox_fake = self.run_G(gen_z, bbox_class, bbox_real, bbox_text, bbox_patch, padding_mask, background, gen_c, update_emas=True, trunk_out=g_trunk)
+        bbox_fake = self.run_G(gen_z, bbox_class, bbox_real, bbox_text, bbox_patch, padding_mask, background, gen_c, update_emas=True, trunk_out=g_trunk,
+                               enc_partner=enc_partner)
         return bbox_fake, trunk_out
 
     def d_gen_terms(self, bbox_real, bbox_class, bbox_text, bbox_patch, padding_mask, background, gen_z, gen_c, trunk_out=None, gen_out=None):
@@ -279,11 +309,12 @@
             self.g_main_loss(bbox_real, bbox_class, bbox_text, bbox_patch, padding_mask, background, gen_z, gen_c, gain=gain, trunks=trunks).backward()
         if phase == 'Dmain':
             if self.share_D_trunk and hasattr(self.D, 'trunk'):
+                partner = self.encoder_partner('Dmain', trunks[1], background, pair=True) if (trunks is not None and self.pair_D_passes) else None
                 bbox_fake, trunk = self._generate_for_D(bbox_real, bbox_class, bbox_text, bbox_patch, padding_mask, background, gen_z, gen_c,
-                                                        None if trunks is None else trunks[1])
+                                                        None if trunks is None else trunks[1], enc_partner=partner)
                 if self.pair_D_passes:
                     gen_out, real_out = self.D.forward_pair(bbox_fake, bbox_real.detach(), bbox_class, bbox_text, bbox_patch, padding_mask, background, real_c,
-                                                            trunk_out=trunk)
+                                                            trunk_out=trunk, **({} if partner is None else dict(enc_memory=partner)))
                 else:
                     trunk = trunk if trunk is not None else self.D.trunk(background)
                     gen_out = self.run_D(bbox_fake, bbox_class, bbox_text, bbox_patch, padding_mask, background, gen_c, update_emas=True, trunk_out=trunk)
diff --git a/layoutdetr_amd/training/networks_detr.py b/layoutdetr_amd/training/networks_detr.py
--- a/layoutdetr_amd/training/networks_detr.py
+++ b/layoutdetr_amd/training/networks_detr.py
@@ -10,7 +10,7 @@
 from ..hip.linear import linear
 from .detr_backbone import Backbone, Joiner
 from .detr_position_encoding import PositionEmbeddingSine
-from .detr_transformer import Transformer, TransformerEncoder, TransformerEncoderLayer, TransformerWithToken
+from .detr_transformer import EncoderPartner, Transformer, TransformerEncoder, TransformerEncoderLayer, TransformerWithToken
 from .networks_stylegan2 import Decoder
 from .util import TransformerWithToken_layoutganpp, encode_seq_first, encode_seq_first_pair
 
@@ -280,7 +280,7 @@
         from . import shared_decode
         return shared_decode.decode_candidates(self, cond, z)
 
-    def forward(self, z, bbox_class, bbox_real, bbox_text, bbox_patch, padding_mask, background, c, reconst=False, trunk_out=None):
+    def forward(self, z, bbox_class, bbox_real, bbox_text, bbox_patch, padding_mask, background, c, reconst=False, trunk_out=None, enc_partner=None):
         bg_feat, pos = self.trunk(background) if trunk_out is None else trunk_out
         bg_feat, mask = bg_feat[-1].decompose()
         assert mask is not None
@@ -295,7 +295,7 @@
         x = torch.cat([zf, l, text_feat, text_len_feat], dim=-1)
         x = self.fc_in(x, final_relu=True).permute(1, 0, 2)
 
-        x = self.transformer(src=self.input_proj(bg_feat), mask=mask, pos_embed=pos[-1], tgt=x, tgt_key_padding_mask=padding_mask)[0]
+        x = self.transformer(src=self.input_proj(bg_feat), mask=mask, pos_embed=pos[-1], tgt=x, tgt_key_padding_mask=padding_mask, enc_partner=enc_partner)[0]
         bbox_fake = self.bbox_embed(x).sigmoid()
         if not reconst:
             return bbox_fake
@@ -378,7 +378,7 @@
             background = nested_tensor_from_tensor_list(background)
         return self.backbone(background, body_out)
 
-    def _logits(self, bbox, l, text_feat, text_len_feat, l_uncond, padding_mask, src, mask, pos):
+    def _logits(self, bbox, l, text_feat, text_len_feat, l_uncond, padding_mask, src, mask, pos, enc_memory=None):
         b = self.fc_bbox(bbox)
         x = torch.cat([b, l, text_feat, text_len_feat], dim=-1)
         x = self.enc_fc_in(x, final_relu=True).permute(1, 0, 2)
@@ -386,10 +386,10 @@
         x_uncond = self.enc_fc_in_uncond(x_uncond, final_relu=True).permute(1, 0, 2)
         partner = None if composite.active() else self.enc_transformer_uncond.as_prog(x_uncond, padding_mask)
         if partner is not None:
-            x, _, y_uncond = self.enc_transformer(src=src, mask=mask, pos_embed=pos, tgt=x, tgt_key_padding_mask=padding_mask, partner=partner[0])
+            x, _, y_uncond = self.enc_transformer(src=src, mask=mask, pos_embed=pos, tgt=x, tgt_key_padding_mask=padding_mask, partner=partner[0], enc_memory=enc_memory)
             x_uncond = partner[1](y_uncond)
         else:
-            x = self.enc_transformer(src=src, mask=mask, pos_embed=pos, tgt=x, tgt_key_padding_mask=padding_mask)[0]
+            x = self.enc_transformer(src=src, mask=mask, pos_embed=pos, tgt=x, tgt_key_padding_mask=padding_mask, enc_memory=enc_memory)[0]
             x_uncond = self.enc_transformer_uncond(x_uncond, src_key_padding_mask=padding_mask)
         x0 = x.transpose(0, 1)[0]
         logit_disc = self.fc_out_disc(x0).squeeze(-1)
@@ -423,7 +423,15 @@
         logit_cls_uncond = self.fc_out_cls_uncond(x_uncond)
         return bbox_pred, logit_cls, loss_lm, loss_text_len, bg_rec, bbox_pred_uncond, logit_cls_uncond
 
-    def forward(self, bbox, bbox_class, bbox_text, bbox_patch, padding_mask, background, c, reconst=False, trunk_out=None):
+    def encoder_partner(self, trunk_out, plan, key, pair=False):
+        bg_feat, pos = trunk_out
+        bg_feat, mask = bg_feat[-1].decompose()
+        src, pe = self.input_proj(bg_feat), pos[-1]
+        if pair:
+            src, mask, pe = torch.cat([src, src], dim=0), torch.cat([mask, mask], dim=0), torch.cat([pe, pe], dim=0)
+        return EncoderPartner(self.enc_transformer.encoder, src, mask, pe, plan, key)
+
+    def forward(self, bbox, bbox_class, bbox_text, bbox_patch, padding_mask, background, c, reconst=False, trunk_out=None, enc_memory=None):
         bg_feat, pos = self.trunk(background) if trunk_out is None else trunk_out
         bg_feat, mask = bg_feat[-1].decompose()
         assert mask is not None
@@ -434,12 +442,13 @@
         text_feat, text_len = _text_inputs(self, bbox_text, B, N, bbox_class.device)
         text_len_feat = self.enc_text_len(text_len)
         x0, logit_disc, x0_uncond, logit_disc_uncond = self._logits(bbox, l, text_feat, text_len_feat, self.emb_label_uncond(bbox_class), padding_mask,
-                                                                    self.input_proj(bg_feat), mask, pos[-1])
+                                                                    enc_memory.src if enc_memory is not None else self.input_proj(bg_feat), mask, pos[-1],
+                                                                    enc_memory=enc_memory)
         if not reconst:
             return logit_disc, logit_disc_uncond
         return (logit_disc, logit_disc_uncond) + self._reconstruct(x0, x0_uncond, bbox_text, text_len, padding_mask, B, N)
 
-    def forward_pair(self, bbox_fake, bbox_real, bbox_class, bbox_text, bbox_patch, padding_mask, background, c, trunk_out=None):
+    def forward_pair(self, bbox_fake, bbox_real, bbox_class, bbox_text, bbox_patch, padding_mask, background, c, trunk_out=None, enc_memory=None):
         bg_feat, pos = self.trunk(background) if trunk_out is None else trunk_out
         bg_feat, mask = bg_feat[-1].decompose()
         B, N = bbox_patch.shape[0], bbox_patch.shape[1]
@@ -450,6 +459,8 @@
         l_uncond = self.emb_label_uncond(bbox_class)
         two = lambda t: torch.cat([t, t], dim=0)
         x0, logit, x0_uncond, logit_uncond = self._logits(torch.cat([bbox_fake, bbox_real], dim=0), two(l), two(text_feat), two(text_len_feat), two(l_uncond),
-                                                            two(padding_mask), two(self.input_proj(bg_feat)), two(mask), two(pos[-1]))
+                                                            two(padding_mask), enc_memory.src if enc_memory is not None else two(self.input_proj(bg_feat)),
+                                                            enc_memory.mask if enc_memory is not None else two(mask),
+                                                            enc_memory.pos_embed if enc_memory is not None else two(pos[-1]), enc_memory=enc_memory)
         rec = self._reconstruct(x0[B:], x0_uncond[B:], bbox_text, text_len, padding_mask, B, N)
         return (logit[:B], logit_uncond[:B]), (logit[B:], logit_uncond[B:]) + rec
diff --git a/layoutdetr_amd/training/training_loop.py b/layoutdetr_amd/training/training_loop.py
--- a/layoutdetr_amd/training/training_loop.py
+++ b/layoutdetr_amd/training/training_loop.py
@@ -506,6 +506,7 @@
     if exchange is None:
         exchange = lambda ranges: [dp.exchange_async(phase.fm.gflat, lo, hi) for lo, hi in ranges]
     try:
+        loss.backward_staged = True
         run_stage1()
         if between is not None:
             between(1)
@@ -516,6 +517,7 @@
                 between(i)
             exchange(segs[i - 1])
     finally:
+        loss.backward_staged = False
         body.stages = None
     return True
 
```
